# OSLL/slam-constructor

Hardware: AMD Instinct MI355X
Metric: pose-candidates*beams/sec (1080-beam scan, 2000^2 grid) (higher is better)
Workload: dtype f64; 1 GPU; cfg2: tinySLAM HC(dt 0.1, dr 0.1, failed-rounds 128), 1080 beams, 2000x2000 @0.05 m, occupancy cell; parallelism=1 gpu, ranks=1, includes_filter_and_upload=True, mode=default (canonical tree sum, device sincos; com~

## Files before the change

### include/slamhip.h

```cpp
#ifndef SLAMHIP_H
#define SLAMHIP_H

#include <stddef.h>
#include <stdint.h>

#ifdef __cplusplus
extern "C" {
#endif

#define SLAMHIP_VERSION 100

typedef enum {
  SLAMHIP_OK = 0,
  SLAMHIP_ERR_INVALID = -1,
  SLAMHIP_ERR_HIP = -2,
  SLAMHIP_ERR_NO_DEVICE = -3,
  SLAMHIP_ERR_STATE = -4,
  SLAMHIP_ERR_UNSUPPORTED = -5,
  SLAMHIP_ERR_TIMEOUT = -6
} slamhip_status;

enum { SLAMHIP_CELL_OCC = 0, SLAMHIP_CELL_TBM = 1, SLAMHIP_CELL_GMAPPING = 2, SLAMHIP_CELL_CREDIBILIST = 3 };
enum { SLAMHIP_OOPE_OBSTACLE = 0, SLAMHIP_OOPE_MAX = 1, SLAMHIP_OOPE_MEAN = 2,
       SLAMHIP_OOPE_OVERLAP = 3, SLAMHIP_OOPE_GMAPPING = 4 };
enum { SLAMHIP_OIE_DISCREPANCY = 0, SLAMHIP_OIE_OCCUPANCY = 1 };
enum { SLAMHIP_SUM_TREE256 = 0, SLAMHIP_SUM_SEQUENTIAL = 1 };
enum { SLAMHIP_POSE_TRIG_DEVICE = 0, SLAMHIP_POSE_TRIG_HOST = 1,
       SLAMHIP_POSE_TRIG_RAW_EXACT = 2 };
enum { SLAMHIP_TRIG_RAW = 0, SLAMHIP_TRIG_CACHED = 1 };

typedef struct slamhip_ctx slamhip_ctx;
typedef struct slamhip_matcher slamhip_matcher;

typedef struct {
  int oope;
  int oie;
  double area[4];
  double gm_fullness_th;
  int gm_window;
  int sum_order;
  int pose_trig;
} slamhip_spe_cfg;

const char *slamhip_last_error(void);
int slamhip_device_count(int *count);
int slamhip_ctx_create(int device, slamhip_ctx **out);
int slamhip_ctx_destroy(slamhip_ctx *ctx);
int slamhip_ctx_synchronize(slamhip_ctx *ctx);
void *slamhip_ctx_stream(slamhip_ctx *ctx);
enum {
  SLAMHIP_OPT_LOW_LATENCY = 0,
  SLAMHIP_OPT_STAGE_POSES = 1,
  SLAMHIP_OPT_FILTER_CHAINS = 2,
  SLAMHIP_OPT_K6_PATH = 3,
  SLAMHIP_OPT_K6_BATCH_FAST = 4,
  SLAMHIP_OPT_RESIDENT_CHAINS = 6,
  SLAMHIP_OPT_K6_BATCH_KEY64 = 5,
  SLAMHIP_OPT_TBM_PLANE = 7,
  SLAMHIP_OPT_INERT_TAIL = 8
};
int slamhip_ctx_set_option(slamhip_ctx *ctx, int option, int value);
int slamhip_ctx_get_option(slamhip_ctx *ctx, int option, int *value);

int slamhip_map_bind(slamhip_ctx *ctx, int map_id, int cell_model, int width, int height,
                     int origin_x, int origin_y, double scale, const double *unknown_payload);
int slamhip_map_upload_window(slamhip_ctx *ctx, int map_id, int x0, int y0, int w, int h,
                              const double *payload);
int slamhip_map_apply_dirty(slamhip_ctx *ctx, int map_id, int n, const int *coords_xy,
                            const double *payloads);
int slamhip_map_release(slamhip_ctx *ctx, int map_id);
int slamhip_map_set_auto_grow(slamhip_ctx *ctx, int map_id, int on);
int slamhip_map_info(slamhip_ctx *ctx, int map_id, int *cell_model, int *width, int *height, int *origin_x,
                     int *origin_y, double *scale, long long *times_grown);
int slamhip_map_download_window(slamhip_ctx *ctx, int map_id, int x0, int y0, int w, int h,
                                double *payload_out);

enum { SLAMHIP_RENDER_OCCGRID = 0, SLAMHIP_RENDER_PGM = 1 };
enum { SLAMHIP_OCC_TBM_CONSISTENT = 0, SLAMHIP_OCC_TBM_UNKNOWN_EVEN = 1 };
int slamhip_map_render(slamhip_ctx *ctx, int map_id, int format, int occ_kind, int x0, int y0, int w, int h,
                       void *out);
int slamhip_render_cells(int cell_model, int occ_kind, int format, int n, const double *payload, void *out);

enum { SLAMHIP_SCAN_GEN_SEQUENTIAL = 1 };
int slamhip_scan_gen_libm_variant(int *variant);
int slamhip_scan_gen_angles(double half_sector, double angle_inc, int cap, double *angles, int *n);
int slamhip_map_generate_scans(slamhip_ctx *ctx, int map_id, int occ_kind, int variant, int flags, int n_poses,
                               const double *poses_xyt, int n_angles, const double *angles, double max_dist,
                               double occ_threshold, double *range_out, unsigned char *status_out);
int slamhip_scan_generate_host(int cell_model, int occ_kind, int variant, int width, int height, int origin_x, int origin_y,
                               double scale, const double *unknown_payload, const double *payload, int n_poses,
                               const double *poses_xyt, int n_angles, const double *angles, double max_dist,
                               double occ_threshold, double *range_out, unsigned char *status_out);

typedef struct slamhip_pyramid slamhip_pyramid;
int slamhip_pyramid_create(slamhip_ctx *ctx, int fine_map_id, int oie, int first_level_map_id, slamhip_pyramid **out);
int slamhip_pyramid_destroy(slamhip_pyramid *pyr);
int slamhip_pyramid_info(slamhip_pyramid *pyr, int *n_levels, int cap, int *map_id, int *width, int *height,
                         int *origin_x, int *origin_y, double *scale);
int slamhip_pyramid_rebuild(slamhip_pyramid *pyr);
int slamhip_pyramid_refresh(slamhip_pyramid *pyr, int x0, int y0, int w, int h);
int slamhip_pyramid_build_host(int cell_model, int oie, int width, int height, int origin_x, int origin_y, double scale,
                               const double *unknown_payload, const double *payload, int level_cap, int *n_levels,
                               int *level_width, int *level_height, int *level_origin_x, int *level_origin_y,
                               double *level_scale, size_t payload_cap, double *payload_out, size_t *payload_need);
int slamhip_pyramid_score_matches(slamhip_ctx *ctx, slamhip_pyramid *pyr, const slamhip_spe_cfg *cfg,
                                  const double base_pose[3], int n, const double *rotation, const double *rect,
                                  double *score_out, int *level_out);
int slamhip_pyramid_score_matches_device(slamhip_ctx *ctx, slamhip_pyramid *pyr, const slamhip_spe_cfg *cfg,
                                         const double base_pose[3], int n, const double *d_rotation, const double *d_rect,
                                         double *d_score_out, int *d_level_out);

enum { SLAMHIP_RULE_LAST = 0,
       SLAMHIP_RULE_AFFINE = 1,
       SLAMHIP_RULE_MEAN = 2,
       SLAMHIP_RULE_TBM = 3,
       SLAMHIP_RULE_GMAPPING = 4   };
typedef struct {
  int rule;
  double scan_quality;
  double base_occupied_prob, base_occupied_qual;
  double base_empty_prob, base_empty_qual;
  double blur;
  double max_range;
  int occupancy_estimator;
  double area_shift_amount;
} slamhip_scan_adder_cfg;
int slamhip_map_append_scan(slamhip_ctx *ctx, int map_id, const slamhip_scan_adder_cfg *cfg,
                            const double pose[3], int n, const double *range, const double *cos_a,
                            const double *sin_a, const int *is_occ, long long *n_updates);
int slamhip_map_append_scan_q(slamhip_ctx *ctx, int map_id, const slamhip_scan_adder_cfg *cfg,
                              const double pose[3], int n, const double *range, const double *cos_a,
                              const double *sin_a, const int *is_occ, const double *quality, long long *n_updates);
int slamhip_map_append_scan_raw(slamhip_ctx *ctx, int map_id, const slamhip_scan_adder_cfg *cfg, const double pose[3],
                                int n, const double *range, const double *angle, const int *is_occ,
                                const double *quality, long long *n_updates);
int slamhip_omqe_quality(int kind, int n, const double *range, const double *angle, double *out);
int slamhip_map_set_deferred(slamhip_ctx *ctx, int on);
int slamhip_map_drain(slamhip_ctx *ctx, long long *n_updates);
int slamhip_map_download_aux(slamhip_ctx *ctx, int map_id, int x0, int y0, int w, int h, double *out);

int slamhip_scan_upload(slamhip_ctx *ctx, int n, const double *range, const double *cos_a,
                        const double *sin_a, const double *weight, const double *factor);
int slamhip_scan_store(slamhip_ctx *ctx, int slot, int n, const double *range, const double *cos_a,
                       const double *sin_a, const double *weight, const double *factor);
int slamhip_scan_select(slamhip_ctx *ctx, int slot);
int slamhip_scan_set_angles(slamhip_ctx *ctx, int n, const double *angle);
int slamhip_libm_variant(int *variant);
int slamhip_libm_eval(slamhip_ctx *ctx, int variant, int fn, int n, const double *x, double *out);
int slamhip_beam_trig_raw(int n, const double *angle, double *cos_out, double *sin_out);
int slamhip_beam_trig_cached(int n, const double *angle, double a_min, double a_max, double a_inc,
                             double *cos_out, double *sin_out);
int slamhip_filter_scan(int n, const double *range, const double *angle, const int *is_occ,
                        int trig_mode, double a_min, double a_delta, int table_n,
                        const double *tab_sin, const double *tab_cos, const double pose[3],
                        unsigned skip_rate, double max_range, int bounded, int width, int height,
                        int origin_x, int origin_y, double scale, int *kept_idx, int *kept_n);
int slamhip_scan_filter_upload(slamhip_ctx *ctx, int map_id, int n, const double *range, const double *angle,
                               const int *is_occ, const double *factor, int trig_mode, double a_min, double a_max,
                               double a_inc, const double pose[3], unsigned skip_rate, double max_range, int bounded,
                               int weighting, int *kept_n, int *kept_idx);
int slamhip_scan_table_uploads(slamhip_ctx *ctx, long long *uploads);
int slamhip_scan_download(slamhip_ctx *ctx, int cap, double *out5, int *n);
int slamhip_scan_weights(int kind, int n, const double *range, const double *angle, double *out);

int slamhip_score_poses(slamhip_ctx *ctx, int map_id, const slamhip_spe_cfg *cfg, int n_poses,
                        const double *poses_xyt, double *scores_out);
int slamhip_score_poses_device(slamhip_ctx *ctx, int map_id, const slamhip_spe_cfg *cfg,
                               int n_poses, const double *d_poses_xyt, double *d_scores_out);
int slamhip_gm_cache_reset(slamhip_ctx *ctx);
int slamhip_gm_cache_get(slamhip_ctx *ctx, int *cell_xy, double *prob);
int slamhip_gm_cache_set(slamhip_ctx *ctx, const int *cell_xy, double prob);

int slamhip_profile_enable(slamhip_ctx *ctx, int on);
int slamhip_profile_read(slamhip_ctx *ctx, double *kernel_ms_total, long long *launches,
                         long long *units , int reset);

int slamhip_profile_read_map_update(slamhip_ctx *ctx, double *ms_total, long long *calls, long long *records,
                                    int reset);

typedef struct {
  void *user;
  void (*on_scan_test)(void *user, const double pose[3], double score);
  void (*on_pose_update)(void *user, const double pose[3], double score);
  void (*on_matching_end)(void *user, const double delta[3], double best_score);
} slamhip_observer;

int slamhip_matcher_create_mc(slamhip_ctx *ctx, const slamhip_spe_cfg *cfg, unsigned seed,
                              double translation_dispersion, double rotation_dispersion,
                              unsigned failed_attempts_limit, unsigned attempts_limit,
                              slamhip_matcher **out);
int slamhip_matcher_create_hc(slamhip_ctx *ctx, const slamhip_spe_cfg *cfg,
                              unsigned failed_rounds_limit, double translation_delta,
                              double rotation_delta, slamhip_matcher **out);
int slamhip_matcher_create_bf(slamhip_ctx *ctx, const slamhip_spe_cfg *cfg, const double range9[9],
                              slamhip_matcher **out);
int slamhip_matcher_destroy(slamhip_matcher *m);
int slamhip_matcher_reset_state(slamhip_matcher *m);
int slamhip_matcher_set_observer(slamhip_matcher *m, const slamhip_observer *obs);
int slamhip_matcher_set_batch(slamhip_matcher *m, int max_batch);
int slamhip_matcher_set_device_chain(slamhip_matcher *m, int mode, int threads);
int slamhip_matcher_resident_stats(slamhip_matcher *m, long long *matches, long long *gave_up);
int slamhip_matcher_set_tie_check(slamhip_matcher *m, int on);
int slamhip_matcher_process_scan(slamhip_matcher *m, int map_id, const double init_pose[3],
                                 double out_delta[3], double *out_prob);
typedef struct slamhip_raw_scan {
  int n;
  const double *range, *angle;
  const int *is_occ;
  const double *factor;
  int trig_mode;
  double a_min, a_max, a_inc;
// ... 133 lines not shown
```

### slam-constructor_amd/__init__.py

```python
import atexit
import ctypes as C
import os
import subprocess
import weakref

import numpy as np

PKG_DIR = os.path.dirname(os.path.abspath(__file__))
LIB_PATH = os.path.join(PKG_DIR, "libslamhip.so")
TESTING_LIB_PATH = os.path.join(PKG_DIR, "libslamhip_testing.so")
CSRC = os.path.join(PKG_DIR, "csrc")

CELL_OCC, CELL_TBM, CELL_GMAPPING, CELL_CREDIBILIST = 0, 1, 2, 3
OOPE_OBSTACLE, OOPE_MAX, OOPE_MEAN, OOPE_OVERLAP, OOPE_GMAPPING = range(5)
OIE_DISCREPANCY, OIE_OCCUPANCY = 0, 1
SUM_TREE256, SUM_SEQUENTIAL = 0, 1
POSE_TRIG_DEVICE, POSE_TRIG_HOST, POSE_TRIG_RAW_EXACT = 0, 1, 2
(OPT_LOW_LATENCY, OPT_STAGE_POSES, OPT_FILTER_CHAINS, OPT_K6_PATH, OPT_K6_BATCH_FAST, OPT_K6_BATCH_KEY64,
 OPT_RESIDENT_CHAINS, OPT_TBM_PLANE, OPT_INERT_TAIL) = range(9)
TRIG_RAW, TRIG_CACHED = 0, 1
RENDER_OCCGRID, RENDER_PGM = 0, 1
OCC_TBM_CONSISTENT, OCC_TBM_UNKNOWN_EVEN = 0, 1
SCAN_GEN_SEQUENTIAL = 1
SCAN_NO_HIT, SCAN_HIT, SCAN_ASSERT = 0, 1, 2
STRIDE = {CELL_OCC: 1, CELL_TBM: 4, CELL_GMAPPING: 3, CELL_CREDIBILIST: 4}

EXPORTS = """slamhip_last_error slamhip_device_count slamhip_ctx_create slamhip_ctx_destroy
slamhip_ctx_synchronize slamhip_ctx_stream slamhip_ctx_set_option slamhip_ctx_get_option slamhip_map_bind slamhip_map_upload_window
slamhip_map_apply_dirty slamhip_map_release slamhip_map_download_window slamhip_scan_upload
slamhip_beam_trig_raw slamhip_beam_trig_cached slamhip_filter_scan slamhip_scan_weights
slamhip_score_poses slamhip_score_poses_device slamhip_gm_cache_reset slamhip_gm_cache_get slamhip_gm_cache_set
slamhip_profile_enable slamhip_profile_read slamhip_profile_read_map_update slamhip_matcher_create_mc slamhip_matcher_create_hc
slamhip_matcher_create_bf slamhip_matcher_destroy slamhip_matcher_reset_state
slamhip_map_set_auto_grow slamhip_map_info slamhip_map_set_deferred slamhip_map_drain slamhip_matcher_set_observer slamhip_matcher_set_batch slamhip_matcher_set_device_chain slamhip_matcher_set_tie_check slamhip_matcher_process_scan
slamhip_matcher_process_raw_scan slamhip_matcher_stats slamhip_matcher_chain_stats slamhip_matcher_tail_stats slamhip_matcher_resident_stats slamhip_matcher_timing slamhip_pf_normalize slamhip_pf_resampling_is_required slamhip_pf_resample
slamhip_pf_heaviest slamhip_gmapping_create slamhip_gmapping_destroy slamhip_gmapping_predict_match
slamhip_gmapping_plan_resample slamhip_gmapping_blob_size slamhip_gmapping_export
slamhip_gmapping_import slamhip_gmapping_step slamhip_gmapping_set slamhip_gmapping_get
slamhip_gmapping_stats slamhip_gmapping_set_map_update slamhip_map_append_scan slamhip_map_download_aux
slamhip_gmapping_enable_particle_maps slamhip_gmapping_particle_map_download
slamhip_gmapping_particle_map_stats slamhip_gmapping_particle_map_export_size
slamhip_gmapping_particle_map_export slamhip_gmapping_import_maps slamhip_gmapping_particle_maps_append
slamhip_shard_unique_id slamhip_shard_init slamhip_shard_destroy slamhip_shard_info slamhip_shard_allgather
slamhip_shard_stats slamhip_gmapping_set_shard_chain slamhip_gmapping_match_begin slamhip_gmapping_carry_record
slamhip_gmapping_carry_fix slamhip_gmapping_carry_commit slamhip_gmapping_match_finish
slamhip_gmapping_step_sharded slamhip_matcher_process_scan_batch slamhip_matcher_batch_stats slamhip_scan_store slamhip_scan_select
slamhip_shard_attach slamhip_shard_exchange slamhip_shard_p2p_stats slamhip_shard_set_timeout slamhip_gmapping_match_abort
slamhip_gmapping_migration_stats slamhip_map_append_scan_q slamhip_omqe_quality slamhip_scan_filter_upload
slamhip_scan_set_angles slamhip_libm_variant slamhip_libm_eval slamhip_map_append_scan_raw
slamhip_map_render slamhip_gmapping_particle_map_render slamhip_render_cells
slamhip_scan_gen_angles slamhip_scan_gen_libm_variant slamhip_map_generate_scans slamhip_scan_generate_host
slamhip_pyramid_create slamhip_pyramid_destroy slamhip_pyramid_info slamhip_pyramid_rebuild slamhip_pyramid_refresh
slamhip_pyramid_build_host slamhip_pyramid_score_matches slamhip_pyramid_score_matches_device
slamhip_scan_table_uploads slamhip_scan_download""".split()

SHARD_ID_BYTES = 128

_dp = C.POINTER(C.c_double)
_ip = C.POINTER(C.c_int)


class SlamHipError(RuntimeError):
    pass


class ShardMsg(C.Structure):
    _fields_ = [("peer", C.c_int), ("buf", C.c_void_p), ("bytes", C.c_size_t)]


class MatchJob(C.Structure):
    _fields_ = [("map_id", C.c_int), ("scan_slot", C.c_int), ("n", C.c_int), ("range", _dp), ("cos_a", _dp), ("sin_a", _dp),
                ("weight", _dp), ("factor", _dp), ("init_pose", C.c_double * 3)]


class CarryRecord(C.Structure):
    _fields_ = [("has_active", C.c_int), ("first_cx", C.c_int), ("first_cy", C.c_int), ("first_v0", C.c_double),
                ("carry_cx", C.c_int), ("carry_cy", C.c_int), ("carry_prob", C.c_double)]


class SpeCfg(C.Structure):
    _fields_ = [("oope", C.c_int), ("oie", C.c_int), ("area", C.c_double * 4),
                ("gm_fullness_th", C.c_double), ("gm_window", C.c_int), ("sum_order", C.c_int),
                ("pose_trig", C.c_int)]


RULE_LAST, RULE_AFFINE, RULE_MEAN, RULE_TBM, RULE_GMAPPING = range(5)


class ScanAdderCfg(C.Structure):
    _fields_ = [("rule", C.c_int), ("scan_quality", C.c_double), ("base_occupied_prob", C.c_double),
                ("base_occupied_qual", C.c_double), ("base_empty_prob", C.c_double),
                ("base_empty_qual", C.c_double), ("blur", C.c_double), ("max_range", C.c_double),
                ("occupancy_estimator", C.c_int), ("area_shift_amount", C.c_double)]


class GmappingParams(C.Structure):
    _fields_ = [("mean_sample_xy", C.c_double), ("sigma_sample_xy", C.c_double),
                ("mean_sample_th", C.c_double), ("sigma_sample_th", C.c_double),
                ("min_sm_lim_xy", C.c_double), ("max_sm_lim_xy", C.c_double),
                ("min_sm_lim_th", C.c_double), ("max_sm_lim_th", C.c_double),
                ("hc_failed_rounds_limit", C.c_uint), ("hc_translation", C.c_double),
                ("hc_rotation", C.c_double), ("sp_skip_rate", C.c_uint),
                ("sp_max_usable_range", C.c_double), ("oope_fullness_th", C.c_double),
                ("oope_window", C.c_int), ("pose_trig", C.c_int)]


def gmapping_params(gp8=(0.0, 0.1, 0.0, 0.03, 0.6, 0.8, 0.3, 0.4), hc=(6, 0.1, 0.1), skip_rate=0,
                    max_range=-1.0, fullness_th=0.1, window=1, pose_trig=POSE_TRIG_DEVICE):
    p = GmappingParams()
    (p.mean_sample_xy, p.sigma_sample_xy, p.mean_sample_th, p.sigma_sample_th, p.min_sm_lim_xy,
     p.max_sm_lim_xy, p.min_sm_lim_th, p.max_sm_lim_th) = [float(v) for v in gp8]
    p.hc_failed_rounds_limit, p.hc_translation, p.hc_rotation = int(hc[0]), hc[1], hc[2]
    p.sp_skip_rate, p.sp_max_usable_range = skip_rate, max_range
    p.oope_fullness_th, p.oope_window, p.pose_trig = fullness_th, window, pose_trig
    return p


OBS_FN = C.CFUNCTYPE(None, C.c_void_p, _dp, C.c_double)


class Observer(C.Structure):
    _fields_ = [("user", C.c_void_p), ("on_scan_test", OBS_FN), ("on_pose_update", OBS_FN),
                ("on_matching_end", OBS_FN)]


def spe_cfg(oope=OOPE_OBSTACLE, oie=OIE_DISCREPANCY, area=(0, 0, 0, 0), gm_th=0.1, gm_window=1,
            sum_order=SUM_TREE256, pose_trig=POSE_TRIG_DEVICE):
    c = SpeCfg()
    c.oope, c.oie = oope, oie
    for k in range(4):
        c.area[k] = float(area[k])
    c.gm_fullness_th, c.gm_window = gm_th, gm_window
    c.sum_order, c.pose_trig = sum_order, pose_trig
    return c


def build(verbose=False):
    out = None if verbose else subprocess.DEVNULL
    subprocess.check_call(["make", "-j8", "-C", CSRC], stdout=out)
    return LIB_PATH


_libs = {}


def load(testing=False):
    if testing in _libs:
        return _libs[testing]
    path = TESTING_LIB_PATH if testing else LIB_PATH
    if not os.path.exists(path):
        raise SlamHipError("%s is not built (run __graft_entry__.build()); "
                           "there is no CPU fallback" % os.path.basename(path))
    L = C.CDLL(path)
    vp, d, i, u = C.c_void_p, C.c_double, C.c_int, C.c_uint
    L.slamhip_last_error.restype = C.c_char_p
    L.slamhip_ctx_create.argtypes = [i, C.POINTER(vp)]
    L.slamhip_ctx_destroy.argtypes = [vp]
    L.slamhip_ctx_synchronize.argtypes = [vp]
    L.slamhip_ctx_stream.restype = vp
    L.slamhip_ctx_stream.argtypes = [vp]
    L.slamhip_map_bind.argtypes = [vp, i, i, i, i, i, i, d, _dp]
    L.slamhip_map_upload_window.argtypes = [vp, i, i, i, i, i, _dp]
    L.slamhip_map_download_window.argtypes = [vp, i, i, i, i, i, _dp]
    L.slamhip_map_apply_dirty.argtypes = [vp, i, i, _ip, _dp]
    L.slamhip_map_release.argtypes = [vp, i]
    L.slamhip_map_set_auto_grow.argtypes = [vp, i, i]
    L.slamhip_map_info.argtypes = [vp, i, _ip, _ip, _ip, _ip, _ip, _dp, C.POINTER(C.c_longlong)]
    L.slamhip_map_set_deferred.argtypes = [vp, i]
    L.slamhip_map_drain.argtypes = [vp, C.POINTER(C.c_longlong)]
    L.slamhip_scan_upload.argtypes = [vp, i, _dp, _dp, _dp, _dp, _dp]
    L.slamhip_scan_store.argtypes = [vp, i, i, _dp, _dp, _dp, _dp, _dp]
    L.slamhip_scan_select.argtypes = [vp, i]
# ... 1144 lines not shown
```

### slam-constructor_amd/csrc/hc_chain_device.h

```cpp
#pragma once

#include "hc_chain.h"
#include "kernel_pick.h"
#include "slamhip_internal.h"

namespace slamhip {

struct HcTraceEntry {
  double x, y, theta, score;
  int accepted, pad;
};

struct HcHostOut {
  double pose[3];
  double best_prob;
  long long calls, evaluated;
  int steps;
  long long rescored;
  int gm_cx, gm_cy;
  double gm_prob;
  int error;
  unsigned progress;
  unsigned done_seq;
  GmPoseInfo first_info;
  double first_raw;
  long long tail_calls;
};

struct HcChainCtl {
  HcState state[2];
  HcInst walk[2][kHcMaxInst];
  double scores[2][kHcSlots + 7];
  double scores_seq[2][kHcSlots + 7];
  unsigned long long hashes[2][kHcSlots + 7];
  GmPoseInfo infos[2][kHcSlots + 7];
  unsigned done_epoch;
  GmPoseInfo first_info;
  double first_raw;
};

struct alignas(16) HcGranule {
  double score;
  unsigned hash, tag;
};
struct HcResidentCtl {
  HcGranule gran[2][kHcSlots + 7];
  HcGranule seq[2][kHcSlots + 7];
  unsigned fail_epoch;
  unsigned pad[3];
};

struct HcResidentGmCtl {
  HcGranule gran[2][kHcSlots + 7][4];
  unsigned fail_epoch;
  unsigned pad[3];
};

struct HcJobView {
  MapView map;
  ScanView scan;
};

struct HcChainArgs {
  MapView map;
  ScanView scan;
  const HcJobView *jobs;
  int oie;
  GmParams gm;
  int gm_cx, gm_cy;
  double gm_prob;
  int seq;
  int verify;
  HcChainCtl *ctl;
  const double *inits;
  unsigned *n_done;
  const int *tables;
  const int *slots;
  int table_stride;
  const HcShape *shapes;
  int max_inst;
  unsigned long long n_inst;
  double init[3];
  double dt0, dr0;
  unsigned max_failed;
  int shape0;
  unsigned epoch;
  HcHostOut *host;
  HcTraceEntry *trace;
  int trace_cap;
  int trace_stride;
  long long *stamps;
  HcResidentCtl *rctl;
  HcResidentGmCtl *rctl_gm;
  unsigned spin_limit;
  unsigned tag_epoch;
  unsigned *h_all_done;
  int debug_mute;
  int lds_consts;
  int pair;
  int tab_offset;
  int oope;
  double area[4];
  int inert_tail;
};

hipError_t launch_hc_chain_step(const HcChainArgs &a, int cell_model, int k, int nt, hipStream_t stream,
                                hipEvent_t ev_start = nullptr, hipEvent_t ev_stop = nullptr, int n_chains = 1);
hipError_t launch_hc_chain_resident(const HcChainArgs &a, int cell_model, int nt, hipStream_t stream,
                                    hipEvent_t ev_start = nullptr, hipEvent_t ev_stop = nullptr, int n_chains = 1);
hipError_t hc_resident_capacity(int cell_model, HcResidentKey key, int n_beams, bool lds_consts, int *out_wgs,
                                int *out_per_cu = nullptr);
size_t hc_resident_lds_bytes(int nt, int n_beams, bool lds_consts, int max_inst, bool pair = false);
hipError_t launch_hc_chain_resident_gm(const HcChainArgs &a, int nt, hipStream_t stream, hipEvent_t ev_start = nullptr,
                                       hipEvent_t ev_stop = nullptr, int n_chains = 1);
hipError_t hc_resident_gm_capacity(int nt, int n_beams, int *out_wgs, int *out_per_cu = nullptr);
hipError_t launch_chain_marker(const unsigned *n_done, unsigned *h_done_count, unsigned *flag, unsigned seq,
                               hipStream_t stream);

}
```

### slam-constructor_amd/csrc/hc_resident.hip

```cpp
#include <hip/hip_runtime.h>

#include "hc_chain_device.h"
#include "hc_resident_device.h"
#include "score_device.h"

namespace slamhip {

namespace {
constexpr int kSumLanes = 256;
}

template <int H>
struct HcNextEntryT {
  double x, y, theta;
  double p[H][4];
  unsigned counts;
  unsigned flags;
};
static_assert(sizeof(HcNextEntryT<1>) == 64 && sizeof(HcNextEntryT<2>) == 96, "HcNextEntry layout");
static_assert(kHcMaxSeg + 1 <= 15, "HcNextEntry::counts: accepted rounds of a path in 4 bits");
static_assert(6 * kHcMaxInst + 6 < 4096, "HcNextEntry::counts: scorer calls of a path in 12 bits");
__device__ __forceinline__ unsigned hc_entry_counts(const HcNextCore &c, int rounds_acc) {
  return (c.failed & 0xffffu) | (((unsigned)c.batch_calls & 0xfffu) << 16) | (((unsigned)rounds_acc & 0xfu) << 28);
}

__device__ __forceinline__ void wave_min2(double &a, double &b) {
#define HCR_MIN_STEP(OFF)                              \
  {                                                    \
    const double oa = lane_xor_f64<OFF>(a), ob = lane_xor_f64<OFF>(b); \
    a = a < oa ? a : oa;                               \
    b = b < ob ? b : ob;                               \
  }
  HCR_MIN_STEP(32) HCR_MIN_STEP(16) HCR_MIN_STEP(8) HCR_MIN_STEP(4) HCR_MIN_STEP(2) HCR_MIN_STEP(1)
#undef HCR_MIN_STEP
}

constexpr int kSelRescore = -1;
constexpr int kSelFirst = -2;
constexpr int kSelStop = -3;

template <int MODEL, int NT, bool SEQ, bool BATCH, int G, bool WIN = false, bool PAIR = false>
__global__ __launch_bounds__(NT, 4) void k_hc_chain_resident(HcChainArgs a) {
  constexpr int H = PAIR ? 2 : 1;
  constexpr int NTH = NT / H;
  constexpr bool CERT = !WIN;
  typedef HcNextEntryT<H> HcNextEntry;
  extern __shared__ double s_term[];
  __shared__ unsigned long long s_hash[kHcSlots + 7];
  __shared__ double s_sc[kHcSlots + 7];
  __shared__ HcInst s_mine[H][kHcShapes];
  __shared__ double s_cur[H][4];
  __shared__ int s_cur_go[H];
  __shared__ int s_sel;
  __shared__ int s_stop;
  __shared__ HcState s_st;
  __shared__ double s_part[H][4];
  __shared__ unsigned long long s_hpart[H][4];
  __shared__ double s_cert[2][16];
  __shared__ int s_cert_end;
  const int t = threadIdx.x, wave = t >> 6;
  const int half = PAIR ? (t >= NTH ? 1 : 0) : 0;
  const int tl = t - half * NTH, lwave = tl >> 6;
  const bool init_slot = blockIdx.x + 1 == gridDim.x;
  const int slot = init_slot ? kHcSlots - 1 : (PAIR ? 2 * (int)blockIdx.x + half : (int)blockIdx.x);
  const int inst_of_slot = slot / 6, cand = slot - 6 * inst_of_slot;
  const bool exists = init_slot ? half == 0 : slot < 6 * a.max_inst;
  HcResidentCtl *const rc = a.rctl + blockIdx.y;
  HcHostOut *const host = a.host + blockIdx.y;
  const unsigned fail_epoch_at_entry = __hip_atomic_load(&rc->fail_epoch, __ATOMIC_RELAXED, __HIP_MEMORY_SCOPE_AGENT);
#ifdef SLAMHIP_TESTING
  if (a.debug_mute && (int)blockIdx.x + 1 == a.debug_mute) return;
#endif
  MapViewCP map_p;
  ScanViewCP scan_p;
  {
    const __attribute__((address_space(4))) HcChainArgs *ap0 =
        (const __attribute__((address_space(4))) HcChainArgs *)__builtin_amdgcn_kernarg_segment_ptr();
    if (BATCH) {
      const __attribute__((address_space(4))) HcJobView *jv =
          (const __attribute__((address_space(4))) HcJobView *)(unsigned long long)(a.jobs + blockIdx.y);
      map_p = &jv->map;
      scan_p = &jv->scan;
    } else {
      map_p = &ap0->map;
      scan_p = &ap0->scan;
    }
  }
  const ScanView scan = load_view(scan_p);
  const int n = scan.n;
  double br = 0.0, bc = 0.0, bs = 0.0, bw = 0.0, bf = 0.0;
  if (tl < n) {
    br = scan.range[tl];
    bc = scan.cos_a[tl];
    bs = scan.sin_a[tl];
    bw = scan.weight[tl];
    bf = scan.factor[tl];
  }
  if (lwave == 1 && (t & 63) < kHcShapes && !init_slot && exists) {
    const uint4 *src = reinterpret_cast<const uint4 *>(&a.shapes[t & 63].inst[inst_of_slot]);
    uint4 *dst = reinterpret_cast<uint4 *>(&s_mine[half][t & 63]);
#pragma unroll
    for (int q = 0; q < (int)(sizeof(HcInst) / 16); ++q) dst[q] = src[q];
  }
  const bool ldsc = !WIN && a.lds_consts != 0;
  const int n_more = n > NTH ? n - NTH : 0;
  double *const my_term = s_term + (PAIR ? half * a.scan.n : 0);
  double *const s_r = s_term + (PAIR ? 2 * a.scan.n : n) - NTH, *const s_ca = s_r + n_more, *const s_sa = s_ca + n_more;
  if (ldsc) {
    for (int b = NTH + t; b < n; b += NT) {
      s_r[b] = scan.range[b];
      s_ca[b] = scan.cos_a[b];
      s_sa[b] = scan.sin_a[b];
    }
  }
  HcNextEntry *const s_tab = reinterpret_cast<HcNextEntry *>(s_term + a.tab_offset);
  if (t == 0) s_stop = fail_epoch_at_entry == a.epoch ? 1 : 0;
  if (tl < 4 && exists) {
    HcGranule *g0 = (tl & 2) ? &rc->seq[tl & 1][slot] : &rc->gran[tl & 1][slot];
    gran_store(g0, 0.0, 0ull, 0u);
  }
  const bool verify = a.verify != 0;
  const bool stamp = SLAMHIP_STAMPS_ON(a.stamps && slot == 1 && tl == 0 && blockIdx.y == 0);
  HcGranule *const gran = &rc->gran[0][0];
  HcGranule *const gseq = &rc->seq[0][0];
  constexpr int kGranRow = kHcSlots + 7;

  if (t == 0) {
    HcState st{};
    st.x = a.inits ? a.inits[3 * blockIdx.y] : a.init[0];
    st.y = a.inits ? a.inits[3 * blockIdx.y + 1] : a.init[1];
    st.theta = a.inits ? a.inits[3 * blockIdx.y + 2] : a.init[2];
    st.dt = a.dt0;
    st.dr = a.dr0;
    st.shape = a.shape0;
    st.first = 1;
    st.carry_cx = st.carry_cy = -1;
    st.carry_prob = -1.0;
    s_st = st;
    s_sel = kSelFirst;
    s_cert_end = 0;
  }
  __syncthreads();
  if (s_stop) return;
  if (lwave == 0) {
    const HcState &st = s_st;
    bool go = exists;
    double px = st.x, py = st.y, pth = st.theta;
    if (!init_slot && exists) {
      HcInst in;
#pragma unroll
      for (int q = 0; q < 14; ++q) in.w[q] = s_mine[half][st.shape].w[q];
      go = inst_of_slot < (int)((a.n_inst >> (8 * st.shape)) & 0xffull) &&
           (hc_is_root(in) || st.failed + hc_nfail_parent(in) < a.max_failed);
      if (go) {
        const HcRound r = hc_round_of(st, in);
        go = !(hc_trailing(r.failed, a.max_failed) && cand > 0);
        hc_candidate(r.x, r.y, r.theta, r.dt, r.dr, cand, &px, &py, &pth);
      }
    }
    double sn, cs;
    sincos(pth, &sn, &cs);
    if (tl == 0) {
      s_cur[half][0] = px;
      s_cur[half][1] = py;
      s_cur[half][2] = sn;
      s_cur[half][3] = cs;
      s_cur_go[half] = go ? 1 : 0;
    }
  }
  __syncthreads();

  const int t_entry = t;
  for (int k = 0;; ++k) {
    const int pk = k & 1;
    int t = t_entry;
    asm volatile("" : "+v"(t));
    const int lane = t & 63;
    const int tl = PAIR ? t - half * NTH : t;
    const __attribute__((address_space(4))) HcChainArgs *ap =
        (const __attribute__((address_space(4))) HcChainArgs *)__builtin_amdgcn_kernarg_segment_ptr();
    asm volatile("" : "+s"(ap));
    MapViewCP mp = map_p;
    asm volatile("" : "+s"(mp));
    const MapView map = load_view(mp);
    if (stamp && k < 64) ap->stamps[8 * k + 0] = wall_clock64();
    const int sel = s_sel;
    if (sel == kSelStop) break;
    int go, mode = 0;
    double px, py, sn, cs;
    if (sel >= 0) {
      const HcNextEntry &e = s_tab[sel];
      const unsigned flags = e.flags;
      const bool cert_end = CERT && s_cert_end != 0;
      const int done = (int)((flags >> 3) & 1u) | (cert_end ? 1 : 0);
      go = (int)((flags >> (4 + half)) & 1u);
      px = e.p[half][0];
      py = e.p[half][1];
      sn = e.p[half][2];
      cs = e.p[half][3];
      if (wave == NT / 64 - 1 && lane < 1 + H) {
        if (lane == 0) {
          HcState &w = s_st;
          const unsigned counts = e.counts;
          const unsigned failed = counts & 0xffffu;
          const double half = hc_pow_half(failed - w.failed);
          w.x = e.x;
          w.y = e.y;
          w.theta = e.theta;
          w.dt = w.dt * half;
          w.dr = w.dr * half;
          w.recent_acc = 0.5 * w.recent_acc + (double)(counts >> 28);
          w.recent_n = 0.5 * w.recent_n + (double)((counts >> 16) & 0xfffu);
          w.failed = failed;
          w.shape = (int)(flags & 7u);
          w.done = done;
        } else {
          const int hh = lane - 1;
          s_cur[hh][0] = e.p[hh][0];
          s_cur[hh][1] = e.p[hh][1];
          s_cur[hh][2] = e.p[hh][2];
          s_cur[hh][3] = e.p[hh][3];
          s_cur_go[hh] = (int)((flags >> (4 + hh)) & 1u);
        }
      }
      long long tail_calls = 0;
      if (done && ((flags & 64u) || cert_end)) tail_calls = 6ll * (long long)(ap->max_failed - (e.counts & 0xffffu)) + 1ll;
      if (done && init_slot && tail_calls > 0 && ap->trace) {
        __syncthreads();
        HcTraceEntry *const trace = ap->trace + (size_t)blockIdx.y * (size_t)ap->trace_stride;
        const long long at0 = s_st.calls;
        const double best = s_st.best_prob, dt_e = s_st.dt, dr_e = s_st.dr;
        for (long long q = t; q < tail_calls; q += NT) {
          const double hlf = hc_pow_half((unsigned)(q / 6));
          HcTraceEntry te;
          hc_candidate(e.x, e.y, e.theta, dt_e * hlf, dr_e * hlf, (int)(q % 6), &te.x, &te.y, &te.theta);
          te.score = best;
          te.accepted = 0;
          te.pad = 0;
          if (at0 + q < ap->trace_cap) trace[at0 + q] = te;
          else host->error = 2;
        }
        __threadfence_system();
        __syncthreads();
      }
      if (done && init_slot && t == 0) {
        const HcState &w = s_st;
        __threadfence_system();
        HcHostOut *h = host;
        h->pose[0] = e.x;
        h->pose[1] = e.y;
        h->pose[2] = e.theta;
        h->best_prob = w.best_prob;
        h->calls = w.calls + tail_calls;
        h->tail_calls = tail_calls;
        h->evaluated = w.evaluated;
        h->steps = w.steps;
        h->rescored = w.rescored;
        h->gm_cx = -1;
        h->gm_cy = -1;
        h->gm_prob = -1.0;
        __hip_atomic_store(&h->done_seq, ap->epoch, __ATOMIC_RELEASE, __HIP_MEMORY_SCOPE_SYSTEM);
        if (ap->n_done) {
          __threadfence_system();
          const unsigned before = atomicAdd(ap->n_done, 1u);
          if (before + 1u == gridDim.y && ap->h_all_done)
            __hip_atomic_store(ap->h_all_done, ap->epoch, __ATOMIC_RELEASE, __HIP_MEMORY_SCOPE_SYSTEM);
        }
      }
      if (done) break;
    } else {
      if (sel == kSelRescore && init_slot) {
        if (wave == 0) {
          double sn_, cs_;
          sincos(s_st.theta, &sn_, &cs_);
          if (t == 0) {
            s_cur[0][0] = s_st.x;
            s_cur[0][1] = s_st.y;
            s_cur[0][2] = sn_;
            s_cur[0][3] = cs_;
            s_cur_go[0] = 1;
          }
        }
        __syncthreads();
      }
      go = s_cur_go[half];
      px = s_cur[half][0];
      py = s_cur[half][1];
      sn = s_cur[half][2];
      cs = s_cur[half][3];
      mode = sel == kSelRescore ? 1 : 0;
    }
    if (stamp && k < 64) ap->stamps[8 * k + 3] = wall_clock64();
    const unsigned tag = hc_tag(ap->tag_epoch, k);
    if (go) {
      if (WIN) {
        const double half_v = (ap->area[1] - ap->area[0]) / 2, half_h = (ap->area[3] - ap->area[2]) / 2;
        for (int b = tl; b < n; b += NTH) {
          double r_ = br, ca = bc, sa = bs, w = bw, f = bf;
          if (b != tl) {
            r_ = scan.range[b];
            ca = scan.cos_a[b];
            sa = scan.sin_a[b];
            w = scan.weight[b];
            f = scan.factor[b];
          }
          const double c = cs * ca - sn * sa;
          const double s = sn * ca + cs * sa;
          const double ox = px + r_ * c, oy = py + r_ * s;
          my_term[b] = window_probability<MODEL>(map, ap->oie, ap->oope, half_v, half_h, ox, oy) * w * f;
        }
      } else {
        constexpr int UNR = NTH == 256 ? 5 : 4;
        for (int base = tl; base < n; base += UNR * NTH) {
          double4 cell[UNR];
          double w_[UNR], f_[UNR];
  #pragma unroll
          for (int j = 0; j < UNR; ++j) {
            const int b = base + j * NTH;
            w_[j] = 0.0;
            f_[j] = 0.0;
            cell[j] = make_double4(0.0, 0.0, 0.0, 0.0);
            if ((base - lane) + j * NTH >= n) continue;
            const int bc_ = b < n ? b : n - 1;
            double r_ = br, ca = bc, sa = bs;
            w_[j] = bw;
            f_[j] = bf;
            if (j > 0 || base != tl) {
              r_ = ldsc ? s_r[bc_] : scan.range[bc_];
              ca = ldsc ? s_ca[bc_] : scan.cos_a[bc_];
              sa = ldsc ? s_sa[bc_] : scan.sin_a[bc_];
              w_[j] = scan.weight[bc_];
              f_[j] = scan.factor[bc_];
            }
            cell[j] = beam_cell<MODEL>(map, px, py, sn, cs, r_, ca, sa);
          }
  #pragma unroll
          for (int j = 0; j < UNR; ++j) {
            const int b = base + j * NTH;
            if (b < n) my_term[b] = cell_probability<MODEL>(ap->oie, cell[j]) * w_[j] * f_[j];
          }
        }
      }
    }
    double cert_t = 0.0, cert_r = 0.0;
    const bool cert_here = CERT && init_slot && half == 0 && sel >= 0 && !go && ap->inert_tail > 1;
    if (cert_here) {
      const double theta_abs = __builtin_fabs(s_tab[sel].theta);
      double tt = __builtin_inf(), tr = __builtin_inf();
      for (int b = tl; b < n; b += NTH) {
        double r_ = br, ca = bc, sa = bs;
        if (b != tl) {
          r_ = ldsc ? s_r[b] : scan.range[b];
          ca = ldsc ? s_ca[b] : scan.cos_a[b];
          sa = ldsc ? s_sa[b] : scan.sin_a[b];
        }
        double t1, t2;
        hc_cert_beam(px, py, sn, cs, theta_abs, r_, ca, sa, map.scale, map.inv_scale, &t1, &t2);
        tt = tt < t1 ? tt : t1;
        tr = tr < t2 ? tr : t2;
      }
      wave_min2(tt, tr);
      if (lane == 0) {
        s_cert[0][lwave] = tt;
        s_cert[1][lwave] = tr;
      }
    }
    __syncthreads();
    if (cert_here && tl < 64) {
      double tt = tl < NTH / 64 ? s_cert[0][tl] : __builtin_inf(), tr = tl < NTH / 64 ? s_cert[1][tl] : __builtin_inf();
      wave_min2(tt, tr);
      cert_t = tt;
      cert_r = tr;
    }
    if (stamp && k < 64) ap->stamps[8 * k + 4] = wall_clock64();
    if (go) {
      if (SEQ) {
        if (tl == 0) {
          double acc = 0.0;
          int b = 0;
          for (; b + 8 <= n; b += 8) {
            const double t0 = my_term[b], t1 = my_term[b + 1], t2 = my_term[b + 2], t3 = my_term[b + 3];
            const double t4 = my_term[b + 4], t5 = my_term[b + 5], t6 = my_term[b + 6], t7 = my_term[b + 7];
            acc = acc + t0;
            acc = acc + t1;
            acc = acc + t2;
            acc = acc + t3;
            acc = acc + t4;
            acc = acc + t5;
            acc = acc + t6;
            acc = acc + t7;
          }
          for (; b < n; ++b) acc = acc + my_term[b];
          gran_store(&gran[pk * kGranRow + slot], (scan.tot_w == 0.0) ? __builtin_nan("") : acc / scan.tot_w, 0ull, tag);
        }
      } else if (tl < kSumLanes) {
        double acc = 0.0;
        unsigned long long h = 0ull;
        unsigned k_lo = (2u * (unsigned)tl + 1u) * 0x9E3779B1u, k_hi = (2u * (unsigned)tl + 1u) * 0x85EBCA6Bu;
        for (int b = tl; b < n; b += kSumLanes) {
          const double term = my_term[b];
          acc = acc + term;
          if (verify) {
            h += term_fingerprint(term, k_lo, k_hi);
            k_lo += 2u * kSumLanes * 0x9E3779B1u;
            k_hi += 2u * kSumLanes * 0x85EBCA6Bu;
          }
        }
        wave_xor_sum_with(acc, h);
        if (lane == 0) {
          s_part[half][lwave] = acc;
          s_hpart[half][lwave] = h;
        }
      }
    }
    __syncthreads();
    if (go) {
      if (!SEQ) {
        if (tl == 0) {
          const double total = (s_part[half][0] + s_part[half][1]) + (s_part[half][2] + s_part[half][3]);
          const unsigned long long fp =
              verify ? fold_fingerprint48(s_hpart[half][0] + s_hpart[half][1] + s_hpart[half][2] + s_hpart[half][3]) : 0ull;
          gran_store(&gran[pk * kGranRow + slot], (scan.tot_w == 0.0) ? __builtin_nan("") : total / scan.tot_w, fp, tag);
        }
        if (verify && mode && tl == 64) {
          double acc = 0.0;
          for (int b = 0; b < n; ++b) acc = acc + my_term[b];
          gran_store(&gseq[pk * kGranRow + slot], (scan.tot_w == 0.0) ? __builtin_nan("") : acc / scan.tot_w, 0ull, tag);
        }
      }
      if (stamp && k < 64) ap->stamps[8 * k + 5] = wall_clock64();
    } else if (tl == 0 && exists) {
      gran_store(&gran[pk * kGranRow + slot], cert_here ? cert_t : 0.0,
                 cert_here ? (unsigned long long)__double_as_longlong(cert_r) >> 16 : 0ull, tag);
      if (verify && mode) gran_store(&gseq[pk * kGranRow + slot], 0.0, 0ull, tag);
    }

    if (wave != 0) {
      {
        const HcState &sp = s_st;
        const int shape = sp.shape;
        const int n_inst = (int)((ap->n_inst >> (8 * shape)) & 0xffull);
        const unsigned max_failed = ap->max_failed;
        for (int e = t - 64; e < 7 * n_inst; e += NT - 64) {
          const int ti = e / 7, out = e - 7 * ti;
          HcInst in;
          {
            const unsigned long long *src = &ap->shapes[shape].inst[ti].w[0];
#pragma unroll
            for (int q = 0; q < 14; ++q) in.w[q] = src[q];
          }
          if (!(hc_is_root(in) || sp.failed + hc_nfail_parent(in) < max_failed)) continue;
          const bool trailing = hc_trailing(sp.failed + hc_nfail(in), max_failed);
          if (trailing ? out > 1 : hc_child(in, out) >= 0) continue;
          const HcRound r = hc_round_of(sp, in);
          const HcNextCore c = hc_next_core(sp, in, r, out, max_failed);
          HcNextEntry &w = s_tab[e];
          w.x = c.x;
          w.y = c.y;
          w.theta = c.theta;
          w.counts = hc_entry_counts(c, hc_nseg(in) + (out > 0 ? 1 : 0));
          const bool inert = !c.done && ap->inert_tail && hc_inert(c.x, c.y, c.theta, c.dt, c.dr);
          unsigned flags = (unsigned)c.shape | (c.done || inert ? 8u : 0u) | (inert ? 64u : 0u);
#pragma unroll
          for (int hh = 0; hh < H; ++hh) {
            const int slot_h = PAIR ? 2 * (int)blockIdx.x + hh : slot;
            const int inst_h = slot_h / 6, cand_h = slot_h - 6 * inst_h;
            bool go = !c.done && !inert && !init_slot && slot_h < 6 * ap->max_inst;
            double px_ = c.x, py_ = c.y, pth_ = c.theta;
            if (go) {
              HcInst mine;
#pragma unroll
              for (int q = 0; q < 14; ++q) mine.w[q] = s_mine[hh][c.shape].w[q];
              go = inst_h < (int)((ap->n_inst >> (8 * c.shape)) & 0xffull) &&
                   (hc_is_root(mine) || c.failed + hc_nfail_parent(mine) < max_failed);
              if (go) {
                const HcRound r2 = hc_round_from(c.x, c.y, c.theta, c.dt, c.dr, c.failed, mine);
                go = !(hc_trailing(r2.failed, max_failed) && cand_h > 0);
                hc_candidate(r2.x, r2.y, r2.theta, r2.dt, r2.dr, cand_h, &px_, &py_, &pth_);
              }
            }
            double sn_ = 0.0, cs_ = 1.0;
            if (go || (CERT && init_slot && hh == 0 && ap->inert_tail > 1)) sincos(pth_, &sn_, &cs_);
            w.p[hh][0] = px_;
            w.p[hh][1] = py_;
            w.p[hh][2] = sn_;
            w.p[hh][3] = cs_;
            flags |= go ? (16u << hh) : 0u;
          }
          w.flags = flags;
        }
      }
    } else {
      const HcState &sp = s_st;
      const int n_inst = (int)((ap->n_inst >> (8 * sp.shape)) & 0xffull);
      HcInst me;
      {
        const unsigned long long *src = &ap->shapes[sp.shape].inst[lane].w[0];
#pragma unroll
        for (int q = 0; q < 14; ++q) me.w[q] = src[q];
      }
      const bool active = lane < n_inst;
      const bool reach = active && (hc_is_root(me) || sp.failed + hc_nfail_parent(me) < ap->max_failed);
      const bool trailing = reach && hc_trailing(sp.failed + hc_nfail(me), ap->max_failed);
      const int bpi = hc_bp_inst(me);
      const int bp_slot = (!active || bpi < 0) ? -1 : 6 * bpi + hc_bp_cand(me);
      const bool base_here = sp.first || sp.mode == 1;
      const int n_grid = 6 * ap->max_inst;
      const bool rescored = !SEQ && verify && sp.mode == 1;
      bool failed = false;
      {
        const HcGranule *g0 = gran + pk * kGranRow;
        unsigned spins = 0;
        for (;;) {
          u32x4 g[G];
          const HcGranule *gp[G];
          bool ok = true;
#pragma unroll
          for (int q = 0; q < G; ++q) {
            const int i = lane + 64 * q;
            gp[q] = g0 + (i < n_grid ? i : kHcSlots - 1);
          }
          gran_fetch(g, gp);
#pragma unroll
          for (int q = 0; q < G; ++q) {
            const int i = lane + 64 * q;
            const int j = i < n_grid ? i : kHcSlots - 1;
            const bool here = gran_tag(g[q]) == tag;
            ok = ok && here;
            if (here) {
              s_sc[j] = gran_score(g[q]);
              s_hash[j] = gran_hash(g[q]);
            }
          }
          if (__all(ok)) break;
          ++spins;
          if (BATCH) __builtin_amdgcn_s_sleep(8);
          if ((spins & 31u) == 0u) {
            const bool gone = __hip_atomic_load(&rc->fail_epoch, __ATOMIC_RELAXED, __HIP_MEMORY_SCOPE_AGENT) == ap->epoch;
            if (gone || spins > ap->spin_limit) {
              failed = true;
              break;
            }
          }
        }
      }
      if (stamp && k < 64) ap->stamps[8 * k + 1] = wall_clock64();
      if (failed || k + 1 >= kHcResidentMaxSteps) {
        if (lane == 0) {
          __hip_atomic_store(&rc->fail_epoch, ap->epoch, __ATOMIC_RELAXED, __HIP_MEMORY_SCOPE_AGENT);
          __hip_atomic_store(&host->error, failed ? 4 : 5, __ATOMIC_RELAXED, __HIP_MEMORY_SCOPE_SYSTEM);
          __threadfence_system();
          __hip_atomic_store(&host->done_seq, ap->epoch, __ATOMIC_RELEASE, __HIP_MEMORY_SCOPE_SYSTEM);
          s_sel = kSelStop;
        }
      } else {
        double root_prob = sp.first ? s_sc[kHcSlots - 1] : sp.best_prob;
        double s6[6];
#pragma unroll
        for (int c = 0; c < 6; ++c) s6[c] = s_sc[6 * lane + c];
        const double enter = bp_slot < 0 ? root_prob : s_sc[bp_slot];
        double run = enter;
        int out = 0;
        unsigned accmask = 0u;
        bool ambiguous = false;
        unsigned long long run_hash = 0ull;
        if (!SEQ && verify) {
          const unsigned long long root_hash = base_here ? s_hash[kHcSlots - 1] : sp.best_hash;
          unsigned long long hb = bp_slot < 0 ? root_hash : s_hash[bp_slot];
          unsigned long long h6[6];
#pragma unroll
          for (int c = 0; c < 6; ++c) h6[c] = s_hash[6 * lane + c];
          if (!rescored) {
            int amb = 0;
#pragma unroll
            for (int c = 0; c < 6; ++c) {
              const double s = s6[c];
              const double diff = __builtin_fabs(s - run);
              const double as = __builtin_fabs(s), ab = __builtin_fabs(run);
              const int live = (c == 0) | (int)!trailing;
              const int close = (int)(diff <= (as > ab ? as : ab) * 9.094947017729282e-13);
              amb |= live & close & ((int)(h6[c] != hb) | (int)(__double_as_longlong(s) != __double_as_longlong(run)));
              const bool acc = (live & (int)(run < s)) != 0;
              run = acc ? s : run;
              hb = acc ? h6[c] : hb;
              out = acc ? c + 1 : out;
              accmask |= acc ? 1u << c : 0u;
            }
            ambiguous = amb != 0;
          } else {
            const HcGranule *q0 = gseq + pk * kGranRow;
            double bdec = 0.0;
#pragma unroll 1
            for (int c = -1; c < 6; ++c) {
              const int j = c < 0 ? (bp_slot < 0 ? kHcSlots - 1 : bp_slot) : (active ? 6 * lane + c : kHcSlots - 1);
              double sd = 0.0;
              for (unsigned spins = 0;; ++spins) {
                u32x4 g[1];
                const HcGranule *gp[1] = {q0 + j};
                gran_fetch(g, gp);
                sd = gran_score(g[0]);
                if (__all(gran_tag(g[0]) == tag) || spins > ap->spin_limit) break;
              }
              if (c < 0) {
                bdec = sd;
                continue;
              }
              const bool acc = active && (c == 0 || !trailing) && bdec < sd;
              bdec = acc ? sd : bdec;
              run = acc ? s_sc[6 * lane + c] : run;
              hb = acc ? s_hash[6 * lane + c] : hb;
              out = acc ? c + 1 : out;
              accmask |= acc ? 1u << c : 0u;
            }
          }
          run_hash = hb;
        } else {
#pragma unroll
          for (int c = 0; c < 6; ++c)
            if ((c == 0 || !trailing) && run < s6[c]) {
              run = s6[c];
              out = c + 1;
              accmask |= 1u << c;
            }
        }
        bool valid = reach;
#pragma unroll
        for (int o = 0; o < 7; ++o) {
          const unsigned long long has = __ballot(reach && out == o);
          valid = valid && (me.w[o] & ~has) == 0ull;
        }
        const bool terminal = valid && (trailing || hc_child(me, out) < 0);
        const unsigned long long tmask = __ballot(terminal);
        const int tl = tmask ? __ffsll((long long)tmask) - 1 : 0;
        if (stamp && k < 64) ap->stamps[8 * k + 7] = wall_clock64();
        const bool dirty = !SEQ && verify && sp.mode == 0 && __ballot(valid && ambiguous) != 0ull;
        const int out_t = bcast_i(out, tl);
        const double run_t = bcast(run, tl);
        const int depth_t = bcast_i(hc_depth(me), tl);
        const bool trailing_t = bcast_i(trailing ? 1 : 0, tl) != 0;
        const unsigned long long run_hash_t = (unsigned long long)bcast_ll((long long)run_hash, tl);
        if (init_slot && ap->trace && !dirty) {
          HcTraceEntry *const trace = ap->trace + (size_t)blockIdx.y * (size_t)ap->trace_stride;
          const long long base = sp.calls + (sp.first ? 1 : 0);
          if (sp.first && lane == 0 && ap->trace_cap > 0) {
            HcTraceEntry e{sp.x, sp.y, sp.theta, root_prob, 1, 0};
            trace[0] = e;
          }
          if (valid) {
            const HcRound rr = hc_round_of(sp, me);
            const int nc = trailing ? 1 : 6;
            for (int c = 0; c < nc; ++c) {
              HcTraceEntry e;
              hc_candidate(rr.x, rr.y, rr.theta, rr.dt, rr.dr, c, &e.x, &e.y, &e.theta);
              e.score = s_sc[6 * lane + c];
              e.accepted = (accmask >> c) & 1u;
              e.pad = 0;
              const long long at = base + 6ll * hc_depth(me) + c;
              if (at < ap->trace_cap) trace[at] = e;
              else host->error = 2;
            }
          }
        }
        bool cert_end = false;
        if (CERT && ap->inert_tail > 1 && !sp.first && sp.mode == 0 && !dirty && tmask != 0ull) {
          const int nseg_t = bcast_i(hc_nseg(me), tl), nfail_t = bcast_i((int)hc_nfail(me), tl);
          const unsigned failed_next = sp.failed + (unsigned)nfail_t + 1u;
          if (nseg_t == 0 && out_t == 0 && !trailing_t && failed_next < ap->max_failed) {
            const double hlf = hc_pow_half((unsigned)nfail_t + 1u);
            const double t_t = s_sc[kHcSlots - 1];
            const double t_r = __longlong_as_double((long long)(s_hash[kHcSlots - 1] << 16));
            cert_end = sp.dt * hlf < t_t && sp.dr * hlf < t_r;
          }
        }
        if (stamp && k < 64) ap->stamps[8 * k + 2] = wall_clock64();
        if (lane == 0) {
          s_cert_end = cert_end ? 1 : 0;
          HcState &w = s_st;
          if (tmask == 0ull) {
            if (init_slot) {
              __hip_atomic_store(&host->error, 1, __ATOMIC_RELAXED, __HIP_MEMORY_SCOPE_SYSTEM);
              __threadfence_system();
              __hip_atomic_store(&host->done_seq, ap->epoch, __ATOMIC_RELEASE, __HIP_MEMORY_SCOPE_SYSTEM);
            }
            s_sel = kSelStop;
          } else if (!dirty) {
            w.best_prob = run_t;
            w.calls = sp.calls + (sp.first ? 1 : 0) + 6ll * depth_t + (trailing_t ? 1 : 6);
            w.evaluated = sp.evaluated + 6ll * n_inst + (sp.first ? 1 : 0);
            w.first = 0;
            w.mode = 0;
            w.steps = sp.steps + 1;
            if (!SEQ && verify) w.best_hash = run_hash_t;
            s_sel = 7 * tl + out_t;
          } else {
            w.mode = 1;
            w.steps = sp.steps + 1;
            w.evaluated = sp.evaluated + 6ll * n_inst + 1;
            w.rescored = sp.rescored + 1;
            s_sel = kSelRescore;
          }
        }
      }
    }
    __syncthreads();
  }
}

size_t hc_resident_tab_offset(int nt, int n_beams, bool lds_consts, bool pair) {
  const size_t n = (size_t)(n_beams > 0 ? n_beams : 1);
  const size_t nth = (size_t)(pair ? nt / 2 : nt);
  const size_t more = lds_consts && n > nth ? n - nth : 0;
  return (pair ? 2 : 1) * n + 3 * more;
}
size_t hc_resident_lds_bytes(int nt, int n_beams, bool lds_consts, int max_inst, bool pair) {
  return sizeof(double) * hc_resident_tab_offset(nt, n_beams, lds_consts, pair) +
         (pair ? sizeof(HcNextEntryT<2>) : sizeof(HcNextEntryT<1>)) * 7 * (size_t)max_inst;
}

typedef void (*HcResidentKernel)(HcChainArgs);
static HcResidentKernel hc_resident_kernel(int cell_model, const HcResidentKey &key) {
  int nt_v = 0, g_v = 0;
  if (!hc_resident_variant(key, &nt_v, &g_v)) return nullptr;
  return pick_cell_model(cell_model, [&](auto model) -> HcResidentKernel {
    constexpr int M = decltype(model)::value;
    return pick_hc_nt(nt_v, [&](auto nt) -> HcResidentKernel {
      constexpr int NT = decltype(nt)::value;
      if (key.window) return k_hc_chain_resident<M, NT, false, false, 4, true>;
      const auto sweep = [&](auto g) -> HcResidentKernel {
        constexpr int G = decltype(g)::value;
        if constexpr (NT == 512)
          if (key.batch && key.pair) return k_hc_chain_resident<M, 512, false, true, G, false, true>;
        if (key.batch) return k_hc_chain_resident<M, NT, false, true, G>;
        return key.seq ? k_hc_chain_resident<M, NT, true, false, G> : k_hc_chain_resident<M, NT, false, false, G>;
      };
      if (g_v == 2) return sweep(int_c<2>{});
      if (g_v == 4) return sweep(int_c<4>{});
      if constexpr (NT != 1024) return sweep(int_c<7>{});
      return nullptr;
    });
  });
}

static HcResidentKey key_of(const HcChainArgs &a, int nt) {
  return {nt, a.max_inst, a.seq != 0, a.jobs != nullptr, a.pair != 0, a.oope != SLAMHIP_OOPE_OBSTACLE};
}

hipError_t launch_hc_chain_resident(const HcChainArgs &a_in, int cell_model, int nt, hipStream_t stream, hipEvent_t e0,
                                    hipEvent_t e1, int n_chains) {
  if (!a_in.rctl) return hipErrorInvalidValue;
  HcChainArgs a = a_in;
  const HcResidentKey key = key_of(a, nt);
  const bool pair = key.batch && key.pair;
  const bool ldsc = !key.window && a.lds_consts != 0;
  const int grid = pair ? 3 * a.max_inst + 1 : 6 * a.max_inst + 1;
  a.tab_offset = (int)hc_resident_tab_offset(nt, a.scan.n, ldsc, pair);
  return launch_kernel(hc_resident_kernel(cell_model, key), dim3(grid, n_chains), dim3(hc_nt_of(nt)),
                       hc_resident_lds_bytes(nt, a.scan.n, ldsc, a.max_inst, pair), stream, e0, e1, a);
}

hipError_t hc_resident_capacity(int cell_model, HcResidentKey key, int n_beams, bool lds_consts, int *out_wgs,
                                int *out_per_cu) {
  key.seq = false;
  return resident_capacity_of((const void *)hc_resident_kernel(cell_model, key), key.nt,
                              hc_resident_lds_bytes(key.nt, n_beams, lds_consts, key.max_inst, key.batch && key.pair),
                              2048 / key.nt , 6, out_wgs, out_per_cu);
}

}
```

### slam-constructor_amd/csrc/kernel_pick.h

```cpp
#pragma once

#include <hip/hip_runtime_api.h>

#include <type_traits>

#include "slamhip.h"

extern "C" hipError_t hipExtLaunchKernel(const void *function_address, dim3 numBlocks, dim3 dimBlocks, void **args,
                                         size_t sharedMemBytes, hipStream_t stream, hipEvent_t startEvent,
                                         hipEvent_t stopEvent, int flags);

namespace slamhip {

template <int V>
using int_c = std::integral_constant<int, V>;

template <class F>
auto pick_cell_model(int model, F &&f) -> decltype(f(int_c<SLAMHIP_CELL_OCC>{})) {
  switch (model) {
    case SLAMHIP_CELL_OCC: return f(int_c<SLAMHIP_CELL_OCC>{});
    case SLAMHIP_CELL_TBM: return f(int_c<SLAMHIP_CELL_TBM>{});
    case SLAMHIP_CELL_CREDIBILIST: return f(int_c<SLAMHIP_CELL_CREDIBILIST>{});
    default: return nullptr;
  }
}
template <class F>
auto pick_belief_model(int model, F &&f) -> decltype(f(int_c<SLAMHIP_CELL_TBM>{})) {
  switch (model) {
    case SLAMHIP_CELL_TBM: return f(int_c<SLAMHIP_CELL_TBM>{});
    case SLAMHIP_CELL_CREDIBILIST: return f(int_c<SLAMHIP_CELL_CREDIBILIST>{});
    default: return nullptr;
  }
}
template <class F>
auto pick_bool(bool b, F &&f) -> decltype(f(std::false_type{})) {
  return b ? f(std::true_type{}) : f(std::false_type{});
}
constexpr int hc_nt_of(int nt) { return nt == 256 || nt == 1024 ? nt : 512; }
constexpr int mc_nt_of(int nt) { return nt == 512 ? 512 : 1024; }
template <class F>
auto pick_hc_nt(int nt, F &&f) -> decltype(f(int_c<512>{})) {
  switch (hc_nt_of(nt)) {
    case 256: return f(int_c<256>{});
    case 1024: return f(int_c<1024>{});
    default: return f(int_c<512>{});
  }
}
template <class F>
auto pick_mc_nt(int nt, F &&f) -> decltype(f(int_c<512>{})) {
  return mc_nt_of(nt) == 512 ? f(int_c<512>{}) : f(int_c<1024>{});
}

template <class... P>
hipError_t launch_kernel(void (*kernel)(P...), dim3 grid, dim3 block, size_t lds_bytes, hipStream_t stream, hipEvent_t e0,
                         hipEvent_t e1, typename std::common_type<P>::type... args) {
  if (!kernel) return hipErrorInvalidValue;
  void *argv[] = {(void *)&args..., nullptr};
  if (e0 || e1) hipExtLaunchKernel((const void *)kernel, grid, block, argv, lds_bytes, stream, e0, e1, 0);
  else hipLaunchKernel((const void *)kernel, grid, block, argv, lds_bytes, stream);
  return hipGetLastError();
}

constexpr int hc_gran_per_lane(int grid) { return grid <= 128 ? 2 : (grid <= 256 ? 4 : 7); }

struct HcResidentKey {
  int nt, max_inst;
  bool seq, batch, pair, window;
};
inline bool hc_resident_variant(const HcResidentKey &k, int *nt, int *g) {
  const int slots = 6 * k.max_inst + 1;
  *nt = hc_nt_of(k.nt);
  *g = k.window ? 4 : hc_gran_per_lane(slots);
  if (k.seq && k.batch) return false;
  if (k.window) return !k.seq && !k.batch && slots <= 256;
  if (k.batch && k.pair) return k.nt == 512;
  return !(*nt == 1024 && *g == 7);
}

inline hipError_t resident_capacity_of(const void *kernel, int nt, size_t lds_bytes, int by_waves, int per_cu_cap,
                                       int *out_wgs, int *out_per_cu) {
  if (!kernel) return hipErrorInvalidValue;
  int dev = 0, cus = 0, per_cu = 0;
  hipError_t e = hipGetDevice(&dev);
  if (e != hipSuccess) return e;
  e = hipDeviceGetAttribute(&cus, hipDeviceAttributeMultiprocessorCount, dev);
  if (e != hipSuccess) return e;
  e = hipOccupancyMaxActiveBlocksPerMultiprocessor(&per_cu, kernel, nt, lds_bytes);
  if (e != hipSuccess) return e;
  per_cu = per_cu < by_waves ? per_cu : by_waves;
  if (per_cu_cap > 0 && per_cu > per_cu_cap) per_cu = per_cu_cap;
  *out_wgs = per_cu * (cus - 1);
  if (out_per_cu) *out_per_cu = per_cu;
  return hipSuccess;
}

}
```

### slam-constructor_amd/csrc/matchers.cpp

```cpp

#include <cstdlib>
#include <limits>
#include <mutex>

#include "bf_device.h"
#include "hc_chain_device.h"
#include "hc_shape.h"
#include "mc_chain_device.h"
#include "matchers.h"
#include "resident_policy.h"

namespace slamhip {

template <class T, bool kPinned>
class HipBlock {
  T *p_ = nullptr;

 public:
  HipBlock() = default;
  HipBlock(const HipBlock &) = delete;
  HipBlock &operator=(const HipBlock &) = delete;
  HipBlock(HipBlock &&o) noexcept : p_(o.p_) { o.p_ = nullptr; }
  HipBlock &operator=(HipBlock &&o) noexcept {
    if (this != &o) {
      reset();
      p_ = o.p_;
      o.p_ = nullptr;
    }
    return *this;
  }
  ~HipBlock() { reset(); }
  T *get() const { return p_; }
  explicit operator bool() const { return p_ != nullptr; }
  void reset() {
    if (p_) {
      if constexpr (kPinned) hipHostFree(p_);
      else hipFree(p_);
    }
    p_ = nullptr;
  }
  hipError_t alloc(size_t count, unsigned pinned_flags = 0) {
    reset();
    if constexpr (kPinned) return hipHostMalloc(&p_, sizeof(T) * count, pinned_flags);
    else return hipMalloc(&p_, sizeof(T) * count);
  }
};
template <class T>
using DeviceBuf = HipBlock<T, false>;
template <class T>
using PinnedBuf = HipBlock<T, true>;
constexpr unsigned kPinnedCoherent = hipHostMallocMapped | hipHostMallocCoherent;

template <class Entry>
struct StageBlock {
  PinnedBuf<char> h;
  DeviceBuf<char> d;
  size_t table_at = 0;
  int alloc(int cap, hipStream_t stream) {
    table_at = 16 + ((sizeof(double) * 3 * (size_t)cap + 15) & ~(size_t)15);
    const size_t bytes = table_at + ((sizeof(Entry) * (size_t)cap + 15) & ~(size_t)15);
    SLAMHIP_CHECK(h.alloc(bytes, hipHostMallocMapped));
    std::memset(h.get(), 0, bytes);
    SLAMHIP_CHECK(d.alloc(bytes));
    SLAMHIP_CHECK(hipMemsetAsync(d.get(), 0, bytes, stream));
    return SLAMHIP_OK;
  }
  unsigned *d_n_done() const { return reinterpret_cast<unsigned *>(d.get()); }
  double *h_inits() const { return reinterpret_cast<double *>(h.get() + 16); }
  double *d_inits() const { return reinterpret_cast<double *>(d.get() + 16); }
  Entry *h_table() const { return reinterpret_cast<Entry *>(h.get() + table_at); }
  Entry *d_table() const { return reinterpret_cast<Entry *>(d.get() + table_at); }
  size_t bytes_upto_inits(int n) const { return 16 + sizeof(double) * 3 * (size_t)n; }
  size_t bytes_upto_table(int n) const { return table_at + sizeof(Entry) * (size_t)n; }
};

struct ShapeSizes {
  int n_inst[kHcShapes] = {0};
  int max_inst = 1;
  unsigned long long packed() const {
    unsigned long long v = 0;
    for (int b = 0; b < kHcShapes; ++b) v |= (unsigned long long)(n_inst[b] & 0xff) << (8 * b);
    return v;
  }
};

template <class Rctl, class Entry>
struct ChainSet {
  int cap = 0;
  DeviceBuf<HcChainCtl> d_ctl;
  PinnedBuf<HcHostOut> h_out;
  StageBlock<Entry> stage;
  DeviceBuf<HcShape> d_shapes;
  ShapeSizes shapes;
  int built_inst = 0, nt = 256;
  PinnedBuf<unsigned> h_done_count;
  DeviceBuf<Rctl> d_rctl;
  PinnedBuf<unsigned> h_all_done;
  int rctl_grid = 0, rctl_chains = 0;
  unsigned rctl_launches = 0;
  unsigned epoch = 0;
  double steps_avg;
  explicit ChainSet(double steps_avg0) : steps_avg(steps_avg0) {}
};

}

struct BatchJobResult {
  double pose[3] = {0, 0, 0}, prob = 0;
  long long calls = 0, evaluated = 0, rescored = 0;
  int steps = 0, error = 0;
  bool on_chain = false;
};
struct HcBatch : slamhip::ChainSet<slamhip::HcResidentCtl, slamhip::HcJobView> {
  HcBatch() : ChainSet(16.0) {}
  bool resident_call = false;
  slamhip::PinnedBuf<double> h_scan;
  slamhip::DeviceBuf<double> d_scan;
  size_t scan_cap = 0;
  bool pair = false;
  int cus = 0;
  slamhip::PinnedBuf<slamhip::HcTraceEntry> h_trace;
  int trace_per = 0, trace_chains = 0;
  long long kernels = 0;
  std::vector<BatchJobResult> res;
};

struct slamhip_matcher {
  slamhip_ctx *ctx = nullptr;
  slamhip_spe_cfg cfg{};
  std::unique_ptr<slamhip::PoseEnumerator> pe;
  slamhip_observer obs{};
  bool has_obs = false;
  bool is_hc = false, is_mc = false, is_bf = false;
  int max_batch = 0;
  double p_accept0 = 0.25;
  slamhip::MatchJob job;
  double t_stage_us = 0, t_score_us = 0;
  int device = 0;
  int tie_check = -1;
  long long chain_rescored = 0;
  long long tail_calls = 0;
  long long rescored_poses = 0;
  std::vector<double> keep_scores;
  std::vector<unsigned long long> keep_fprints;
  int chain_mode = -1;
  bool chain_mode_explicit = false;
  int chain_nt = 1024, chain_ahead = 3;
  unsigned chain_epoch = 0;
  double chain_steps_avg = 12.0;
  long long chain_launched = 0;
  unsigned rctl_launches = 0;
  slamhip::ResidentPolicy resident;
  enum class ResidentForm { Lone, Batch, Window, MonteCarlo, Pair };
  struct ResidentCap {
    int cell_model, nt;
    ResidentForm form;
    int n_beams, lds_consts, max_inst, cap, per_cu;
  };
  std::vector<ResidentCap> resident_caps;
  slamhip::PinnedBuf<slamhip::HcTraceEntry> h_trace;
  int trace_cap = 0;
  slamhip::DeviceBuf<long long> d_stamps;
  int debug_resident_mute = 0;
  int debug_trace_cap = 0;
  int debug_fail_next = 0;
  struct HcChain {
    unsigned max_failed = 0;
    double dt = 0, dr = 0;
    slamhip::DeviceBuf<slamhip::HcChainCtl> d_chain;
    slamhip::DeviceBuf<slamhip::HcShape> d_shapes;
    slamhip::PinnedBuf<slamhip::HcHostOut> h_chain;
    slamhip::ShapeSizes shapes;
    slamhip::DeviceBuf<slamhip::HcResidentCtl> d_rctl;
    slamhip::DeviceBuf<slamhip::HcResidentGmCtl> d_rctl_gm;
  } hc;
  std::unique_ptr<HcBatch> batch;
  struct McChain {
    slamhip::DeviceBuf<slamhip::McChainCtl> d_mc;
    slamhip::PinnedBuf<slamhip::McHostOut> h_mc;
    slamhip::DeviceBuf<slamhip::McResidentCtl> d_rctl;
    int rctl_grid = 0;
    slamhip::DeviceBuf<slamhip::McPair> d_tape;
    slamhip::PinnedBuf<double> h_tape;
    size_t tape_cap = 0;
    size_t tape_base = 0;
    size_t tape_filled = 0;
    hipStream_t tape_stream = nullptr;
    hipEvent_t tape_ready = nullptr;
    int slots = 0;
    ~McChain() {
      if (tape_stream) hipStreamDestroy(tape_stream);
      if (tape_ready) hipEventDestroy(tape_ready);
    }
  } mc;
  struct BfSweep {
    double r[9] = {0};
    std::vector<double> off;
    int nx = 0, ny = 0, nt = 0;
    slamhip::DeviceBuf<double> d_off, d_poses, d_scores, d_agg_s;
    slamhip::DeviceBuf<unsigned long long> d_fp;
    slamhip::DeviceBuf<long long> d_pidx, d_agg_i;
    slamhip::DeviceBuf<unsigned> d_counters;
    slamhip::PinnedBuf<slamhip::BfHostOut> h_out;
    long long cap = 0;
    unsigned seq = 0;
    std::vector<double> scores_host;
  } bf;
};

using namespace slamhip;

namespace {

int invalid_arg(const char *msg) {
  set_error(msg);
  return SLAMHIP_ERR_INVALID;
}

int make_matcher(slamhip_ctx *ctx, const slamhip_spe_cfg *cfg, std::unique_ptr<PoseEnumerator> pe,
                 int default_batch, slamhip_matcher **out) {
  if (!ctx || !cfg || !out) return invalid_arg("null argument");
  auto *m = new slamhip_matcher;
  m->ctx = ctx;
  m->device = ctx->device;
  m->cfg = *cfg;
  m->pe = std::move(pe);
  m->max_batch = default_batch;
  *out = m;
  return SLAMHIP_OK;
}

constexpr int kChainNeedsHost = 1;
constexpr int kChainUnsettled = 3;
constexpr int kChainDefaultMode = 2;


unsigned next_epoch(unsigned &counter) {
  if (++counter == 0) ++counter;
  return counter;
}

void replay_trace(const slamhip_observer &obs, const HcTraceEntry *entries, long long calls) {
  for (long long i = 0; i < calls; ++i) {
    const HcTraceEntry &e = entries[i];
    const double p3[3] = {e.x, e.y, e.theta};
    if (obs.on_scan_test) obs.on_scan_test(obs.user, p3, e.score);
    if (e.accepted && obs.on_pose_update) obs.on_pose_update(obs.user, p3, e.score);
  }
}

int build_shapes(int want, double reach, HcShape *d_shapes, ShapeSizes *sizes) {
  std::vector<HcShape> shapes(kHcShapes);
  sizes->max_inst = 1;
  for (int b = 0; b < kHcShapes; ++b) {
    hc_build_shape(hc_bucket_rate(b), 1.0, reach, want, &shapes[b]);
    sizes->n_inst[b] = shapes[b].n_inst;
    sizes->max_inst = std::max(sizes->max_inst, shapes[b].n_inst);
  }
  SLAMHIP_CHECK(hipMemcpy(d_shapes, shapes.data(), sizeof(HcShape) * kHcShapes, hipMemcpyHostToDevice));
  return SLAMHIP_OK;
}

bool hc_limit_on_device(const slamhip_matcher *m) {
  if (m->hc.max_failed == 0 || m->hc.max_failed > 1000) return false;
  for (double step : {m->hc.dt, m->hc.dr}) {
    if (step == 0.0) continue;
    int e = 0;
    (void)std::frexp(std::fabs(step), &e);
    if (!std::isfinite(step) || e - 1 - (int)m->hc.max_failed - 1 < -1021) return false;
  }
  return true;
}

bool is_window_oope(int oope) {
  return oope == SLAMHIP_OOPE_MAX || oope == SLAMHIP_OOPE_MEAN || oope == SLAMHIP_OOPE_OVERLAP;
}

bool tie_check_default(slamhip_matcher *m) {
  if (m->tie_check < 0) m->tie_check = 1;
  return m->tie_check == 1;
}

bool chain_eligible(slamhip_matcher *m) {
  if (!m->is_hc || !hc_limit_on_device(m)) return false;
  const bool gm = m->cfg.oope == SLAMHIP_OOPE_GMAPPING;
  const bool win = is_window_oope(m->cfg.oope);
  if (win && (m->cfg.sum_order != SLAMHIP_SUM_TREE256 || m->chain_mode == 1)) return false;
  if ((m->cfg.oope != SLAMHIP_OOPE_OBSTACLE && !gm && !win) || m->cfg.pose_trig != SLAMHIP_POSE_TRIG_DEVICE) return false;
  if (gm && (m->cfg.gm_window != 1 || m->cfg.sum_order != SLAMHIP_SUM_TREE256 || m->ctx->scan_n > 1280)) return false;
  if (!m->ctx->low_latency || m->ctx->stage_poses) return false;
  if (m->ctx->scan_n > 4096) return false;
  if (m->max_batch < 6 * kHcMaxInst) return false;
  if (m->chain_mode < 0) m->chain_mode = kChainDefaultMode;
  return m->chain_mode >= 1;
}

bool hc_resident_asked(slamhip_matcher *m) {
  const bool gm = m->cfg.oope == SLAMHIP_OOPE_GMAPPING && m->chain_mode_explicit;
  const bool armed = m->resident.armed();
  return m->chain_mode == 2 && (m->cfg.oope == SLAMHIP_OOPE_OBSTACLE || is_window_oope(m->cfg.oope) || gm) && armed;
}
std::mutex g_resident_mu;
int g_resident_cus[64] = {0};
int g_device_cus[64] = {0};
struct ResidentLease {
  int device = -1, cus = 0;
  bool take(int dev, int wgs, int per_cu) {
    if (dev < 0 || dev >= 64 || per_cu <= 0) return false;
    std::lock_guard<std::mutex> lk(g_resident_mu);
    if (g_device_cus[dev] == 0) {
      int n = 0;
      if (hipDeviceGetAttribute(&n, hipDeviceAttributeMultiprocessorCount, dev) != hipSuccess || n <= 1) return false;
      g_device_cus[dev] = n;
    }
    const int need = (wgs + per_cu - 1) / per_cu;
    if (g_resident_cus[dev] + need > g_device_cus[dev] - 1) return false;
    g_resident_cus[dev] += need;
    device = dev;
    cus = need;
    return true;
  }
  void release() {
    if (device < 0) return;
    std::lock_guard<std::mutex> lk(g_resident_mu);
    g_resident_cus[device] -= cus;
    device = -1;
  }
  ~ResidentLease() { release(); }
};

using ResidentForm = slamhip_matcher::ResidentForm;
int resident_capacity(slamhip_matcher *m, int cell_model, int nt, ResidentForm form, int n_beams, bool lds_consts, int max_inst,
                      int *wgs, int *per_cu = nullptr) {
  for (const auto &c : m->resident_caps)
    if (c.cell_model == cell_model && c.nt == nt && c.form == form && c.n_beams == n_beams &&
        c.lds_consts == (lds_consts ? 1 : 0) && c.max_inst == max_inst) {
      *wgs = c.cap;
      if (per_cu) *per_cu = c.per_cu;
      return SLAMHIP_OK;
    }
  int cap = 0, pc = 0;
  if (form == ResidentForm::MonteCarlo) {
    SLAMHIP_CHECK(mc_resident_capacity(cell_model, nt, n_beams, lds_consts, &cap, &pc));
  } else {
    const bool pair = form == ResidentForm::Pair;
    const HcResidentKey key{nt, max_inst, false, pair || form == ResidentForm::Batch, pair, form == ResidentForm::Window};
    SLAMHIP_CHECK(hc_resident_capacity(cell_model, key, n_beams, lds_consts, &cap, &pc));
  }
  if (cap < 0) cap = 0;
  if (m->resident_caps.size() >= 64) m->resident_caps.clear();
  m->resident_caps.push_back({cell_model, nt, form, n_beams, lds_consts ? 1 : 0, max_inst, cap, pc});
  *wgs = cap;
  if (per_cu) *per_cu = pc;
  return SLAMHIP_OK;
}
int resident_capacity_pick(slamhip_matcher *m, int cell_model, int nt, ResidentForm form, int n_beams, int max_inst, int wgs_needed,
                           bool may_lds_consts, int *lds_consts, int *wgs, int *per_cu = nullptr) {
  *lds_consts = 0;
  if (may_lds_consts) {
    int rc = resident_capacity(m, cell_model, nt, form, n_beams, true, max_inst, wgs, per_cu);
    if (rc) return rc;
    if (wgs_needed <= *wgs) {
      *lds_consts = 1;
      return SLAMHIP_OK;
    }
  }
  return resident_capacity(m, cell_model, nt, form, n_beams, false, max_inst, wgs, per_cu);
}

struct LoneChainText {
  const char *resident_ended, *resident, *no_end, *step;
};

template <bool kResident, class HostOut, class LaunchOne, class Idle>
int lone_chain_wait(slamhip_ctx *ctx, volatile HostOut *h, unsigned epoch, int ahead, const int &launched,
                    LaunchOne &&launch_one, Idle &&idle, const LoneChainText &text) {
  unsigned long long spins = 0;
  while (h->done_seq != epoch) {
    if constexpr (!kResident) {
      const int started = (int)h->progress;
      if (launched - started < ahead) {
        if (launched >= (1 << 20)) {
          set_error(text.no_end);
          return SLAMHIP_ERR_STATE;
        }
        const int rc = launch_one();
        if (rc) return rc;
        continue;
      }
    }
    const int rc = idle();
    if (rc) return rc;
    if ((++spins & 0xfffffull) == 0) {
      hipError_t qe = hipStreamQuery(ctx->stream);
      if (kResident && qe == hipSuccess && h->done_seq != epoch) {
        set_error(text.resident_ended);
        return SLAMHIP_ERR_STATE;
      }
      if (qe != hipSuccess && qe != hipErrorNotReady) return hip_fail(qe, kResident ? text.resident : text.step);
    }
  }
  __atomic_thread_fence(__ATOMIC_ACQUIRE);
  return SLAMHIP_OK;
}

template <class Args, class HostOut, class Fit, class LaunchResident, class FailOver, class LaunchStep, class Idle>
int run_lone_chain(slamhip_matcher *m, Args &a, volatile HostOut *h, bool resident, const double &t0, int *launched_out,
                   Fit &&fit, LaunchResident &&launch_resident, FailOver &&fail_over, LaunchStep &&launch_step,
                   Idle &&idle, const LoneChainText &text) {
  slamhip_ctx *ctx = m->ctx;
  int launched = 0, rc = SLAMHIP_OK;
  auto launch_one = [&]() -> int {
    hipEvent_t e0, e1;
    int r = profile_event_pair(ctx, &e0, &e1);
    if (r) return r;
    SLAMHIP_CHECK(launch_step(launched, e0, e1));
    ++launched;
    return SLAMHIP_OK;
  };
  bool ran_resident = false;
  if (resident) {
    ResidentLease lease;
    bool fits = false, gave_up = false;
    rc = fit(lease, &fits);
    if (rc) return rc;
    if (fits) {
      a.spin_limit = m->resident.spin_limit();
      a.tag_epoch = ++m->rctl_launches;
      a.debug_mute = m->debug_resident_mute;
      hipEvent_t e0, e1;
      rc = profile_event_pair(ctx, &e0, &e1);
      if (rc) return rc;
      SLAMHIP_CHECK(launch_resident(e0, e1));
      launched = 1;
      m->resident.note_launch();
      rc = lone_chain_wait<true>(ctx, h, a.epoch, 0, launched, launch_one, idle, text);
      if (rc) return rc;
      if (h->error == 4 || h->error == 5) {
        SLAMHIP_CHECK(hipStreamSynchronize(ctx->stream));
        if (h->error == 4) m->resident.note_give_up();
        h->error = 0;
        launched = 0;
        gave_up = true;
      } else {
        m->resident.note_success(MatchJob::now_us() - t0);
        ran_resident = true;
      }
    }
    if (!ran_resident) {
      rc = fail_over(gave_up);
      if (rc) return rc;
    }
  }
  if (!ran_resident) {
    const int first = std::max(2, std::min(256, (int)(m->chain_steps_avg * 0.75)));
    for (int i = 0; i < first; ++i) {
      rc = launch_one();
      if (rc) return rc;
    }
    rc = lone_chain_wait<false>(ctx, h, a.epoch, m->chain_ahead, launched, launch_one, idle, text);
    if (rc) return rc;
  }
  *launched_out = launched;
  return SLAMHIP_OK;
}

template <class HostOut>
int lone_chain_report(slamhip_matcher *m, volatile HostOut *h, int launched, int scan_n, double t0,
                      const double init_pose[3], double out_delta[3], double *out_prob) {
  slamhip_ctx *ctx = m->ctx;
  MatchJob &job = m->job;
  job.scorer_calls = h->calls;
  job.poses_evaluated = h->evaluated;
  job.launches = h->steps;
  job.t_build_us = job.t_replay_us = 0;
  m->chain_launched = launched;
  m->chain_rescored = h->rescored;
  m->chain_steps_avg = 0.75 * m->chain_steps_avg + 0.25 * (double)h->steps;
  if (ctx->profile) {
    ctx->prof_launches += launched;
    ctx->prof_units += h->evaluated * (long long)scan_n;
  }
  out_delta[0] = h->pose[0] - init_pose[0];
  out_delta[1] = h->pose[1] - init_pose[1];
  out_delta[2] = h->pose[2] - init_pose[2];
  *out_prob = h->best_prob;
  m->t_score_us = MatchJob::now_us() - t0;
  if (m->has_obs) {
    const double t1 = MatchJob::now_us();
    replay_trace(m->obs, m->h_trace.get(), h->calls);
    job.t_replay_us = MatchJob::now_us() - t1;
    if (m->obs.on_matching_end) m->obs.on_matching_end(m->obs.user, out_delta, *out_prob);
  }
  return SLAMHIP_OK;
}

int chain_prepare(slamhip_matcher *m) {
  slamhip_matcher::HcChain &hc = m->hc;
  if (hc.d_chain) return SLAMHIP_OK;
  SLAMHIP_CHECK(hc.d_chain.alloc(1));
  SLAMHIP_CHECK(hipMemsetAsync(hc.d_chain.get(), 0, sizeof(HcChainCtl), m->ctx->stream));
  SLAMHIP_CHECK(hc.d_shapes.alloc(kHcShapes));
  const int rc = build_shapes(kHcDefaultInst, 0.002, hc.d_shapes.get(), &hc.shapes);
  if (rc) return rc;
  SLAMHIP_CHECK(hc.h_chain.alloc(1, kPinnedCoherent));
  std::memset(hc.h_chain.get(), 0, sizeof(HcHostOut));
  return SLAMHIP_OK;
}

int chain_process_scan(slamhip_matcher *m, int map_id, const double init_pose[3], double out_delta[3],
                       double *out_prob, bool resident) {
  slamhip_ctx *ctx = m->ctx;
  slamhip_matcher::HcChain &hc = m->hc;
  int rc = chain_prepare(m);
  if (rc) return rc;
  HcChainArgs a;
  std::memset(&a, 0, sizeof(a));
  int cell_model = 0, oie_eff = m->cfg.oie;
  rc = score_views(ctx, map_id, &m->cfg, &a.map, &a.scan, &cell_model, nullptr, &oie_eff);
  if (rc) return rc;
  if (m->has_obs && !m->h_trace) {
    m->trace_cap = 1 << 16;
    SLAMHIP_CHECK(m->h_trace.alloc(m->trace_cap, kPinnedCoherent));
  }
  const bool win = is_window_oope(m->cfg.oope), gm = m->cfg.oope == SLAMHIP_OOPE_GMAPPING;
  a.oie = oie_eff;
  a.oope = win ? m->cfg.oope : SLAMHIP_OOPE_OBSTACLE;
  for (int k = 0; k < 4; ++k) a.area[k] = m->cfg.area[k];
  if (win && !resident) return kChainNeedsHost;
  a.max_inst = hc.shapes.max_inst;
  a.gm.fullness_th = m->cfg.gm_fullness_th;
  a.gm.window = m->cfg.gm_window;
  a.gm_cx = ctx->gm_cx;
  a.gm_cy = ctx->gm_cy;
  a.gm_prob = ctx->gm_prob;
  a.seq = m->cfg.sum_order == SLAMHIP_SUM_SEQUENTIAL ? 1 : 0;
  a.verify = (tie_check_default(m) && !a.seq) ? 1 : 0;
  a.inert_tail = ctx->inert_tail;
  a.ctl = hc.d_chain.get();
  a.shapes = hc.d_shapes.get();
  a.n_inst = hc.shapes.packed();
  for (int k = 0; k < 3; ++k) a.init[k] = init_pose[k];
  a.dt0 = hc.dt;
  a.dr0 = hc.dr;
  a.max_failed = hc.max_failed;
  a.shape0 = hc_bucket_of(m->p_accept0);
  a.epoch = next_epoch(m->chain_epoch);
  a.host = hc.h_chain.get();
  a.trace = m->has_obs ? m->h_trace.get() : nullptr;
  a.trace_cap = m->has_obs ? m->trace_cap : 0;
  if (m->has_obs && m->debug_trace_cap > 0) a.trace_cap = std::min(a.trace_cap, m->debug_trace_cap);
  a.stamps = m->d_stamps.get();
  volatile HcHostOut *h = hc.h_chain.get();
  h->error = 0;
  h->progress = 0;
  h->tail_calls = 0;
  double t0 = MatchJob::now_us();
  const HcChainArgs a_chain = a;
  const int grid = 6 * a.max_inst + 1;
  int launched = 0;
  rc = run_lone_chain(
      m, a, h, resident, t0, &launched,
      [&](ResidentLease &lease, bool *fits) -> int {
        int cap = 0, per_cu = 0, r = SLAMHIP_OK;
        if (gm) SLAMHIP_CHECK(hc_resident_gm_capacity(m->chain_nt, a.scan.n, &cap, &per_cu));
        else r = resident_capacity_pick(m, cell_model, m->chain_nt, win ? ResidentForm::Window : ResidentForm::Lone, a.scan.n,
                                        a.max_inst, grid, !win, &a.lds_consts, &cap, &per_cu);
        if (r) return r;
        if (grid > cap || !lease.take(m->device, grid, per_cu)) return SLAMHIP_OK;
        if (gm && !hc.d_rctl_gm) {
          SLAMHIP_CHECK(hc.d_rctl_gm.alloc(1));
          SLAMHIP_CHECK(hipMemsetAsync(hc.d_rctl_gm.get(), 0, sizeof(HcResidentGmCtl), ctx->stream));
        }
        if (!gm && !hc.d_rctl) {
          SLAMHIP_CHECK(hc.d_rctl.alloc(1));
          SLAMHIP_CHECK(hipMemsetAsync(hc.d_rctl.get(), 0, sizeof(HcResidentCtl), ctx->stream));
        }
        a.rctl = hc.d_rctl.get();
        a.rctl_gm = hc.d_rctl_gm.get();
        *fits = true;
        return SLAMHIP_OK;
      },
      [&](hipEvent_t e0, hipEvent_t e1) {
        return gm ? launch_hc_chain_resident_gm(a, m->chain_nt, ctx->stream, e0, e1)
                  : launch_hc_chain_resident(a, cell_model, m->chain_nt, ctx->stream, e0, e1);
      },
      [&](bool) -> int {
        if (win) return kChainNeedsHost;
        a = a_chain;
        a.epoch = next_epoch(m->chain_epoch);
        h->progress = 0;
        h->tail_calls = 0;
        t0 = MatchJob::now_us();
        return SLAMHIP_OK;
      },
      [&](int step, hipEvent_t e0, hipEvent_t e1) {
        return launch_hc_chain_step(a, cell_model, step, m->chain_nt, ctx->stream, e0, e1);
      },
      []() -> int {
        __builtin_ia32_pause();
        return SLAMHIP_OK;
      },
      LoneChainText{"internal: the co-resident chain ended without publishing a result", "co-resident hill-climbing chain",
                    "hill-climbing chain did not end", "hill-climbing chain kernel"});
  if (rc) return rc;
  m->chain_launched = launched;
  if (h->error == 1) {
    set_error("internal: the device replay found no terminal round (hill-climbing chain bug)");
    return SLAMHIP_ERR_STATE;
  }
  if (h->error == 7) return kChainUnsettled;
  if (h->error == 2 || h->error == 3) return kChainNeedsHost;
  if (gm) {
    ctx->gm_cx = h->gm_cx;
    ctx->gm_cy = h->gm_cy;
    ctx->gm_prob = h->gm_prob;
  }
  m->tail_calls = h->tail_calls;
  return lone_chain_report(m, h, launched, a.scan.n, t0, init_pose, out_delta, out_prob);
}

struct ManyChainsText {
  const char *resident, *no_end;
};
inline void set_rctl(HcChainArgs &a, HcResidentCtl *p) { a.rctl = p; }
inline void set_rctl(HcChainArgs &a, HcResidentGmCtl *p) { a.rctl_gm = p; }

template <class Set>
int many_chains_prepare(slamhip_ctx *ctx, Set &s, int n, int want, double reach, int cap0) {
  if (want != s.built_inst) {
    SLAMHIP_CHECK(hipStreamSynchronize(ctx->stream));
    const int rc = build_shapes(want, reach, s.d_shapes.get(), &s.shapes);
    if (rc) return rc;
    s.built_inst = want;
  }
  const int total = n * (6 * s.shapes.max_inst + 1);
  s.nt = total <= 256 ? 1024 : (total <= 512 ? 512 : 256);
  if (n > s.cap) {
    SLAMHIP_CHECK(hipStreamSynchronize(ctx->stream));
    s.d_rctl.reset();
    s.rctl_grid = s.rctl_chains = 0;
    int cap = cap0;
    while (cap < n) cap *= 2;
    SLAMHIP_CHECK(s.d_ctl.alloc(cap));
    SLAMHIP_CHECK(hipMemsetAsync(s.d_ctl.get(), 0, sizeof(HcChainCtl) * cap, ctx->stream));
    SLAMHIP_CHECK(s.h_out.alloc(cap, kPinnedCoherent));
    std::memset(s.h_out.get(), 0, sizeof(HcHostOut) * cap);
    const int rc = s.stage.alloc(cap, ctx->stream);
    if (rc) return rc;
    s.cap = cap;
  }
  return SLAMHIP_OK;
}

template <class Set>
void many_chains_args(Set &s, int n, HcChainArgs &a) {
  a.max_inst = s.shapes.max_inst;
  a.ctl = s.d_ctl.get();
  a.inits = s.stage.d_inits();
  a.n_done = s.stage.d_n_done();
  a.shapes = s.d_shapes.get();
  a.n_inst = s.shapes.packed();
  a.epoch = next_epoch(s.epoch);
  a.host = s.h_out.get();
  volatile HcHostOut *h = s.h_out.get();
  for (int c = 0; c < n; ++c) {
    h[c].error = 0;
    h[c].progress = 0;
    h[c].tail_calls = 0;
  }
}

template <class Set, class Fit, class LaunchResident, class LaunchStep, class Collect>
int run_many_chains(slamhip_ctx *ctx, ResidentPolicy &policy, Set &s, HcChainArgs &a, int n, bool resident,
                    double first_burst, bool *ran_resident_out, int *launched_out, Fit &&fit,
                    LaunchResident &&launch_resident, LaunchStep &&launch_step, Collect &&collect,
                    const ManyChainsText &text) {
  hipStream_t st = ctx->stream;
  volatile HcHostOut *h_out = s.h_out.get();
  int launched = 0, rc = SLAMHIP_OK;
  bool ran_resident = false;
  if (resident) {
    ResidentLease lease;
    bool fits = false;
    rc = fit(lease, &fits);
    if (rc) return rc;
    if (fits) {
      const double t_res0 = MatchJob::now_us();
      a.spin_limit = policy.spin_limit();
      if (!s.d_rctl) {
        SLAMHIP_CHECK(s.d_rctl.alloc(s.cap));
        SLAMHIP_CHECK(hipMemsetAsync(s.d_rctl.get(), 0, sizeof(*s.d_rctl.get()) * s.cap, st));
      }
      if (!s.h_all_done) {
        SLAMHIP_CHECK(s.h_all_done.alloc(1, kPinnedCoherent));
        *s.h_all_done.get() = 0;
      }
      if (6 * s.shapes.max_inst + 1 > s.rctl_grid || n > s.rctl_chains)
        SLAMHIP_CHECK(hipMemsetAsync(s.d_rctl.get(), 0, sizeof(*s.d_rctl.get()) * s.cap, st));
      s.rctl_grid = 6 * s.shapes.max_inst + 1;
      s.rctl_chains = n;
      set_rctl(a, s.d_rctl.get());
      a.tag_epoch = ++s.rctl_launches;
      a.h_all_done = s.h_all_done.get();
      hipEvent_t e0, e1;
      rc = profile_event_pair(ctx, &e0, &e1);
      if (rc) return rc;
      SLAMHIP_CHECK(launch_resident(e0, e1));
      launched = 1;
      policy.note_launch();
      volatile unsigned *all_done = s.h_all_done.get();
      unsigned long long spins = 0;
      bool gave_up = false;
      for (;;) {
        if (*all_done == a.epoch) break;
        __builtin_ia32_pause();
        if ((++spins & 0xffffull) == 0) {
          for (int c = 0; c < n && !gave_up; ++c)
            gave_up = h_out[c].done_seq == a.epoch && (h_out[c].error == 4 || h_out[c].error == 5);
          if (gave_up) break;
          hipError_t qe = hipStreamQuery(st);
          if (qe == hipSuccess && *all_done != a.epoch) {
            gave_up = true;
            break;
          }
          if (qe != hipSuccess && qe != hipErrorNotReady) return hip_fail(qe, text.resident);
        }
      }
      if (gave_up) {
        SLAMHIP_CHECK(hipStreamSynchronize(st));
        policy.note_give_up();
        SLAMHIP_CHECK(hipMemsetAsync(s.stage.d_n_done(), 0, sizeof(unsigned), st));
        for (int c = 0; c < n; ++c) h_out[c].error = 0;
        a.rctl = nullptr;
        a.rctl_gm = nullptr;
        a.h_all_done = nullptr;
        a.debug_mute = 0;
        launched = 0;
        a.epoch = next_epoch(s.epoch);
      } else {
        ran_resident = true;
        policy.note_success(MatchJob::now_us() - t_res0);
      }
    }
  }
  auto burst = [&](int count, unsigned *seq_out) -> int {
    for (int i = 0; i < count; ++i) {
      hipEvent_t e0, e1;
      int r = profile_event_pair(ctx, &e0, &e1);
      if (r) return r;
      SLAMHIP_CHECK(launch_step(launched, e0, e1));
      ++launched;
    }
    const unsigned seq = next_epoch(ctx->seq);
    SLAMHIP_CHECK(launch_chain_marker(s.stage.d_n_done(), s.h_done_count.get(), ctx->h_done_flag, seq, st));
    *seq_out = seq;
    return SLAMHIP_OK;
// ... 730 lines not shown
int slamhip_matcher_set_device_chain(slamhip_matcher *m, int mode, int threads) {
  if (!m || mode < 0 || mode > 2 || (threads != 0 && threads != 256 && threads != 512 && threads != 1024))
    return invalid_arg("bad device-chain setting");
  (void)chain_eligible(m);
  m->chain_mode = mode;
  m->chain_mode_explicit = true;
  m->resident.reset();
  if (threads) m->chain_nt = threads;
  return SLAMHIP_OK;
}

int slamhip_matcher_set_tie_check(slamhip_matcher *m, int on) {
  if (!m || (on != 0 && on != 1)) return invalid_arg("bad tie-check setting");
  m->tie_check = on;
  return SLAMHIP_OK;
}

#ifdef SLAMHIP_TESTING
int slamhip_matcher_debug_stamps(slamhip_matcher *m, long long *out512) {
  if (!m) return invalid_arg("null matcher");
  if (!m->d_stamps) {
    SLAMHIP_CHECK(m->d_stamps.alloc(512));
    SLAMHIP_CHECK(hipMemset(m->d_stamps.get(), 0, sizeof(long long) * 512));
    SLAMHIP_CHECK(hipDeviceSynchronize());
    return SLAMHIP_OK;
  }
  SLAMHIP_CHECK(hipDeviceSynchronize());
  if (out512) SLAMHIP_CHECK(hipMemcpy(out512, m->d_stamps.get(), sizeof(long long) * 512, hipMemcpyDeviceToHost));
  return SLAMHIP_OK;
}
#endif

int slamhip_matcher_process_scan_batch(slamhip_matcher *m, int n_jobs, const slamhip_match_job *jobs,
                                       double *out_deltas, double *out_probs) {
  if (!m || n_jobs < 0 || (n_jobs > 0 && (!jobs || !out_deltas || !out_probs))) return invalid_arg("null argument");
  if (n_jobs == 0) return SLAMHIP_OK;
  slamhip_ctx *ctx = m->ctx;
  for (int c = 0; c < n_jobs; ++c) {
    const slamhip_match_job &j = jobs[c];
    if (j.scan_slot >= 0) {
      if (j.scan_slot >= (int)ctx->scan_slots.size() || !ctx->scan_slots[j.scan_slot].d)
        return invalid_arg("a match job names a scan slot nothing is stored in");
    } else if (j.n <= 0 || !j.range || !j.cos_a || !j.sin_a || !j.weight) {
      return invalid_arg("bad scan in a match job");
    }
  }
  SLAMHIP_CHECK(hipSetDevice(ctx->device));
  if (!m->batch) m->batch = std::make_unique<HcBatch>();
  HcBatch *b = m->batch.get();
  b->res.assign(n_jobs, BatchJobResult{});
  b->kernels = 0;
  bool chains = n_jobs > 1 && batch_chain_eligible(m);
  for (int c = 0; c < n_jobs && chains; ++c)
    chains = (jobs[c].scan_slot >= 0 ? ctx->scan_slots[jobs[c].scan_slot].n : jobs[c].n) <= 4096;
  if (chains) {
    const int rc = hc_batch_run(m, n_jobs, jobs);
    if (rc) return rc;
  }
  long long calls = 0, evaluated = 0, steps = 0;
  const double *saved_ptr = ctx->scan_ptr;
  const size_t saved_stride = ctx->scan_stride;
  const int saved_n = ctx->scan_n;
  const double saved_tot_w = ctx->scan_tot_w;
  std::vector<double> saved_w, saved_f;
  bool fell_back = false, uploaded = false;
  for (int c = 0; c < n_jobs; ++c) {
    BatchJobResult &r = b->res[c];
    const slamhip_match_job &j = jobs[c];
    double *dl = out_deltas + 3 * c;
    if (r.on_chain) {
      for (int q = 0; q < 3; ++q) dl[q] = r.pose[q] - j.init_pose[q];
      out_probs[c] = r.prob;
      if (m->has_obs) {
        replay_trace(m->obs, b->h_trace.get() + (size_t)c * b->trace_per, r.calls);
        if (m->obs.on_matching_end) m->obs.on_matching_end(m->obs.user, dl, r.prob);
      }
    } else {
      if (!fell_back) {
        saved_w = ctx->h_weight;
        saved_f = ctx->h_factor;
        fell_back = true;
      }
      uploaded = uploaded || j.scan_slot < 0;
      int rc = j.scan_slot >= 0 ? slamhip_scan_select(ctx, j.scan_slot)
                                : slamhip_scan_upload(ctx, j.n, j.range, j.cos_a, j.sin_a, j.weight, j.factor);
      if (rc) return rc;
      rc = slamhip_matcher_process_scan(m, j.map_id, j.init_pose, dl, &out_probs[c]);
      if (rc) return rc;
      r.calls = m->job.scorer_calls;
      r.evaluated = m->job.poses_evaluated;
      r.steps = (int)m->job.launches;
      r.rescored = m->chain_rescored;
      for (int q = 0; q < 3; ++q) r.pose[q] = j.init_pose[q] + dl[q];
      r.prob = out_probs[c];
    }
    calls += r.calls;
    evaluated += r.evaluated;
    steps = std::max<long long>(steps, r.steps);
  }
  if (fell_back) {
    if (uploaded && saved_ptr == ctx->d_scan) {
      ctx->scan_n = 0;
    } else {
      ctx->scan_ptr = saved_ptr;
      ctx->scan_stride = saved_stride;
      ctx->scan_n = saved_n;
      ctx->scan_tot_w = saved_tot_w;
      ctx->h_weight.swap(saved_w);
      ctx->h_factor.swap(saved_f);
    }
  }
  m->job.scorer_calls = calls;
  m->job.poses_evaluated = evaluated;
  m->job.launches = steps;
  m->chain_launched = b->kernels;
  long long resc = 0;
  for (const BatchJobResult &r : b->res) resc += r.rescored;
  m->chain_rescored = resc;
  return SLAMHIP_OK;
}

int slamhip_matcher_batch_stats(slamhip_matcher *m, int job, long long *scorer_calls, long long *poses_evaluated,
                                long long *super_steps, int *on_device_chain) {
  if (!m || !m->batch || job < 0 || job >= (int)m->batch->res.size()) return invalid_arg("no such job in the last batch");
  const BatchJobResult &r = m->batch->res[job];
  if (scorer_calls) *scorer_calls = r.calls;
  if (poses_evaluated) *poses_evaluated = r.evaluated;
  if (super_steps) *super_steps = r.steps;
  if (on_device_chain) *on_device_chain = r.on_chain ? 1 : 0;
  return SLAMHIP_OK;
}

#ifdef SLAMHIP_TESTING
int slamhip_matcher_debug_trace_cap(slamhip_matcher *m, int cap) {
  if (!m || cap < 0) return invalid_arg("bad trace cap");
  m->debug_trace_cap = cap;
  return SLAMHIP_OK;
}
#endif

int slamhip_matcher_stats(slamhip_matcher *m, long long *scorer_calls, long long *poses_evaluated,
                          long long *launches) {
  if (!m) return invalid_arg("null matcher");
  if (scorer_calls) *scorer_calls = m->job.scorer_calls;
  if (poses_evaluated) *poses_evaluated = m->job.poses_evaluated;
  if (launches) *launches = m->job.launches;
  return SLAMHIP_OK;
}

int slamhip_matcher_process_raw_scan(slamhip_matcher *m, int map_id, const slamhip_raw_scan *scan, const double init_pose[3],
                                     double out_delta[3], double *out_prob, int *kept_n) {
  if (!m || !scan || !init_pose || !out_delta || !out_prob) return invalid_arg("null argument");
  int kept = 0;
  const int rc = slamhip_scan_filter_upload(m->ctx, map_id, scan->n, scan->range, scan->angle, scan->is_occ, scan->factor,
                                            scan->trig_mode, scan->a_min, scan->a_max, scan->a_inc, init_pose, scan->skip_rate,
                                            scan->max_range, scan->bounded, scan->weighting, &kept, nullptr);
  if (kept_n) *kept_n = kept;
  if (rc) return rc;
  if (kept == 0) {
    out_delta[0] = out_delta[1] = out_delta[2] = 0.0;
    *out_prob = std::numeric_limits<double>::quiet_NaN();
    return SLAMHIP_OK;
  }
  return slamhip_matcher_process_scan(m, map_id, init_pose, out_delta, out_prob);
}

int slamhip_matcher_tail_stats(slamhip_matcher *m, long long *calls_closed_form) {
  if (!m || !calls_closed_form) return invalid_arg("null argument");
  *calls_closed_form = m->tail_calls;
  return SLAMHIP_OK;
}

int slamhip_matcher_chain_stats(slamhip_matcher *m, long long *kernels_launched, long long *steps_rescored) {
  if (!m) return invalid_arg("null matcher");
  if (kernels_launched) *kernels_launched = m->chain_launched;
  if (steps_rescored) *steps_rescored = m->chain_rescored;
  return SLAMHIP_OK;
}

#ifdef SLAMHIP_TESTING
int slamhip_matcher_debug_fail_next(slamhip_matcher *m, int n) {
  if (!m || n < 0) return invalid_arg("bad count");
  m->debug_fail_next = n;
  return SLAMHIP_OK;
}
int slamhip_matcher_debug_resident_mute(slamhip_matcher *m, int slot_plus_1) {
  if (!m) return invalid_arg("null matcher");
  m->debug_resident_mute = slot_plus_1;
  return SLAMHIP_OK;
}
int slamhip_map_debug_nbr_masks(slamhip_ctx *ctx, int map_id, int *valid, long long *mismatches) {
  if (!ctx || map_id < 0 || map_id >= (int)ctx->maps.size() || !ctx->maps[map_id].bound) return invalid_arg("unknown map id");
  DeviceMap &dm = ctx->maps[map_id];
  if (valid) *valid = dm.nbr_ok ? 1 : 0;
  if (mismatches) *mismatches = 0;
  if (!dm.nbr_ok || !mismatches) return SLAMHIP_OK;
  SLAMHIP_CHECK(hipSetDevice(ctx->device));
  DeviceBuf<unsigned long long> d_count;
  unsigned long long h_count = 0;
  SLAMHIP_CHECK(d_count.alloc(1));
  SLAMHIP_CHECK(hipMemsetAsync(d_count.get(), 0, sizeof(unsigned long long), ctx->stream));
  SLAMHIP_CHECK(launch_nbr_check(dm.d_payload, dm.width, dm.height, dm.pitch, dm.nbr_th, d_count.get(), ctx->stream));
  SLAMHIP_CHECK(hipMemcpyAsync(&h_count, d_count.get(), sizeof(h_count), hipMemcpyDeviceToHost, ctx->stream));
  SLAMHIP_CHECK(hipStreamSynchronize(ctx->stream));
  *mismatches = (long long)h_count;
  return SLAMHIP_OK;
}
int slamhip_map_debug_prob_plane(slamhip_ctx *ctx, int map_id, int *valid, long long *mismatches) {
  if (!ctx || map_id < 0 || map_id >= (int)ctx->maps.size() || !ctx->maps[map_id].bound) return invalid_arg("unknown map id");
  DeviceMap &dm = ctx->maps[map_id];
  if (valid) *valid = dm.prob_ok ? 1 : 0;
  if (mismatches) *mismatches = 0;
  if (!dm.prob_ok || !mismatches) return SLAMHIP_OK;
  DeviceBuf<unsigned long long> d_count;
  unsigned long long h_count = 0;
  SLAMHIP_CHECK(d_count.alloc(1));
  SLAMHIP_CHECK(hipMemsetAsync(d_count.get(), 0, sizeof(unsigned long long), ctx->stream));
  SLAMHIP_CHECK(launch_prob_check(dm.cell_model, dm.d_payload, dm.d_prob, dm.width, dm.height, dm.pitch, d_count.get(), ctx->stream));
  SLAMHIP_CHECK(hipMemcpyAsync(&h_count, d_count.get(), sizeof(h_count), hipMemcpyDeviceToHost, ctx->stream));
  SLAMHIP_CHECK(hipStreamSynchronize(ctx->stream));
  *mismatches = (long long)h_count;
  return SLAMHIP_OK;
}
#endif

int slamhip_matcher_resident_stats(slamhip_matcher *m, long long *matches, long long *gave_up) {
  if (!m) return invalid_arg("null matcher");
  if (matches) *matches = m->resident.matches;
  if (gave_up) *gave_up = m->resident.gave_up;
  return SLAMHIP_OK;
}

int slamhip_matcher_timing(slamhip_matcher *m, double *build_us, double *stage_us, double *score_us,
                           double *replay_us) {
  if (!m) return invalid_arg("null matcher");
  if (build_us) *build_us = m->job.t_build_us;
  if (stage_us) *stage_us = m->t_stage_us;
  if (score_us) *score_us = m->t_score_us;
  if (replay_us) *replay_us = m->job.t_replay_us;
  return SLAMHIP_OK;
}

int slamhip_matcher_process_scan(slamhip_matcher *m, int map_id, const double init_pose[3],
                                 double out_delta[3], double *out_prob) {
  if (!m || !init_pose || !out_delta || !out_prob) return invalid_arg("null argument");
  slamhip_ctx *ctx = m->ctx;
  SLAMHIP_CHECK(hipSetDevice(ctx->device));
#ifdef SLAMHIP_TESTING
  if (m->debug_fail_next > 0) {
    --m->debug_fail_next;
    set_error("injected failure (slamhip_matcher_debug_fail_next)");
    return SLAMHIP_ERR_HIP;
  }
#endif
  bool force_exact = false;
  if (chain_eligible(m)) {
    const int crc = chain_process_scan(m, map_id, init_pose, out_delta, out_prob, hc_resident_asked(m));
    if (crc == kChainUnsettled) force_exact = true;
    else if (crc != kChainNeedsHost) return crc;
  }
  if (!force_exact && mc_chain_eligible(m)) {
    const int crc = mc_chain_process_scan(m, map_id, init_pose, out_delta, out_prob);
    if (crc != kChainNeedsHost) return crc;
  }
  if (!force_exact && bf_device_eligible(m)) {
    const int crc = bf_device_process_scan(m, map_id, init_pose, out_delta, out_prob);
    if (crc != kChainNeedsHost) return crc;
  }
  const bool gm_cfg = m->cfg.oope == SLAMHIP_OOPE_GMAPPING;
  const bool gm_exact_cfg = gm_cfg && (m->cfg.sum_order == SLAMHIP_SUM_SEQUENTIAL || m->cfg.pose_trig == SLAMHIP_POSE_TRIG_RAW_EXACT);
  const bool gm_checked = gm_cfg && !gm_exact_cfg && tie_check_default(m);
  std::unique_ptr<PoseEnumerator> pe_at_start;
  if (gm_checked && !force_exact) pe_at_start = m->pe->clone();
  const GmCarry carry_at_start{ctx->gm_cx, ctx->gm_cy, ctx->gm_prob};
  struct BufferingObserver {
    const slamhip_observer *to;
    bool hold;
    struct Ev {
      int kind;
      double p[3], s;
    };
    std::vector<Ev> held;
    static void test(void *u, const double p[3], double s) {
      auto *o = static_cast<BufferingObserver *>(u);
      if (o->hold) o->held.push_back(Ev{0, {p[0], p[1], p[2]}, s});
      else if (o->to->on_scan_test) o->to->on_scan_test(o->to->user, p, s);
    }
    static void update(void *u, const double p[3], double s) {
      auto *o = static_cast<BufferingObserver *>(u);
      if (o->hold) o->held.push_back(Ev{1, {p[0], p[1], p[2]}, s});
      else if (o->to->on_pose_update) o->to->on_pose_update(o->to->user, p, s);
    }
    void flush() {
      for (const Ev &e : held) {
        if (e.kind == 0 && to->on_scan_test) to->on_scan_test(to->user, e.p, e.s);
        if (e.kind == 1 && to->on_pose_update) to->on_pose_update(to->user, e.p, e.s);
      }
      held.clear();
    }
  } buffering{&m->obs, false, {}};
  const slamhip_observer obs_wrap{&buffering, &BufferingObserver::test, &BufferingObserver::update, nullptr};
  m->chain_rescored = 0;
  m->tail_calls = 0;
  m->t_stage_us = m->t_score_us = 0;
  for (;;) {
    const bool gm_exact = gm_exact_cfg || force_exact;
    const bool gm = gm_cfg && !gm_exact;
    slamhip_spe_cfg run_cfg = m->cfg;
    if (force_exact) {
      run_cfg.sum_order = SLAMHIP_SUM_SEQUENTIAL;
      run_cfg.pose_trig = scan_angles_known(ctx) ? SLAMHIP_POSE_TRIG_RAW_EXACT : SLAMHIP_POSE_TRIG_HOST;
    }
    const int budget = gm_exact ? 1 : (m->max_batch > 0 ? m->max_batch : 256);
    int rc = ensure_pose_capacity(ctx, budget + 2);
    if (rc) return rc;
    (void)tie_check_default(m);
    const bool checked = m->tie_check == 1 && !gm_cfg && m->cfg.sum_order == SLAMHIP_SUM_TREE256 && ctx->low_latency &&
                         !ctx->stage_poses;
    GmCarry carry;
    carry.cx = ctx->gm_cx;
    carry.cy = ctx->gm_cy;
    carry.prob = ctx->gm_prob;
    MatchJob &job = m->job;
    buffering.hold = gm && gm_checked && pe_at_start != nullptr;
    job.start(m->pe.get(), Pose{init_pose[0], init_pose[1], init_pose[2]}, gm, m->has_obs ? &obs_wrap : nullptr,
              carry, m->p_accept0);
    bool redo = false;
    while (!job.done) {
      const int n = job.plan(budget, ctx->h_poses);
      if (n == 0) break;
      const double t0 = MatchJob::now_us();
      unsigned seq = 0;
      ctx->want_fprints = checked;
      rc = score_staged(ctx, map_id, &run_cfg, n, nullptr, 0, &seq);
      ctx->want_fprints = false;
      if (rc) return rc;
      m->pe->idle_work();
      rc = score_wait(ctx, seq);
      if (rc) return rc;
      m->t_score_us += MatchJob::now_us() - t0;
      if (gm && gm_checked && pe_at_start && job.gm_unsettled(ctx->h_scores, ctx->h_gm_info, ctx)) {
        redo = true;
        break;
      }
      if (checked && job.ambiguous(ctx->h_scores, ctx->h_fprints)) {
        m->keep_scores.assign(ctx->h_scores, ctx->h_scores + n);
        m->keep_fprints.assign(ctx->h_fprints, ctx->h_fprints + n);
        ctx->h_poses[3 * n] = job.best.x;
        ctx->h_poses[3 * n + 1] = job.best.y;
        ctx->h_poses[3 * n + 2] = job.best.theta;
        slamhip_spe_cfg seq_cfg = m->cfg;
        seq_cfg.sum_order = SLAMHIP_SUM_SEQUENTIAL;
        rc = score_staged(ctx, map_id, &seq_cfg, n + 1, nullptr, 0, &seq);
        if (rc) return rc;
        rc = score_wait(ctx, seq);
        if (rc) return rc;
        ++m->chain_rescored;
        m->rescored_poses += n + 1;
        rc = job.consume(m->keep_scores.data(), ctx->h_gm_info, ctx, m->keep_fprints.data(), ctx->h_scores, ctx->h_scores[n]);
      } else {
        rc = job.consume(ctx->h_scores, ctx->h_gm_info, ctx, checked ? ctx->h_fprints : nullptr);
      }
      if (rc) return rc;
    }
    if (redo) {
      m->pe->assign(*pe_at_start);
      pe_at_start.reset();
      ctx->gm_cx = carry_at_start.cx;
      ctx->gm_cy = carry_at_start.cy;
      ctx->gm_prob = carry_at_start.prob;
      buffering.held.clear();
      force_exact = true;
      continue;
    }
    buffering.flush();
    if (force_exact) ++m->chain_rescored;
    if (gm) {
      ctx->gm_cx = job.carry.cx;
      ctx->gm_cy = job.carry.cy;
      ctx->gm_prob = job.carry.prob;
    }
    job.delta(out_delta);
    *out_prob = job.best_prob;
    if (m->has_obs && m->obs.on_matching_end) m->obs.on_matching_end(m->obs.user, out_delta, job.best_prob);
    return SLAMHIP_OK;
  }
}

}
```

### slam-constructor_amd/csrc/score_kernels.hip

```cpp


#include <algorithm>

#include "gm_score_device.h"
#include "kernel_pick.h"
#include "score_device.h"

namespace slamhip {

static constexpr int kBlock = 256;
static constexpr int kMaxPosesPerBlock = 16;

__global__ void k_publish(unsigned *flag, unsigned seq) {
  __hip_atomic_store(flag, seq, __ATOMIC_RELEASE, __HIP_MEMORY_SCOPE_SYSTEM);
}

__global__ void k_stall(long long ticks) {
  const long long t0 = wall_clock64();
  while (wall_clock64() - t0 < ticks) __builtin_amdgcn_s_sleep(64);
}
hipError_t launch_stall(int ms, hipStream_t stream) {
  hipLaunchKernelGGL(k_stall, dim3(1), dim3(1), 0, stream, (long long)ms * 100000ll);
  return hipGetLastError();
}

hipError_t launch_publish(unsigned *flag, unsigned seq, hipStream_t stream) {
  hipLaunchKernelGGL(k_publish, dim3(1), dim3(1), 0, stream, flag, seq);
  return hipGetLastError();
}

__global__ __launch_bounds__(256) void k_scan_pull(const double2 *__restrict__ src, double2 *__restrict__ dst, int n2,
                                                   unsigned *counter, unsigned *h_flag, unsigned seq) {
  const int i = blockIdx.x * 256 + threadIdx.x;
  if (i < n2) dst[i] = src[i];
  __syncthreads();
  if (threadIdx.x == 0) {
    const unsigned before = __hip_atomic_fetch_add(counter, 1u, __ATOMIC_RELAXED, __HIP_MEMORY_SCOPE_AGENT);
    if (before + 1u == gridDim.x) {
      __hip_atomic_store(counter, 0u, __ATOMIC_RELAXED, __HIP_MEMORY_SCOPE_AGENT);
      __hip_atomic_store(h_flag, seq, __ATOMIC_RELAXED, __HIP_MEMORY_SCOPE_SYSTEM);
    }
  }
}

hipError_t launch_scan_pull(const double *h_src, double *d_dst, size_t n_doubles, unsigned *counter, unsigned *h_flag,
                            unsigned seq, hipStream_t stream) {
  const int n2 = (int)((n_doubles + 1) / 2);
  hipLaunchKernelGGL(k_scan_pull, dim3((n2 + 255) / 256), dim3(256), 0, stream,
                     reinterpret_cast<const double2 *>(h_src), reinterpret_cast<double2 *>(d_dst), n2, counter, h_flag,
                     seq);
  return hipGetLastError();
}

__global__ __launch_bounds__(256) void k_scan_assemble(ScanAssembleArgs a, unsigned *counter, unsigned *h_flag, unsigned seq) {
  const int q = blockIdx.x * 256 + threadIdx.x;
  if (q < (int)a.stride) {
    double r = 0.0, c = 0.0, s = 0.0, w = 0.0, f = 0.0;
    if (q < a.n) {
      r = a.h_range[q];
      const int i = a.h_kept ? a.h_kept[q] : q;
      c = a.tab_cos[i];
      s = a.tab_sin[i];
      w = a.h_weight ? a.h_weight[q] : (a.tab_viny ? a.tab_viny[i] * sqrt(r) : a.w_even);
      f = a.h_factor ? a.h_factor[q] : 1.0;
    }
    a.dst[q] = r;
    a.dst[a.stride + q] = c;
    a.dst[2 * a.stride + q] = s;
    a.dst[3 * a.stride + q] = w;
    a.dst[4 * a.stride + q] = f;
  }
  __syncthreads();
  if (threadIdx.x == 0) {
    const unsigned before = __hip_atomic_fetch_add(counter, 1u, __ATOMIC_RELAXED, __HIP_MEMORY_SCOPE_AGENT);
    if (before + 1u == gridDim.x) {
      __hip_atomic_store(counter, 0u, __ATOMIC_RELAXED, __HIP_MEMORY_SCOPE_AGENT);
      __hip_atomic_store(h_flag, seq, __ATOMIC_RELAXED, __HIP_MEMORY_SCOPE_SYSTEM);
    }
  }
}

hipError_t launch_scan_assemble(const ScanAssembleArgs &a, unsigned *counter, unsigned *h_flag, unsigned seq,
                                hipStream_t stream) {
  hipLaunchKernelGGL(k_scan_assemble, dim3(((int)a.stride + 255) / 256), dim3(256), 0, stream, a, counter, h_flag, seq);
  return hipGetLastError();
}

__global__ __launch_bounds__(256) void k_block_pull(const uint4 *__restrict__ src, uint4 *__restrict__ dst, int n16) {
  const int i = blockIdx.x * 256 + threadIdx.x;
  if (i < n16) dst[i] = src[i];
}

hipError_t launch_block_pull(const void *h_src, void *d_dst, size_t bytes, hipStream_t stream) {
  const int n16 = (int)((bytes + 15) / 16);
  if (n16 <= 0) return hipSuccess;
  hipLaunchKernelGGL(k_block_pull, dim3((n16 + 255) / 256), dim3(256), 0, stream, reinterpret_cast<const uint4 *>(h_src),
                     reinterpret_cast<uint4 *>(d_dst), n16);
  return hipGetLastError();
}

template <int MODEL, int KB, bool WRITE_TERMS, bool FPRINT>
__global__ __launch_bounds__(kBlock) void k_score_point(ScoreArgs a) {
  __shared__ double s_pose[kMaxPosesPerBlock][4];
  __shared__ double s_part[kMaxPosesPerBlock][4];
  __shared__ unsigned long long s_hpart[FPRINT ? kMaxPosesPerBlock : 1][4];
  const int t = threadIdx.x;
  const int lane = t & 63, wave = t >> 6;
  const int n = a.scan.n;
  const int p0 = blockIdx.x * a.poses_per_block;
  const int npb = min(a.poses_per_block, a.n_poses - p0);

  double pose_x = 0.0, pose_y = 0.0, pose_th = 0.0, pose_sn = 0.0, pose_cs = 0.0;
  if (t < npb) {
    const int p = p0 + t;
    pose_th = a.poses[3 * p + 2];
    pose_x = a.poses[3 * p];
    pose_y = a.poses[3 * p + 1];
    if (a.pose_sc) {
      pose_sn = a.pose_sc[2 * p];
      pose_cs = a.pose_sc[2 * p + 1];
    }
  }

  constexpr int KR = KB > 0 ? KB : 1;
  double br[KR], bc[KR], bs[KR], bw[KR], bf[KR];
  if (KB > 0) {
#pragma unroll
    for (int k = 0; k < KR; ++k) {
      const int b = t + kBlock * k;
      const bool ok = b < n;
      br[k] = ok ? a.scan.range[b] : 0.0;
      bc[k] = ok ? a.scan.cos_a[b] : 0.0;
      bs[k] = ok ? a.scan.sin_a[b] : 0.0;
      bw[k] = ok ? a.scan.weight[b] : 0.0;
      bf[k] = ok ? a.scan.factor[b] : 0.0;
    }
  }
  if (t < npb) {
    if (!a.pose_sc) sincos(pose_th, &pose_sn, &pose_cs);
    s_pose[t][0] = pose_x;
    s_pose[t][1] = pose_y;
    s_pose[t][2] = pose_sn;
    s_pose[t][3] = pose_cs;
  }
  __syncthreads();

  const double scale = a.map.scale, inv_scale = a.map.inv_scale;
  const unsigned fk_lo = (2u * (unsigned)t + 1u) * 0x9E3779B1u, fk_hi = (2u * (unsigned)t + 1u) * 0x85EBCA6Bu;
  for (int j = 0; j < npb; ++j) {
    const double x = s_pose[j][0], y = s_pose[j][1], sn = s_pose[j][2], cs = s_pose[j][3];
    double acc = 0.0;
    unsigned long long h = 0ull;
    if (KB > 0) {
#pragma unroll
      for (int k = 0; k < KR; ++k) {
        const int b = t + kBlock * k;
        if (b < n) {
          const double c = cs * bc[k] - sn * bs[k];
          const double s = sn * bc[k] + cs * bs[k];
          const double wx = x + br[k] * c;
          const double wy = y + br[k] * s;
          const double pr = point_probability<MODEL>(a.map, a.oie, to_cell(wx, scale, inv_scale), to_cell(wy, scale, inv_scale));
          const double term = pr * bw[k] * bf[k];
          if (WRITE_TERMS) a.terms[(size_t)(p0 + j) * n + b] = term;
          acc = acc + term;
          if (FPRINT) h += term_fingerprint(term, fk_lo + (unsigned)k * (2u * kBlock * 0x9E3779B1u),
                                            fk_hi + (unsigned)k * (2u * kBlock * 0x85EBCA6Bu));
        }
      }
    } else {
      for (int b = t; b < n; b += kBlock) {
        const double ca = a.scan.cos_a[b], sa = a.scan.sin_a[b], r = a.scan.range[b];
        const double c = cs * ca - sn * sa;
        const double s = sn * ca + cs * sa;
        const double wx = x + r * c;
        const double wy = y + r * s;
        const double pr = point_probability<MODEL>(a.map, a.oie, to_cell(wx, scale, inv_scale), to_cell(wy, scale, inv_scale));
        const double term = pr * a.scan.weight[b] * a.scan.factor[b];
        if (WRITE_TERMS) a.terms[(size_t)(p0 + j) * n + b] = term;
        acc = acc + term;
        if (FPRINT) {
          const unsigned kq = (unsigned)(b / kBlock);
          h += term_fingerprint(term, fk_lo + kq * (2u * kBlock * 0x9E3779B1u), fk_hi + kq * (2u * kBlock * 0x85EBCA6Bu));
        }
      }
    }
    if (FPRINT) {
      wave_xor_sum_with(acc, h);
      if (lane == 0) s_hpart[j][wave] = h;
    } else {
      acc = wave_xor_sum(acc);
    }
    if (lane == 0) s_part[j][wave] = acc;
  }
  __syncthreads();
  if (t < npb) {
    const double total = (s_part[t][0] + s_part[t][1]) + (s_part[t][2] + s_part[t][3]);
    a.scores[p0 + t] = (a.scan.tot_w == 0.0) ? __builtin_nan("") : total / a.scan.tot_w;
    if (FPRINT) a.fprints[p0 + t] = s_hpart[t][0] + s_hpart[t][1] + s_hpart[t][2] + s_hpart[t][3];
  }
}

__global__ __launch_bounds__(64) void k_sum_sequential(const double *terms, int n_poses, int n,
                                                      double tot_w, double *scores) {
  const int p = blockIdx.x * 64 + threadIdx.x;
  if (p < n_poses) {
    const double *row = terms + (size_t)p * n;
    double acc = 0.0;
    for (int b = 0; b < n; ++b) acc = acc + row[b];
    scores[p] = (tot_w == 0.0) ? __builtin_nan("") : acc / tot_w;
  }
}

template <int KB, bool ONE>
__global__ __launch_bounds__(kBlock, (ONE && KB <= 5) ? 5 : 1) void k_score_gmapping(ScoreArgs a) {
  extern __shared__ double s_dyn[];
  __shared__ double s_pose[kMaxPosesPerBlock][4];
  __shared__ double s_part[kMaxPosesPerBlock][4];
  __shared__ double s_unknown[4];
  __shared__ int s_run0_len;
  const int t = threadIdx.x;
  const int lane = t & 63, wave = t >> 6;
  const int n = a.scan.n;
// ... 522 lines not shown
```

### slam-constructor_amd/csrc/slamhip_api.cpp

```cpp

#include <cmath>
#include <cstdio>
#include <cstdlib>
#include <cstring>
#include <limits>
#include <random>

#include "slamhip_internal.h"
#include "libm_exact.h"

namespace slamhip {

static thread_local std::string g_last_error;

void set_error(const std::string &msg) { g_last_error = msg; }

static thread_local std::string g_refusal;

hipError_t refuse_launch(const char *why) {
  g_refusal = why;
  return hipErrorInvalidValue;
}

int hip_fail(hipError_t e, const char *what) {
// ... 520 lines not shown
  if (lane && (!ctx->low_latency || ctx->stage_poses || !ctx->stream_b))
    return invalid("the second launch lane needs the zero-copy path and lane_fork()");
  DeviceMap tiled_view;
  DeviceMap *m = nullptr;
  if (tiled) {
    if (!cfg || cfg->oope != SLAMHIP_OOPE_GMAPPING || !ctx->low_latency)
      return invalid("per-particle maps are scored by the GMapping kernel on the zero-copy path only");
    tiled_device_map(tiled, &tiled_view);
    m = &tiled_view;
  } else {
    m = get_map(ctx, map_id);
  }
  if (!m) return invalid("unknown map id");
  int rc = check_cfg(*m, cfg);
  if (rc) return rc;
  if (n_poses <= 0) return SLAMHIP_OK;
  const bool host_trig = cfg->pose_trig == SLAMHIP_POSE_TRIG_HOST;
  if (cfg->pose_trig != SLAMHIP_POSE_TRIG_DEVICE && cfg->pose_trig != SLAMHIP_POSE_TRIG_HOST &&
      cfg->pose_trig != SLAMHIP_POSE_TRIG_RAW_EXACT)
    return invalid("unknown pose_trig");
  if (off < 0 || off + n_poses > ctx->pose_cap) return invalid("staging window outside the pose capacity");
  ctx->gm_exact_last = false;
  if (off != 0 && (!ctx->low_latency || ctx->stage_poses))
    return invalid("staging windows need the zero-copy path");
  if (host_trig) {
    for (int p = off; p < off + n_poses; ++p) {
      ::sincos(ctx->h_poses[3 * p + 2], &ctx->h_pose_sc[2 * p], &ctx->h_pose_sc[2 * p + 1]);
    }
  }
  const bool gm = cfg->oope == SLAMHIP_OOPE_GMAPPING;
  if (cfg->pose_trig == SLAMHIP_POSE_TRIG_RAW_EXACT || (gm && cfg->sum_order == SLAMHIP_SUM_SEQUENTIAL)) {
    if (lane) return invalid("the exact modes run on the context's first launch lane");
    return score_exact(ctx, *m, cfg, n_poses, tiled, off);
  }
  ScoreArgs a;
  if (ctx->low_latency) {
    const double *poses_src = ctx->h_poses + 3 * (size_t)off;
    const double *sc_src = host_trig ? ctx->h_pose_sc + 2 * (size_t)off : nullptr;
    if (ctx->stage_poses) {
      SLAMHIP_CHECK(hipMemcpyAsync(ctx->d_poses, ctx->h_poses, sizeof(double) * 3 * n_poses,
                                   hipMemcpyHostToDevice, ctx->stream));
      poses_src = ctx->d_poses;
      if (host_trig) {
        SLAMHIP_CHECK(hipMemcpyAsync(ctx->d_pose_sc, ctx->h_pose_sc, sizeof(double) * 2 * n_poses,
                                     hipMemcpyHostToDevice, ctx->stream));
        sc_src = ctx->d_pose_sc;
      }
    }
    rc = fill_args(ctx, *m, cfg, n_poses, poses_src, sc_src, ctx->h_scores + off, &a);
    if (rc) return rc;
    if (gm) a.gm_info = ctx->h_gm_info + off;
    if (ctx->want_fprints && cfg->oope != SLAMHIP_OOPE_GMAPPING && cfg->sum_order == SLAMHIP_SUM_TREE256)
      a.fprints = ctx->h_fprints + off;
    if (tiled) {
      a.tables = tiled->tables;
      a.pose_slot = ctx->h_pose_slot + off;
      a.table_stride = tiled->table_stride;
    }
    unsigned &counter = lane ? ctx->seq_b : ctx->seq;
    unsigned seq = ++counter;
    if (seq == 0) seq = ++counter;
    const hipStream_t stream = lane ? ctx->stream_b : ctx->stream;
    rc = launch_timed(ctx, a, *m, cfg, stream);
    if (rc) return rc;
    SLAMHIP_CHECK(launch_publish(lane ? ctx->h_done_flag_b : ctx->h_done_flag, seq, stream));
    if (async_seq) {
      *async_seq = seq;
      return SLAMHIP_OK;
    }
    return score_wait(ctx, seq, lane);
  }
  if (host_trig)
    SLAMHIP_CHECK(hipMemcpyAsync(ctx->d_pose_sc, ctx->h_pose_sc, sizeof(double) * 2 * n_poses,
                                 hipMemcpyHostToDevice, ctx->stream));
  SLAMHIP_CHECK(hipMemcpyAsync(ctx->d_poses, ctx->h_poses, sizeof(double) * 3 * n_poses,
                               hipMemcpyHostToDevice, ctx->stream));
  rc = fill_args(ctx, *m, cfg, n_poses, ctx->d_poses, host_trig ? ctx->d_pose_sc : nullptr,
                 ctx->d_scores, &a);
  if (rc) return rc;
  if (gm) a.gm_info = ctx->d_gm_info;
  rc = launch_timed(ctx, a, *m, cfg, ctx->stream);
  if (rc) return rc;
  SLAMHIP_CHECK(hipMemcpyAsync(ctx->h_scores, ctx->d_scores, sizeof(double) * n_poses,
                               hipMemcpyDeviceToHost, ctx->stream));
  if (gm)
    SLAMHIP_CHECK(hipMemcpyAsync(ctx->h_gm_info, ctx->d_gm_info, sizeof(GmPoseInfo) * n_poses,
                                 hipMemcpyDeviceToHost, ctx->stream));
  SLAMHIP_CHECK(hipStreamSynchronize(ctx->stream));
  return SLAMHIP_OK;
}

}

using namespace slamhip;

extern "C" {

const char *slamhip_last_error(void) { return g_last_error.c_str(); }

int slamhip_device_count(int *count) {
  if (!count) return invalid("null count");
  *count = 0;
  hipError_t e = hipGetDeviceCount(count);
  if (e != hipSuccess) {
    *count = 0;
    return hip_fail(e, "hipGetDeviceCount");
  }
  return SLAMHIP_OK;
}

int slamhip_ctx_create(int device, slamhip_ctx **out) {
  if (!out) return invalid("null out");
  *out = nullptr;
  int count = 0;
  hipError_t e = hipGetDeviceCount(&count);
  if (e != hipSuccess || count <= 0) {
    g_last_error = "no HIP device available (the scorer has no CPU fallback)";
    return SLAMHIP_ERR_NO_DEVICE;
  }
  if (device < 0 || device >= count) return invalid("device index out of range");
  SLAMHIP_CHECK(hipSetDevice(device));
  auto *ctx = new slamhip_ctx;
  ctx->device = device;
  e = hipStreamCreateWithFlags(&ctx->stream, hipStreamNonBlocking);
  if (e != hipSuccess) {
    delete ctx;
    return hip_fail(e, "hipStreamCreate");
  }
  e = hipHostMalloc(&ctx->h_done_flag, sizeof(unsigned), kPinned);
  if (e != hipSuccess) {
    hipStreamDestroy(ctx->stream);
    delete ctx;
    return hip_fail(e, "completion flag allocation");
  }
  *ctx->h_done_flag = 0;
  *out = ctx;
  return SLAMHIP_OK;
}

int slamhip_ctx_set_option(slamhip_ctx *ctx, int option, int value) {
  if (!ctx) return invalid("null argument");
  switch (option) {
    case SLAMHIP_OPT_LOW_LATENCY: ctx->low_latency = value != 0; break;
    case SLAMHIP_OPT_STAGE_POSES: ctx->stage_poses = value != 0; break;
    case SLAMHIP_OPT_FILTER_CHAINS: ctx->filter_chains = value != 0; break;
    case SLAMHIP_OPT_K6_PATH:
      if (value < 0 || value > 2) return invalid("SLAMHIP_OPT_K6_PATH: 0 (default), 1 (counting sort) or 2 (radix sort)");
      ctx->k6_path = value;
      break;
    case SLAMHIP_OPT_K6_BATCH_FAST: ctx->k6_batch_fast = value != 0; break;
    case SLAMHIP_OPT_K6_BATCH_KEY64: ctx->k6_batch_key64 = value != 0; break;
    case SLAMHIP_OPT_RESIDENT_CHAINS: ctx->resident_chains = value != 0; break;
    case SLAMHIP_OPT_TBM_PLANE: ctx->tbm_plane = value != 0; break;
    case SLAMHIP_OPT_INERT_TAIL:
      if (value < 0 || value > 2) return invalid("SLAMHIP_OPT_INERT_TAIL: 0 (off), 1 (identical poses) or 2 (default: certified poses too)");
      ctx->inert_tail = value;
      break;
    default: return invalid("unknown option");
  }
  return SLAMHIP_OK;
}

int slamhip_ctx_get_option(slamhip_ctx *ctx, int option, int *value) {
  if (!ctx || !value) return invalid("null argument");
  switch (option) {
    case SLAMHIP_OPT_LOW_LATENCY: *value = ctx->low_latency; break;
    case SLAMHIP_OPT_STAGE_POSES: *value = ctx->stage_poses; break;
    case SLAMHIP_OPT_FILTER_CHAINS: *value = ctx->filter_chains; break;
    case SLAMHIP_OPT_K6_PATH: *value = ctx->k6_path; break;
    case SLAMHIP_OPT_K6_BATCH_FAST: *value = ctx->k6_batch_fast; break;
    case SLAMHIP_OPT_K6_BATCH_KEY64: *value = ctx->k6_batch_key64; break;
    case SLAMHIP_OPT_RESIDENT_CHAINS: *value = ctx->resident_chains; break;
    case SLAMHIP_OPT_TBM_PLANE: *value = ctx->tbm_plane; break;
    case SLAMHIP_OPT_INERT_TAIL: *value = ctx->inert_tail; break;
    default: return invalid("unknown option");
  }
  return SLAMHIP_OK;
}

int slamhip_ctx_destroy(slamhip_ctx *ctx) {
  if (!ctx) return SLAMHIP_OK;
  hipSetDevice(ctx->device);
  hipStreamSynchronize(ctx->stream);
  pyramids_release(ctx);
  for (auto &m : ctx->maps) {
    if (m.d_payload) hipFree(m.d_payload);
    if (m.d_aux) hipFree(m.d_aux);
    if (m.d_prob) hipFree(m.d_prob);
  }
  if (ctx->d_scan) hipFree(ctx->d_scan);
  if (ctx->d_scan_tab) hipFree(ctx->d_scan_tab);
  if (ctx->d_scan_angle) hipFree(ctx->d_scan_angle);
  if (ctx->d_exact_trig) hipFree(ctx->d_exact_trig);
  if (ctx->d_gm_exact_cache) hipFree(ctx->d_gm_exact_cache);
  for (auto &sl : ctx->scan_slots)
    if (sl.d) hipFree(sl.d);
  for (int k = 0; k < 2; ++k) {
    if (ctx->h_scan_stage[k]) hipHostFree(ctx->h_scan_stage[k]);
    if (ctx->scan_stage_done[k]) hipEventDestroy(ctx->scan_stage_done[k]);
    if (k == 0 && ctx->h_scan_pulled) hipHostFree(ctx->h_scan_pulled);
    if (k == 0 && ctx->d_scan_pull_count) hipFree(ctx->d_scan_pull_count);
  }
  if (ctx->d_poses) hipFree(ctx->d_poses);
  if (ctx->d_scores) hipFree(ctx->d_scores);
  if (ctx->d_pose_sc) hipFree(ctx->d_pose_sc);
  if (ctx->d_gm_info) hipFree(ctx->d_gm_info);
  if (ctx->h_poses) hipHostFree(ctx->h_poses);
  if (ctx->h_scores) hipHostFree(ctx->h_scores);
  if (ctx->h_pose_sc) hipHostFree(ctx->h_pose_sc);
  if (ctx->h_gm_info) hipHostFree(ctx->h_gm_info);
  if (ctx->h_fprints) hipHostFree(ctx->h_fprints);
  if (ctx->h_pose_slot) hipHostFree(ctx->h_pose_slot);
  if (ctx->d_terms) hipFree(ctx->d_terms);
  if (ctx->d_dirty_xy) hipFree(ctx->d_dirty_xy);
  if (ctx->d_dirty_val) hipFree(ctx->d_dirty_val);
  for (hipEvent_t ev : ctx->ev_pool)
    if (ev) hipEventDestroy(ev);
  if (ctx->h_done_flag) hipHostFree(ctx->h_done_flag);
  if (ctx->stream_b) {
    hipStreamSynchronize(ctx->stream_b);
    hipStreamDestroy(ctx->stream_b);
    hipHostFree(ctx->h_done_flag_b);
    hipEventDestroy(ctx->ev_fork);
  }
  mu_release(ctx);
  render_release(ctx);
  scan_gen_release(ctx);
  shard_release(ctx);
  hipStreamDestroy(ctx->stream);
  delete ctx;
  return SLAMHIP_OK;
}

int slamhip_ctx_synchronize(slamhip_ctx *ctx) {
  if (!ctx) return invalid("null ctx");
  SLAMHIP_CHECK(hipStreamSynchronize(ctx->stream));
  return SLAMHIP_OK;
}

void *slamhip_ctx_stream(slamhip_ctx *ctx) { return ctx ? (void *)ctx->stream : nullptr; }

int slamhip_map_bind(slamhip_ctx *ctx, int map_id, int cell_model, int width, int height,
                     int origin_x, int origin_y, double scale, const double *unknown_payload) {
  if (!ctx) return invalid("null ctx");
  if (map_id < 0 || map_id > 4095) return invalid("map_id out of range [0, 4095]");
  if (cell_model < SLAMHIP_CELL_OCC || cell_model > SLAMHIP_CELL_CREDIBILIST)
    return invalid("unknown cell model");
  if (width <= 0 || height <= 0 || !(scale > 0) || !unknown_payload)
    return invalid("bad map geometry");
  SLAMHIP_CHECK(hipSetDevice(ctx->device));
  if ((int)ctx->maps.size() <= map_id) ctx->maps.resize(map_id + 1);
  DeviceMap old = ctx->maps[map_id];
  DeviceMap nm;
  nm.bound = true;
  nm.cell_model = cell_model;
  nm.width = width;
  nm.height = height;
  nm.pitch = (width + 15) & ~15;
  nm.origin_x = origin_x;
  nm.origin_y = origin_y;
  nm.scale = scale;
  const int sh = cell_stride_host(cell_model), cd = cell_doubles(cell_model);
  for (int k = 0; k < 4; ++k) nm.unknown[k] = k < sh ? unknown_payload[k] : 0.0;
  nm.bytes = (size_t)nm.pitch * height * cd * sizeof(double);
  SLAMHIP_CHECK(hipMalloc(&nm.d_payload, nm.bytes));
  SLAMHIP_CHECK(launch_fill_cells(nm.d_payload, (size_t)nm.pitch * height, cd, nm.unknown, ctx->stream));
  if (old.bound && old.cell_model == cell_model && old.d_payload) {
    const int dx = origin_x - old.origin_x, dy = origin_y - old.origin_y;
    const int sx0 = std::max(0, -dx), sy0 = std::max(0, -dy);
    const int sx1 = std::min(old.width, width - dx), sy1 = std::min(old.height, height - dy);
    if (sx1 > sx0 && sy1 > sy0) {
      const size_t cb = cd * sizeof(double);
      SLAMHIP_CHECK(hipMemcpy2DAsync(
          nm.d_payload + ((size_t)(sy0 + dy) * nm.pitch + (sx0 + dx)) * cd, nm.pitch * cb,
          old.d_payload + ((size_t)sy0 * old.pitch + sx0) * cd, old.pitch * cb,
          (size_t)(sx1 - sx0) * cb, sy1 - sy0, hipMemcpyDeviceToDevice, ctx->stream));
    }
  }
  if (old.bound && old.cell_model == cell_model && old.d_aux && old.aux_stride) {
    const size_t ab = (size_t)nm.pitch * height * old.aux_stride * sizeof(double);
    SLAMHIP_CHECK(hipMalloc(&nm.d_aux, ab));
    SLAMHIP_CHECK(hipMemsetAsync(nm.d_aux, 0, ab, ctx->stream));
    nm.aux_stride = old.aux_stride;
    const int dx = origin_x - old.origin_x, dy = origin_y - old.origin_y;
    const int sx0 = std::max(0, -dx), sy0 = std::max(0, -dy);
    const int sx1 = std::min(old.width, width - dx), sy1 = std::min(old.height, height - dy);
    if (sx1 > sx0 && sy1 > sy0) {
      const size_t cb = old.aux_stride * sizeof(double);
      SLAMHIP_CHECK(hipMemcpy2DAsync(
          nm.d_aux + ((size_t)(sy0 + dy) * nm.pitch + (sx0 + dx)) * old.aux_stride, nm.pitch * cb,
          old.d_aux + ((size_t)sy0 * old.pitch + sx0) * old.aux_stride, old.pitch * cb,
          (size_t)(sx1 - sx0) * cb, sy1 - sy0, hipMemcpyDeviceToDevice, ctx->stream));
    }
  }
  SLAMHIP_CHECK(hipStreamSynchronize(ctx->stream));
  if (old.d_payload) hipFree(old.d_payload);
  if (old.d_aux) hipFree(old.d_aux);
  if (old.d_prob) hipFree(old.d_prob);
  if (old.bound && old.cell_model == cell_model) {
    nm.auto_grow = old.auto_grow;
    nm.grown = old.grown;
  }
  ctx->maps[map_id] = nm;
  return SLAMHIP_OK;
}

int slamhip_map_set_auto_grow(slamhip_ctx *ctx, int map_id, int on) {
  DeviceMap *m = get_map(ctx, map_id);
  if (!m) return invalid("unknown map id");
  m->auto_grow = on != 0;
  return SLAMHIP_OK;
}

int slamhip_map_set_deferred(slamhip_ctx *ctx, int on) {
  if (!ctx) return invalid("null context");
  SLAMHIP_CHECK(hipSetDevice(ctx->device));
  if (!on) {
    long long nu = 0;
    const int rc = slamhip_map_drain(ctx, &nu);
    if (rc) return rc;
  }
  mu_set_deferred(ctx, on != 0);
  return SLAMHIP_OK;
}

int slamhip_map_drain(slamhip_ctx *ctx, long long *n_updates) {
  if (!ctx) return invalid("null context");
// ... 295 lines not shown
}

int slamhip_beam_trig_raw(int n, const double *angle, double *cos_out, double *sin_out) {
  if (n < 0 || !angle || !cos_out || !sin_out) return invalid("bad arguments");
  for (int i = 0; i < n; ++i) ::sincos(angle[i], &sin_out[i], &cos_out[i]);
  return SLAMHIP_OK;
}

int slamhip_beam_trig_cached(int n, const double *angle, double a_min, double a_max, double a_inc,
                             double *cos_out, double *sin_out) {
  if (n < 0 || !angle || !cos_out || !sin_out || !(a_inc > 0)) return invalid("bad arguments");
  struct Table {
    double a_min = 0, a_max = 0, a_inc = 0;
    std::vector<double> ts, tc;
  };
  static thread_local Table tab;
  if (tab.ts.empty() || tab.a_min != a_min || tab.a_max != a_max || tab.a_inc != a_inc) {
    tab.ts.clear();
    tab.tc.clear();
    for (double a = a_min; a < a_max; a += a_inc) {
      double sv, cv;
      ::sincos(a, &sv, &cv);
      tab.ts.push_back(sv);
      tab.tc.push_back(cv);
    }
    tab.a_min = a_min;
    tab.a_max = a_max;
    tab.a_inc = a_inc;
  }
  const std::vector<double> &ts = tab.ts, &tc = tab.tc;
  for (int i = 0; i < n; ++i) {
    const int idx = (int)std::round((angle[i] - a_min) / a_inc);
    if (idx < 0 || idx >= (int)ts.size()) return invalid("scan angle outside the trig table");
    cos_out[i] = tc[idx];
    sin_out[i] = ts[idx];
  }
  return SLAMHIP_OK;
}

int slamhip_filter_scan(int n, const double *range, const double *angle, const int *is_occ,
                        int trig_mode, double a_min, double a_delta, int table_n,
                        const double *tab_sin, const double *tab_cos, const double pose[3],
                        unsigned skip_rate, double max_range, int bounded, int width, int height,
                        int origin_x, int origin_y, double scale, int *kept_idx, int *kept_n) {
  if (n < 0 || !range || !angle || !pose || !kept_idx || !kept_n) return invalid("bad arguments");
  if (trig_mode == SLAMHIP_TRIG_CACHED && (!tab_sin || !tab_cos || table_n <= 0))
    return invalid("cached trig mode needs the table");
  constexpr double eps = std::numeric_limits<double>::epsilon();
  double sb, cb;
  ::sincos(pose[2], &sb, &cb);
  int kept = 0;
  for (int i = 0; i < n; ++i) {
    if (skip_rate && (unsigned(i) % skip_rate)) continue;
    double c, s;
    if (trig_mode == SLAMHIP_TRIG_CACHED) {
      const int idx = (int)std::round((angle[i] - a_min) / a_delta);
      if (idx < 0 || idx >= table_n) return invalid("scan angle outside the trig table");
      c = cb * tab_cos[idx] - sb * tab_sin[idx];
      s = sb * tab_cos[idx] + cb * tab_sin[idx];
    } else {
      ::sincos(pose[2] + angle[i], &s, &c);
    }
    const double wx = pose[0] + range[i] * c, wy = pose[1] + range[i] * s;
    const int cx = (int)std::floor(wx / scale), cy = (int)std::floor(wy / scale);
    bool has_cell = true;
    if (bounded) {
      const int ix = cx + origin_x, iy = cy + origin_y;
      has_cell = 0 <= ix && ix < width && 0 <= iy && iy < height;
    }
    const bool too_far = (0.0 < max_range + eps) && (max_range < range[i] + eps);
    if ((is_occ && !is_occ[i]) || !has_cell || too_far) continue;
    kept_idx[kept++] = i;
  }
  *kept_n = kept;
  return SLAMHIP_OK;
}

int slamhip_scan_weights(int kind, int n, const double *range, const double *angle, double *out) {
  if (n < 0 || !range || !angle || !out) return invalid("bad arguments");
  if (kind == 0) {
    const double w = 1.0 / n;
    for (int i = 0; i < n; ++i) out[i] = w;
    return SLAMHIP_OK;
  }
  if (kind == 1) {
    for (int i = 0; i < n; ++i) {
      double sv, cv;
      ::sincos(angle[i], &sv, &cv);
      const double ac = std::abs(cv);
      double w = std::abs(sv) + ac;
      if (0.9 < ac) w = 3;
      else if (0.8 < ac) w = 2;
      out[i] = w * std::sqrt(range[i]);
    }
    return SLAMHIP_OK;
  }
  if (kind == 2) {
    constexpr int NB = 20;
    unsigned hist[NB] = {0};
    std::vector<double> dirs(n > 0 ? n : 1, 0.0);
    const double step = (180 * M_PI / 180) / NB;
    for (int i = 1; i < n; ++i) {
      double s1, c1, s0, c0;
      ::sincos(angle[i], &s1, &c1);
      ::sincos(angle[i - 1], &s0, &c0);
      const double d_x = range[i] * c1 - range[i - 1] * c0;
      const double d_y = range[i] * s1 - range[i - 1] * s0;
      double a = 0;
      if (d_y != 0) {
        a = std::acos(d_x / std::sqrt(d_x * d_x + d_y * d_y));
        if (d_y < 0 && d_x != 0) a = M_PI - a;
      }
      const size_t bin = (size_t)std::floor(a / step);
      if (bin >= NB) return invalid("angle histogram bin out of range (reference asserts here)");
      hist[bin]++;
      dirs[i] = a;
    }
    for (int i = 0; i < n; ++i) {
      const unsigned v = i == 0 ? (unsigned)n : hist[(size_t)std::floor(dirs[i] / step)];
      out[i] = 1.0 / v;
    }
    return SLAMHIP_OK;
  }
  return invalid("unknown weighting kind");
}

static int scan_tables_upload(slamhip_ctx *ctx) {
  const slamhip_ctx::ScanPrep &sp = ctx->scan_prep;
  const int n = (int)sp.cos_a.size();
  SLAMHIP_CHECK(hipSetDevice(ctx->device));
  if (n > ctx->scan_tab_cap) {
    SLAMHIP_CHECK(hipStreamSynchronize(ctx->stream));
    if (ctx->d_scan_tab) hipFree(ctx->d_scan_tab);
    ctx->d_scan_tab = nullptr;
    ctx->scan_tab_cap = 0;
    int cap = 2048;
    while (cap < n) cap *= 2;
    SLAMHIP_CHECK(hipMalloc(&ctx->d_scan_tab, sizeof(double) * 3 * cap));
    ctx->scan_tab_cap = cap;
  }
  const size_t cap = (size_t)ctx->scan_tab_cap, bytes = sizeof(double) * n;
  SLAMHIP_CHECK(hipMemcpyAsync(ctx->d_scan_tab, sp.cos_a.data(), bytes, hipMemcpyHostToDevice, ctx->stream));
  SLAMHIP_CHECK(hipMemcpyAsync(ctx->d_scan_tab + cap, sp.sin_a.data(), bytes, hipMemcpyHostToDevice, ctx->stream));
  SLAMHIP_CHECK(hipMemcpyAsync(ctx->d_scan_tab + 2 * cap, sp.viny_f.data(), bytes, hipMemcpyHostToDevice, ctx->stream));
  SLAMHIP_CHECK(hipStreamSynchronize(ctx->stream));
  ++ctx->scan_tab_uploads;
  return SLAMHIP_OK;
}

int slamhip_scan_filter_upload(slamhip_ctx *ctx, int map_id, int n, const double *range, const double *angle,
                               const int *is_occ, const double *factor, int trig_mode, double a_min, double a_max,
                               double a_inc, const double pose[3], unsigned skip_rate, double max_range, int bounded,
                               int weighting, int *kept_n, int *kept_idx) {
  if (!ctx || n <= 0 || !range || !angle || !pose) return invalid("bad arguments");
  if (weighting < 0 || weighting > 2) return invalid("unknown weighting kind");
  DeviceMap *m = get_map(ctx, map_id);
  if (bounded && !m) return invalid("unknown map id");
  slamhip_ctx::ScanPrep &sp = ctx->scan_prep;
  const bool same = (int)sp.angle.size() == n && sp.trig_mode == trig_mode && sp.a_min == a_min && sp.a_max == a_max &&
                    sp.a_inc == a_inc && std::memcmp(sp.angle.data(), angle, sizeof(double) * n) == 0;
  if (!same) {
    scan_angles_materialise(ctx);
    sp.angle.assign(angle, angle + n);
    sp.trig_mode = trig_mode;
    sp.a_min = a_min;
    sp.a_max = a_max;
    sp.a_inc = a_inc;
    sp.cos_a.resize(n);
    sp.sin_a.resize(n);
    int rc = trig_mode == SLAMHIP_TRIG_CACHED
                 ? slamhip_beam_trig_cached(n, angle, a_min, a_max, a_inc, sp.cos_a.data(), sp.sin_a.data())
                 : slamhip_beam_trig_raw(n, angle, sp.cos_a.data(), sp.sin_a.data());
    if (rc) {
      sp.angle.clear();
      return rc;
    }
    sp.viny_f.resize(n);
    for (int i = 0; i < n; ++i) {
      double sv, cv;
      ::sincos(angle[i], &sv, &cv);
      const double ac = std::abs(cv);
      double w = std::abs(sv) + ac;
      if (0.9 < ac) w = 3;
      else if (0.8 < ac) w = 2;
      sp.viny_f[i] = w;
    }
    rc = scan_tables_upload(ctx);
    if (rc) {
      sp.angle.clear();
      return rc;
    }
  }
  constexpr double eps = std::numeric_limits<double>::epsilon();
  std::vector<int> &kept = sp.kept_next;
  kept.clear();
  const bool cut = 0.0 < max_range + eps;
  double sb = 0, cb = 1;
  if (bounded) ::sincos(pose[2], &sb, &cb);
  for (int i = 0; i < n; ++i) {
    if (skip_rate && (unsigned(i) % skip_rate)) continue;
    if (is_occ && !is_occ[i]) continue;
    const bool too_far = cut && (max_range < range[i] + eps);
    if (too_far) continue;
    if (bounded) {
      double c, s;
      if (trig_mode == SLAMHIP_TRIG_CACHED) {
        c = cb * sp.cos_a[i] - sb * sp.sin_a[i];
        s = sb * sp.cos_a[i] + cb * sp.sin_a[i];
      } else {
        ::sincos(pose[2] + angle[i], &s, &c);
      }
      const double wx = pose[0] + range[i] * c, wy = pose[1] + range[i] * s;
      const int ix = (int)std::floor(wx / m->scale) + m->origin_x, iy = (int)std::floor(wy / m->scale) + m->origin_y;
      if (!(0 <= ix && ix < m->width && 0 <= iy && iy < m->height)) continue;
    }
    kept.push_back(i);
  }
  const int k = (int)kept.size();
  if (kept_n) *kept_n = k;
  if (kept_idx) std::memcpy(kept_idx, kept.data(), sizeof(int) * k);
  if (k == 0) {
    ctx->scan_n = 0;
    ctx->scan_angle_lazy = false;
    return SLAMHIP_OK;
  }
  double *st = nullptr;
  size_t c = 0;
  int rc = scan_stage_acquire(ctx, k, &st, &c);
  if (rc) return rc;
  ScanAssembleArgs as{};
  double *r_ = st;
  as.h_range = r_;
  if (k == n) {
    std::memcpy(r_, range, sizeof(double) * k);
  } else {
    int *k_ = reinterpret_cast<int *>(st + c);
    for (int q = 0; q < k; ++q) r_[q] = range[kept[q]];
    std::memcpy(k_, kept.data(), sizeof(int) * k);
    as.h_kept = k_;
  }
  if (weighting == 0) {
    as.w_even = 1.0 / k;
    ctx->h_weight.assign(k, as.w_even);
  } else if (weighting == 1) {
    ctx->h_weight.resize(k);
    for (int q = 0; q < k; ++q) ctx->h_weight[q] = sp.viny_f[kept[q]] * std::sqrt(r_[q]);
    as.tab_viny = ctx->d_scan_tab + 2 * (size_t)ctx->scan_tab_cap;
  } else {
    sp.a.resize(k);
    sp.r.assign(r_, r_ + k);
    sp.w.resize(k);
    for (int q = 0; q < k; ++q) sp.a[q] = angle[kept[q]];
    rc = slamhip_scan_weights(2, k, sp.r.data(), sp.a.data(), sp.w.data());
    if (rc) return rc;
    double *w_ = st + 3 * c;
    std::memcpy(w_, sp.w.data(), sizeof(double) * k);
    ctx->h_weight.assign(w_, w_ + k);
    as.h_weight = w_;
  }
  if (factor) {
    double *f_ = st + 2 * c;
    for (int q = 0; q < k; ++q) f_[q] = factor[kept[q]];
    ctx->h_factor.assign(f_, f_ + k);
    as.h_factor = f_;
  } else {
    ctx->h_factor.assign(k, 1.0);
  }
  as.tab_cos = ctx->d_scan_tab;
  as.tab_sin = ctx->d_scan_tab + (size_t)ctx->scan_tab_cap;
  as.dst = ctx->d_scan;
  as.stride = c;
  as.n = k;
  int turn = 0;
  const double tot_w = weighting == 0 ? scan_total_weight_even(k, as.w_even) : scan_total_weight(ctx->h_weight.data(), k);
  const unsigned seq = scan_stage_turnover(ctx, k, c, tot_w, &turn);
  SLAMHIP_CHECK(launch_scan_assemble(as, ctx->d_scan_pull_count, ctx->h_scan_pulled + turn, seq, ctx->stream));
  rc = scan_stage_fork(ctx, turn);
  if (rc) return rc;
  sp.kept.swap(kept);
  ctx->scan_angle_lazy = true;
  return SLAMHIP_OK;
}

int slamhip_scan_set_angles(slamhip_ctx *ctx, int n, const double *angle) {
  if (!ctx || !angle) return invalid("bad arguments");
  if (n != ctx->scan_n || n <= 0) return invalid("slamhip_scan_set_angles: n is not the current scan's point count");
  ctx->h_scan_angle.assign(angle, angle + n);
  ctx->scan_angle_lazy = false;
  ctx->scan_angle_on_device = false;
  return SLAMHIP_OK;
}

int slamhip_scan_table_uploads(slamhip_ctx *ctx, long long *uploads) {
  if (!ctx || !uploads) return invalid("null argument");
  *uploads = ctx->scan_tab_uploads;
  return SLAMHIP_OK;
}

int slamhip_scan_download(slamhip_ctx *ctx, int cap, double *out5, int *n) {
  if (!ctx || !n || cap < 0 || (cap > 0 && !out5)) return invalid("bad arguments");
  *n = ctx->scan_n;
  if (cap == 0 || ctx->scan_n <= 0 || !ctx->scan_ptr) return SLAMHIP_OK;
  if (cap < ctx->scan_n) return invalid("slamhip_scan_download: room for fewer points than the current scan has");
  SLAMHIP_CHECK(hipSetDevice(ctx->device));
  SLAMHIP_CHECK(hipMemcpy2DAsync(out5, sizeof(double) * cap, ctx->scan_ptr, sizeof(double) * ctx->scan_stride,
                                 sizeof(double) * ctx->scan_n, 5, hipMemcpyDeviceToHost, ctx->stream));
  SLAMHIP_CHECK(hipStreamSynchronize(ctx->stream));
  return SLAMHIP_OK;
}

int slamhip_libm_variant(int *variant) {
  if (!variant) return invalid("null variant");
  *variant = libm_variant();
  return SLAMHIP_OK;
}

int slamhip_libm_eval(slamhip_ctx *ctx, int variant, int fn, int n, const double *x, double *out) {
  if (!ctx || n < 0 || (n > 0 && (!x || !out)) || fn < 0 || fn > 2 || (variant != 0 && variant != 1))
    return invalid("bad arguments");
  if (n == 0) return SLAMHIP_OK;
  SLAMHIP_CHECK(hipSetDevice(ctx->device));
  double *d = nullptr;
  SLAMHIP_CHECK(hipMalloc(&d, sizeof(double) * 2 * (size_t)n));
  hipError_t e = hipMemcpyAsync(d, x, sizeof(double) * n, hipMemcpyHostToDevice, ctx->stream);
  if (e == hipSuccess) e = launch_libm_eval(variant == 1, fn, d, d + n, n, ctx->stream);
  if (e == hipSuccess) e = hipMemcpyAsync(out, d + n, sizeof(double) * n, hipMemcpyDeviceToHost, ctx->stream);
  if (e == hipSuccess) e = hipStreamSynchronize(ctx->stream);
  hipFree(d);
  if (e != hipSuccess) return hip_fail(e, "slamhip_libm_eval");
  return SLAMHIP_OK;
}

int slamhip_omqe_quality(int kind, int n, const double *range, const double *angle, double *out) {
  if (n < 0 || !range || !angle || !out) return invalid("bad arguments");
  if (kind == 0) {
    for (int i = 0; i < n; ++i) out[i] = 1.0;
    return SLAMHIP_OK;
  }
  if (kind == 1) return slamhip_scan_weights(2, n, range, angle, out);
  return invalid("unknown observation quality estimator");
}

int slamhip_score_poses(slamhip_ctx *ctx, int map_id, const slamhip_spe_cfg *cfg, int n_poses,
                        const double *poses_xyt, double *scores_out) {
  if (!ctx) return invalid("null ctx");
  if (n_poses < 0 || (n_poses > 0 && (!poses_xyt || !scores_out))) return invalid("bad pose batch");
  if (n_poses == 0) return SLAMHIP_OK;
  SLAMHIP_CHECK(hipSetDevice(ctx->device));
  int rc = ensure_pose_capacity(ctx, n_poses);
  if (rc) return rc;
  std::memcpy(ctx->h_poses, poses_xyt, sizeof(double) * 3 * n_poses);
  rc = score_staged(ctx, map_id, cfg, n_poses);
  if (rc) return rc;
  if (cfg->oope == SLAMHIP_OOPE_GMAPPING) gm_carry_fixup(ctx, n_poses);
  std::memcpy(scores_out, ctx->h_scores, sizeof(double) * n_poses);
  return SLAMHIP_OK;
}

int slamhip_score_poses_device(slamhip_ctx *ctx, int map_id, const slamhip_spe_cfg *cfg,
                               int n_poses, const double *d_poses_xyt, double *d_scores_out) {
  DeviceMap *m = get_map(ctx, map_id);
  if (!m) return invalid("unknown map id");
  int rc = check_cfg(*m, cfg);
  if (rc) return rc;
  if (n_poses <= 0) return SLAMHIP_OK;
  if (!d_poses_xyt || !d_scores_out) return invalid("null device buffers");
  if (cfg->pose_trig != SLAMHIP_POSE_TRIG_DEVICE)
    return invalid("device-resident poses use device sincos (pose_trig = DEVICE): the host-trig and exact modes take host poses");
  if (cfg->oope == SLAMHIP_OOPE_GMAPPING && cfg->sum_order == SLAMHIP_SUM_SEQUENTIAL)
    return invalid("the GMapping OOPE's beam-order mode keeps the reference's cache in call order: slamhip_score_poses");
  SLAMHIP_CHECK(hipSetDevice(ctx->device));
  ScoreArgs a;
  rc = fill_args(ctx, *m, cfg, n_poses, d_poses_xyt, nullptr, d_scores_out, &a);
  if (rc) return rc;
  if (cfg->oope == SLAMHIP_OOPE_GMAPPING) {
    rc = ensure_pose_capacity(ctx, n_poses);
    if (rc) return rc;
    a.gm_info = nullptr;
  }
  return launch_timed(ctx, a, *m, cfg, ctx->stream);
}

int slamhip_gm_cache_reset(slamhip_ctx *ctx) {
  if (!ctx) return invalid("null ctx");
  ctx->gm_cx = ctx->gm_cy = 0;
  ctx->gm_prob = -1.0;
  return SLAMHIP_OK;
}

int slamhip_gm_cache_get(slamhip_ctx *ctx, int *cell_xy, double *prob) {
  if (!ctx || !cell_xy || !prob) return invalid("bad arguments");
  cell_xy[0] = ctx->gm_cx;
  cell_xy[1] = ctx->gm_cy;
  *prob = ctx->gm_prob;
  return SLAMHIP_OK;
}

int slamhip_gm_cache_set(slamhip_ctx *ctx, const int *cell_xy, double prob) {
  if (!ctx || !cell_xy) return invalid("bad arguments");
  ctx->gm_cx = cell_xy[0];
  ctx->gm_cy = cell_xy[1];
  ctx->gm_prob = prob;
  return SLAMHIP_OK;
}

int slamhip_profile_enable(slamhip_ctx *ctx, int on) {
  if (!ctx) return invalid("null ctx");
  ctx->profile = on != 0;
  return SLAMHIP_OK;
}

int slamhip_profile_read(slamhip_ctx *ctx, double *kernel_ms_total, long long *launches,
                         long long *units, int reset) {
  if (!ctx) return invalid("null ctx");
  int rc = profile_resolve(ctx);
  if (rc) return rc;
  if (kernel_ms_total) *kernel_ms_total = ctx->prof_ms;
  if (launches) *launches = ctx->prof_launches;
  if (units) *units = ctx->prof_units;
  if (reset) {
    ctx->prof_ms = 0;
    ctx->prof_launches = 0;
    ctx->prof_units = 0;
  }
  return SLAMHIP_OK;
}

int slamhip_profile_read_map_update(slamhip_ctx *ctx, double *ms_total, long long *calls, long long *records,
                                    int reset) {
  if (!ctx) return invalid("null ctx");
  int rc = profile_resolve(ctx);
  if (rc) return rc;
  if (ms_total) *ms_total = ctx->prof_k6_ms;
  if (calls) *calls = ctx->prof_k6_calls;
  if (records) *records = ctx->prof_k6_records;
// ... 56 lines not shown
```

### slam-constructor_amd/csrc/slamhip_internal.h

```cpp
#pragma once

#ifdef SLAMHIP_TESTING
#define SLAMHIP_STAMPS_ON(expr) (expr)
#else
#define SLAMHIP_STAMPS_ON(expr) false
#endif


#include <hip/hip_runtime.h>

#include <cstdint>
#include <string>
#include <vector>

#include "slamhip.h"

namespace slamhip {

struct MapView {
  const double *payload;
  int width, height, pitch;
  int origin_x, origin_y;
  double scale, inv_scale;
  double unknown[4];
// ... 84 lines not shown
  const double *poses;
  const double *pose_sc;
  double *scores;
  int n_poses;
  int poses_per_block;
  int oie;
  double area[4];
  GmParams gm;
  GmPoseInfo *gm_info;
  double *terms;
  unsigned long long *fprints;
  const int *tables;
  const int *pose_slot;
  int table_stride;
  int xcd_blocks;
  int model_override;
};

constexpr int kTileShift = 7;
constexpr int kTileSide = 1 << kTileShift;
constexpr int kTileMask = kTileSide - 1;
constexpr int kTileCells = kTileSide * kTileSide;
constexpr int kTileStateWords = kTileCells / 16;
__host__ __device__ inline unsigned mu_settle_class(double c0, long long unknown_bits, int fresh_ok) {
  long long bits;
  __builtin_memcpy(&bits, &c0, 8);
  return bits == 0ll ? 1u : ((c0 == 0.0 || (fresh_ok && bits == unknown_bits)) ? 3u : 0u);
}

inline int cell_doubles(int model) { return model == SLAMHIP_CELL_OCC ? 1 : 4; }
inline int cell_stride_host(int model) {
  return cell_is_belief(model) ? 4 : (model == SLAMHIP_CELL_GMAPPING ? 3 : 1);
}

hipError_t launch_score(const ScoreArgs &a, int cell_model, int oope, int sum_order,
                        hipStream_t stream, hipEvent_t ev_start = nullptr,
                        hipEvent_t ev_stop = nullptr);
hipError_t launch_publish(unsigned *flag, unsigned seq, hipStream_t stream);
hipError_t launch_exact_beam_trig(bool fma, const double *poses, int n_poses, const double *d_angle, int n, size_t stride,
                                  double *d_cos, double *d_sin, double *d_identity_sc, hipStream_t stream);
hipError_t launch_score_gmapping_exact(bool fma, const ScoreArgs &a, const double *d_angle, int raw_trig, void *d_cache,
                                       hipStream_t stream);
hipError_t launch_libm_eval(bool fma, int fn, const double *d_x, double *d_out, int n, hipStream_t stream);
int libm_variant();
hipError_t launch_stall(int ms, hipStream_t stream);
hipError_t launch_block_pull(const void *h_src, void *d_dst, size_t bytes, hipStream_t stream);
hipError_t launch_scan_pull(const double *h_src, double *d_dst, size_t n_doubles, unsigned *counter, unsigned *h_flag,
                            unsigned seq, hipStream_t stream);
struct ScanAssembleArgs {
  const double *h_range;
  const int *h_kept;
  const double *h_factor, *h_weight;
  const double *tab_cos, *tab_sin, *tab_viny;
  double *dst;
  size_t stride;
  int n;
  double w_even;
};
hipError_t launch_scan_assemble(const ScanAssembleArgs &a, unsigned *counter, unsigned *h_flag, unsigned seq,
                                hipStream_t stream);
hipError_t launch_scatter_cells(double *payload, int pitch, int cell_dbl, int stride_host, int n,
                                const int *d_coords, const double *d_vals, hipStream_t stream);
hipError_t launch_repack_window(double *dst, int dst_pitch, int cell_dbl, const double *src,
                                int stride_host, int x0, int y0, int w, int h, hipStream_t stream);
hipError_t launch_fill_cells(double *dst, size_t n_cells, int cell_dbl, const double *unknown4,
                             hipStream_t stream);

struct DeviceMap {
  bool bound = false;
  int cell_model = 0;
  int width = 0, height = 0, pitch = 0;
  int origin_x = 0, origin_y = 0;
  double scale = 1.0;
  double unknown[4] = {0, 0, 0, 0};
  double *d_payload = nullptr;
  size_t bytes = 0;
  double *d_aux = nullptr;
  int aux_stride = 0;
  bool auto_grow = false;
  long grown = 0;
  bool nbr_ok = false;
  double nbr_th = 0.0;
  double nbr_other_th = 0.0;
  double *d_prob = nullptr;
  bool prob_ok = false;
};
hipError_t launch_prob_build(int model, const double *payload, double *prob, int width, int height, int pitch, int x0, int y0, int w, int h,
                             hipStream_t stream);
hipError_t launch_prob_cells(int model, const double *payload, double *prob, int width, int height, int pitch, int n, const int *d_coords,
                             hipStream_t stream);
hipError_t launch_prob_check(int model, const double *payload, const double *prob, int width, int height, int pitch,
                             unsigned long long *d_count, hipStream_t stream);
hipError_t launch_nbr_build(double *payload, int width, int height, int pitch, double th, int x0, int y0, int w, int h,
                            hipStream_t stream);
hipError_t launch_nbr_cells(double *payload, int width, int height, int pitch, double th, int n, const int *d_coords,
                            hipStream_t stream);
hipError_t launch_nbr_check(const double *payload, int width, int height, int pitch, double th, unsigned long long *d_count,
                            hipStream_t stream);

void mu_allow_scan_reuse(slamhip_ctx *ctx, bool on);
bool mu_set_deferred(slamhip_ctx *ctx, bool on);
int mu_drain(slamhip_ctx *ctx, long long *n_updates, int *err);
void mu_release(slamhip_ctx *ctx);
void shard_release(slamhip_ctx *ctx);
void render_release(slamhip_ctx *ctx);
void scan_gen_release(slamhip_ctx *ctx);
void pyramids_release(slamhip_ctx *ctx);
void set_error(const std::string &msg);
int hip_fail(hipError_t e, const char *what);
hipError_t refuse_launch(const char *why);

}

#define SLAMHIP_CHECK(expr)                                        \
  do {                                                             \
    hipError_t _e = (expr);                                        \
    if (_e != hipSuccess) return slamhip::hip_fail(_e, #expr);     \
  } while (0)

struct slamhip_ctx {
  int device = 0;
  hipStream_t stream = nullptr;
  std::vector<slamhip::DeviceMap> maps;
  double *d_scan = nullptr;
  double *h_scan_stage[2] = {nullptr, nullptr};
  hipEvent_t scan_stage_done[2] = {nullptr, nullptr};
  int scan_stage_turn = 0;
  unsigned scan_pull_seq[2] = {0, 0}, scan_pull_next = 0;
  unsigned *h_scan_pulled = nullptr;
  unsigned *d_scan_pull_count = nullptr;
  int scan_cap = 0, scan_n = 0;
  double scan_tot_w = 0.0;
  const double *scan_ptr = nullptr;
  size_t scan_stride = 0;
  struct ScanSlot {
    double *d = nullptr;
    int cap = 0, n = 0;
    double tot_w = 0.0;
    std::vector<double> w, f;
  };
  std::vector<ScanSlot> scan_slots;
  struct ScanPrep {
    std::vector<double> angle, cos_a, sin_a, viny_f;
    int trig_mode = -1;
    double a_min = 0, a_max = 0, a_inc = 0;
    std::vector<double> r, a, c, s, w, f;
    std::vector<int> kept;
    std::vector<int> kept_next;
  } scan_prep;
  double *d_scan_tab = nullptr;
  int scan_tab_cap = 0;
  long long scan_tab_uploads = 0;
  std::vector<double> h_weight, h_factor;
  std::vector<double> h_scan_angle;
  bool scan_angle_lazy = false;
  double *d_scan_angle = nullptr;
  int scan_angle_cap = 0;
  bool scan_angle_on_device = false;
  double *d_exact_trig = nullptr;
  size_t exact_trig_cap = 0;
  void *d_gm_exact_cache = nullptr;
  bool gm_exact_last = false;
  double *d_poses = nullptr, *d_scores = nullptr, *d_pose_sc = nullptr;
  double *h_poses = nullptr, *h_scores = nullptr, *h_pose_sc = nullptr;
  slamhip::GmPoseInfo *d_gm_info = nullptr, *h_gm_info = nullptr;
  unsigned long long *h_fprints = nullptr;
  bool want_fprints = false;
  int *h_pose_slot = nullptr;
  int pose_cap = 0;
  double *d_terms = nullptr;
  size_t terms_cap = 0;
  int *d_dirty_xy = nullptr;
  double *d_dirty_val = nullptr;
  int dirty_cap = 0;
  int gm_cx = 0, gm_cy = 0;
  double gm_prob = -1.0;
  unsigned *h_done_flag = nullptr;
  unsigned seq = 0;
  hipStream_t stream_b = nullptr;
  unsigned *h_done_flag_b = nullptr;
  unsigned seq_b = 0;
  hipEvent_t ev_fork = nullptr;
  void *shard = nullptr;
  void *mu_scratch = nullptr, *mu_bscratch = nullptr;
  unsigned char *d_render = nullptr;
  size_t render_cap = 0;
  void *d_scan_gen = nullptr;
  size_t scan_gen_cap = 0;
  std::vector<double> scan_gen_stage;
  std::vector<void *> pyramids;
  bool low_latency = true;
  bool stage_poses = false;
  bool filter_chains = true, k6_batch_fast = true, k6_batch_key64 = false, resident_chains = true, tbm_plane = true;
  int inert_tail = 2;
  int k6_path = 0;
  bool profile = false;
  std::vector<hipEvent_t> ev_pool;
  size_t ev_used = 0;
  std::vector<char> ev_kind;
  double prof_ms = 0.0;
  long long prof_launches = 0, prof_units = 0;
  double prof_k6_ms = 0.0;
  long long prof_k6_calls = 0, prof_k6_records = 0;
};

namespace slamhip {
inline bool scan_angles_known(const slamhip_ctx *ctx) {
  return ctx->scan_angle_lazy || (int)ctx->h_scan_angle.size() == ctx->scan_n;
}
void scan_angles_materialise(slamhip_ctx *ctx);
struct TiledTarget {
  const double *pool;
  const int *tables;
  int table_stride, tiles_x, width, height, origin_x, origin_y;
  double scale;
  double unknown[4];
  int nbr_ok;
  double nbr_th;
};
int ensure_pose_capacity(slamhip_ctx *ctx, int n);
int score_staged(slamhip_ctx *ctx, int map_id, const slamhip_spe_cfg *cfg, int n_poses,
                 const TiledTarget *tiled = nullptr, int off = 0, unsigned *async_seq = nullptr, int lane = 0);
int score_wait(slamhip_ctx *ctx, unsigned seq, int lane = 0);
int lane_fork(slamhip_ctx *ctx);
int score_views(slamhip_ctx *ctx, int map_id, const slamhip_spe_cfg *cfg, MapView *map, ScanView *scan,
                int *cell_model, const TiledTarget *tiled = nullptr, int *oie_eff = nullptr);
int profile_event_pair(slamhip_ctx *ctx, hipEvent_t *e0, hipEvent_t *e1, int kind = 0);
struct ProfilePairGuard {
  hipEvent_t e0 = nullptr, e1 = nullptr;
  hipStream_t stream = nullptr;
  bool closed = true;
  int open(slamhip_ctx *ctx, hipStream_t st, int kind);
  int close();
  bool on() const { return e1 != nullptr; }
  ~ProfilePairGuard() {
    if (!closed && e1) (void)hipEventRecord(e1, stream);
  }
};

struct GmChainResult {
  double pose[3];
  double prob;
  long long calls, evaluated;
  int steps;
  int cx, cy;
  double cprob;
  GmPoseInfo first_info;
  double first_raw;
  int error;
};
struct GmMultiChain;
int gm_multi_chain_run(slamhip_ctx *ctx, GmMultiChain **scratch, int map_id, const slamhip_spe_cfg *cfg,
                       unsigned max_failed, double dt, double dr, int n, const double *inits, GmChainResult *out,
                       long long *kernels_launched, const TiledTarget *tiled = nullptr, const int *slots = nullptr);
void gm_multi_chain_free(GmMultiChain *s);
bool gm_multi_chain_fits_resident(slamhip_ctx *ctx, int n);
}
```

Before: 13.16 billion pose-candidates*beams/s.

## Fuse scan assembly prologue into the resident hill-climbing chain kernel

Scan filtering no longer launches the scan-assemble kernel straight away. It records a pending assembly, and when the lone resident hill-climbing chain can run it, that chain kernel builds the range, trig, weight and factor values itself from the raw filtered scan. Those values go into LDS and are written back to the scan buffer. This saves one kernel launch and a global round trip per scan on the filter-and-match path. In exchange it adds deferred-state bookkeeping, extra LDS for the weight and factor arrays (which may lower occupancy), and fallback paths that run the assembly eagerly when fusion is not possible.

```diff
diff --git a/include/slamhip.h b/include/slamhip.h
--- a/include/slamhip.h
+++ b/include/slamhip.h
@@ -57,6 +57,8 @@
   SLAMHIP_OPT_RESIDENT_CHAINS = 6,
   SLAMHIP_OPT_K6_BATCH_KEY64 = 5,
   SLAMHIP_OPT_TBM_PLANE = 7,
+  SLAMHIP_OPT_RAW_PROLOGUE = 9,
+  SLAMHIP_OPT_RAW_PROLOGUE_MATCHES = 10,
   SLAMHIP_OPT_INERT_TAIL = 8
 };
 int slamhip_ctx_set_option(slamhip_ctx *ctx, int option, int value);
diff --git a/slam-constructor_amd/__init__.py b/slam-constructor_amd/__init__.py
--- a/slam-constructor_amd/__init__.py
+++ b/slam-constructor_amd/__init__.py
@@ -17,7 +17,7 @@
 SUM_TREE256, SUM_SEQUENTIAL = 0, 1
 POSE_TRIG_DEVICE, POSE_TRIG_HOST, POSE_TRIG_RAW_EXACT = 0, 1, 2
 (OPT_LOW_LATENCY, OPT_STAGE_POSES, OPT_FILTER_CHAINS, OPT_K6_PATH, OPT_K6_BATCH_FAST, OPT_K6_BATCH_KEY64,
- OPT_RESIDENT_CHAINS, OPT_TBM_PLANE, OPT_INERT_TAIL) = range(9)
+ OPT_RESIDENT_CHAINS, OPT_TBM_PLANE, OPT_INERT_TAIL, OPT_RAW_PROLOGUE, OPT_RAW_PROLOGUE_MATCHES) = range(11)
 TRIG_RAW, TRIG_CACHED = 0, 1
 RENDER_OCCGRID, RENDER_PGM = 0, 1
 OCC_TBM_CONSISTENT, OCC_TBM_UNKNOWN_EVEN = 0, 1
diff --git a/slam-constructor_amd/csrc/hc_chain_device.h b/slam-constructor_amd/csrc/hc_chain_device.h
--- a/slam-constructor_amd/csrc/hc_chain_device.h
+++ b/slam-constructor_amd/csrc/hc_chain_device.h
@@ -102,6 +102,7 @@
   int oope;
   double area[4];
   int inert_tail;
+  ScanAssembleArgs raw;
 };
 
 hipError_t launch_hc_chain_step(const HcChainArgs &a, int cell_model, int k, int nt, hipStream_t stream,
@@ -110,7 +111,7 @@
                                     hipEvent_t ev_start = nullptr, hipEvent_t ev_stop = nullptr, int n_chains = 1);
 hipError_t hc_resident_capacity(int cell_model, HcResidentKey key, int n_beams, bool lds_consts, int *out_wgs,
                                 int *out_per_cu = nullptr);
-size_t hc_resident_lds_bytes(int nt, int n_beams, bool lds_consts, int max_inst, bool pair = false);
+size_t hc_resident_lds_bytes(int nt, int n_beams, int lds_consts, int max_inst, bool pair = false);
 hipError_t launch_hc_chain_resident_gm(const HcChainArgs &a, int nt, hipStream_t stream, hipEvent_t ev_start = nullptr,
                                        hipEvent_t ev_stop = nullptr, int n_chains = 1);
 hipError_t hc_resident_gm_capacity(int nt, int n_beams, int *out_wgs, int *out_per_cu = nullptr);
diff --git a/slam-constructor_amd/csrc/hc_resident.hip b/slam-constructor_amd/csrc/hc_resident.hip
--- a/slam-constructor_amd/csrc/hc_resident.hip
+++ b/slam-constructor_amd/csrc/hc_resident.hip
@@ -2,6 +2,7 @@
 
 #include "hc_chain_device.h"
 #include "hc_resident_device.h"
+#include "scan_assemble_device.h"
 #include "score_device.h"
 
 namespace slamhip {
@@ -39,8 +40,9 @@
 constexpr int kSelFirst = -2;
 constexpr int kSelStop = -3;
 
-template <int MODEL, int NT, bool SEQ, bool BATCH, int G, bool WIN = false, bool PAIR = false>
+template <int MODEL, int NT, bool SEQ, bool BATCH, int G, bool WIN = false, bool PAIR = false, bool RAW = false>
 __global__ __launch_bounds__(NT, 4) void k_hc_chain_resident(HcChainArgs a) {
+  static_assert(!RAW || (!SEQ && !BATCH && !WIN && !PAIR), "RAW: the lone 1-cell chain in the default sum order only");
   constexpr int H = PAIR ? 2 : 1;
   constexpr int NTH = NT / H;
   constexpr bool CERT = !WIN;
@@ -58,6 +60,7 @@
   __shared__ unsigned long long s_hpart[H][4];
   __shared__ double s_cert[2][16];
   __shared__ int s_cert_end;
+  const long long t_kernel_begin = SLAMHIP_STAMPS_ON(a.stamps != nullptr) ? (long long)wall_clock64() : 0ll;
   const int t = threadIdx.x, wave = t >> 6;
   const int half = PAIR ? (t >= NTH ? 1 : 0) : 0;
   const int tl = t - half * NTH, lwave = tl >> 6;
@@ -89,24 +92,47 @@
   const ScanView scan = load_view(scan_p);
   const int n = scan.n;
   double br = 0.0, bc = 0.0, bs = 0.0, bw = 0.0, bf = 0.0;
-  if (tl < n) {
+  if (!RAW && tl < n) {
     br = scan.range[tl];
     bc = scan.cos_a[tl];
     bs = scan.sin_a[tl];
     bw = scan.weight[tl];
     bf = scan.factor[tl];
   }
-  if (lwave == 1 && (t & 63) < kHcShapes && !init_slot && exists) {
+  const bool mine_here = lwave == 1 && (t & 63) < kHcShapes && !init_slot && exists;
+  constexpr int kMineQ = (int)(sizeof(HcInst) / 16);
+  uint4 mine_regs[kMineQ];
+  ScanPoint raw_more{0.0, 0.0, 0.0, 0.0, 0.0};
+  if constexpr (RAW) {
+    if (mine_here) {
+      const uint4 *src = reinterpret_cast<const uint4 *>(&a.shapes[t & 63].inst[inst_of_slot]);
+#pragma unroll
+      for (int q = 0; q < kMineQ; ++q) mine_regs[q] = src[q];
+    }
+    asm volatile("" ::: "memory");
+    if (tl < n) {
+      const ScanPoint p = scan_assemble_point(a.raw, tl);
+      br = p.range;
+      bc = p.cos_a;
+      bs = p.sin_a;
+      bw = p.weight;
+      bf = p.factor;
+    }
+    if (NTH + t < n) raw_more = scan_assemble_point(a.raw, NTH + t);
+    asm volatile("" ::: "memory");
+  }
+  if (mine_here) {
     const uint4 *src = reinterpret_cast<const uint4 *>(&a.shapes[t & 63].inst[inst_of_slot]);
     uint4 *dst = reinterpret_cast<uint4 *>(&s_mine[half][t & 63]);
 #pragma unroll
-    for (int q = 0; q < (int)(sizeof(HcInst) / 16); ++q) dst[q] = src[q];
-  }
-  const bool ldsc = !WIN && a.lds_consts != 0;
+    for (int q = 0; q < kMineQ; ++q) dst[q] = RAW ? mine_regs[q] : src[q];
+  }
+  const bool ldsc = RAW || (!WIN && a.lds_consts != 0);
   const int n_more = n > NTH ? n - NTH : 0;
   double *const my_term = s_term + (PAIR ? half * a.scan.n : 0);
   double *const s_r = s_term + (PAIR ? 2 * a.scan.n : n) - NTH, *const s_ca = s_r + n_more, *const s_sa = s_ca + n_more;
-  if (ldsc) {
+  double *const s_w = s_sa + n_more, *const s_f = s_w + n_more;
+  if (!RAW && ldsc) {
     for (int b = NTH + t; b < n; b += NT) {
       s_r[b] = scan.range[b];
       s_ca[b] = scan.cos_a[b];
@@ -121,6 +147,7 @@
   }
   const bool verify = a.verify != 0;
   const bool stamp = SLAMHIP_STAMPS_ON(a.stamps && slot == 1 && tl == 0 && blockIdx.y == 0);
+  if (stamp) a.stamps[6] = t_kernel_begin;
   HcGranule *const gran = &rc->gran[0][0];
   HcGranule *const gseq = &rc->seq[0][0];
   constexpr int kGranRow = kHcSlots + 7;
@@ -168,8 +195,41 @@
       s_cur_go[half] = go ? 1 : 0;
     }
   }
+  if constexpr (RAW) {
+    for (int b = NTH + t; b < n; b += NT) {
+      const ScanPoint p = b == NTH + t ? raw_more : scan_assemble_point(a.raw, b);
+      s_r[b] = p.range;
+      s_ca[b] = p.cos_a;
+      s_sa[b] = p.sin_a;
+      s_w[b] = p.weight;
+      s_f[b] = p.factor;
+    }
+  }
   __syncthreads();
 
+  auto write_scan_block = [&](int t, double *dst, int stride) __attribute__((always_inline)) {
+    for (int q = t; q < stride; q += NT) {
+      double r_ = 0.0, ca = 0.0, sa = 0.0, w = 0.0, f = 0.0;
+      if (q < NT && q < n) {
+        r_ = br;
+        ca = bc;
+        sa = bs;
+        w = bw;
+        f = bf;
+      } else if (q < n) {
+        r_ = s_r[q];
+        ca = s_ca[q];
+        sa = s_sa[q];
+        w = s_w[q];
+        f = s_f[q];
+      }
+      dst[q] = r_;
+      dst[stride + q] = ca;
+      dst[2 * stride + q] = sa;
+      dst[3 * stride + q] = w;
+      dst[4 * stride + q] = f;
+    }
+  };
   const int t_entry = t;
   for (int k = 0;; ++k) {
     const int pk = k & 1;
@@ -267,6 +327,9 @@
             __hip_atomic_store(ap->h_all_done, ap->epoch, __ATOMIC_RELEASE, __HIP_MEMORY_SCOPE_SYSTEM);
         }
       }
+      if constexpr (RAW) {
+        if (done && init_slot && k == 1) write_scan_block(t, ap->raw.dst, (int)ap->raw.stride);
+      }
       if (done) break;
     } else {
       if (sel == kSelRescore && init_slot) {
@@ -329,8 +392,8 @@
               r_ = ldsc ? s_r[bc_] : scan.range[bc_];
               ca = ldsc ? s_ca[bc_] : scan.cos_a[bc_];
               sa = ldsc ? s_sa[bc_] : scan.sin_a[bc_];
-              w_[j] = scan.weight[bc_];
-              f_[j] = scan.factor[bc_];
+              w_[j] = RAW ? s_w[bc_] : scan.weight[bc_];
+              f_[j] = RAW ? s_f[bc_] : scan.factor[bc_];
             }
             cell[j] = beam_cell<MODEL>(map, px, py, sn, cs, r_, ca, sa);
           }
@@ -433,6 +496,9 @@
       gran_store(&gran[pk * kGranRow + slot], cert_here ? cert_t : 0.0,
                  cert_here ? (unsigned long long)__double_as_longlong(cert_r) >> 16 : 0ull, tag);
       if (verify && mode) gran_store(&gseq[pk * kGranRow + slot], 0.0, 0ull, tag);
+    }
+    if constexpr (RAW) {
+      if (init_slot && k == 1) write_scan_block(t, ap->raw.dst, (int)ap->raw.stride);
     }
 
     if (wave != 0) {
@@ -706,13 +772,13 @@
   }
 }
 
-size_t hc_resident_tab_offset(int nt, int n_beams, bool lds_consts, bool pair) {
+size_t hc_resident_tab_offset(int nt, int n_beams, int lds_consts, bool pair) {
   const size_t n = (size_t)(n_beams > 0 ? n_beams : 1);
   const size_t nth = (size_t)(pair ? nt / 2 : nt);
   const size_t more = lds_consts && n > nth ? n - nth : 0;
-  return (pair ? 2 : 1) * n + 3 * more;
-}
-size_t hc_resident_lds_bytes(int nt, int n_beams, bool lds_consts, int max_inst, bool pair) {
+  return (pair ? 2 : 1) * n + (lds_consts > 1 ? 5 : 3) * more;
+}
+size_t hc_resident_lds_bytes(int nt, int n_beams, int lds_consts, int max_inst, bool pair) {
   return sizeof(double) * hc_resident_tab_offset(nt, n_beams, lds_consts, pair) +
          (pair ? sizeof(HcNextEntryT<2>) : sizeof(HcNextEntryT<1>)) * 7 * (size_t)max_inst;
 }
@@ -731,6 +797,9 @@
         if constexpr (NT == 512)
           if (key.batch && key.pair) return k_hc_chain_resident<M, 512, false, true, G, false, true>;
         if (key.batch) return k_hc_chain_resident<M, NT, false, true, G>;
+        if constexpr (G == 4)
+          if (key.raw) return k_hc_chain_resident<M, NT, false, false, 4, false, false, true>;
+        if (key.raw) return nullptr;
         return key.seq ? k_hc_chain_resident<M, NT, true, false, G> : k_hc_chain_resident<M, NT, false, false, G>;
       };
       if (g_v == 2) return sweep(int_c<2>{});
@@ -742,7 +811,8 @@
 }
 
 static HcResidentKey key_of(const HcChainArgs &a, int nt) {
-  return {nt, a.max_inst, a.seq != 0, a.jobs != nullptr, a.pair != 0, a.oope != SLAMHIP_OOPE_OBSTACLE};
+  return {nt, a.max_inst, a.seq != 0, a.jobs != nullptr, a.pair != 0, a.oope != SLAMHIP_OOPE_OBSTACLE,
+          a.raw.h_range != nullptr};
 }
 
 hipError_t launch_hc_chain_resident(const HcChainArgs &a_in, int cell_model, int nt, hipStream_t stream, hipEvent_t e0,
@@ -751,7 +821,8 @@
   HcChainArgs a = a_in;
   const HcResidentKey key = key_of(a, nt);
   const bool pair = key.batch && key.pair;
-  const bool ldsc = !key.window && a.lds_consts != 0;
+  const int ldsc = key.window ? 0 : (key.raw ? 2 : (a.lds_consts != 0 ? 1 : 0));
+  if (key.raw && a.raw.n != a.scan.n) return hipErrorInvalidValue;
   const int grid = pair ? 3 * a.max_inst + 1 : 6 * a.max_inst + 1;
   a.tab_offset = (int)hc_resident_tab_offset(nt, a.scan.n, ldsc, pair);
   return launch_kernel(hc_resident_kernel(cell_model, key), dim3(grid, n_chains), dim3(hc_nt_of(nt)),
@@ -762,7 +833,8 @@
                                 int *out_per_cu) {
   key.seq = false;
   return resident_capacity_of((const void *)hc_resident_kernel(cell_model, key), key.nt,
-                              hc_resident_lds_bytes(key.nt, n_beams, lds_consts, key.max_inst, key.batch && key.pair),
+                              hc_resident_lds_bytes(key.nt, n_beams, key.raw ? 2 : (lds_consts ? 1 : 0), key.max_inst,
+                                                    key.batch && key.pair),
                               2048 / key.nt , 6, out_wgs, out_per_cu);
 }
 
diff --git a/slam-constructor_amd/csrc/kernel_pick.h b/slam-constructor_amd/csrc/kernel_pick.h
--- a/slam-constructor_amd/csrc/kernel_pick.h
+++ b/slam-constructor_amd/csrc/kernel_pick.h
@@ -66,12 +66,14 @@
 struct HcResidentKey {
   int nt, max_inst;
   bool seq, batch, pair, window;
+  bool raw = false;
 };
 inline bool hc_resident_variant(const HcResidentKey &k, int *nt, int *g) {
   const int slots = 6 * k.max_inst + 1;
   *nt = hc_nt_of(k.nt);
   *g = k.window ? 4 : hc_gran_per_lane(slots);
   if (k.seq && k.batch) return false;
+  if (k.raw && (k.seq || k.batch || k.window || *g != 4)) return false;
   if (k.window) return !k.seq && !k.batch && slots <= 256;
   if (k.batch && k.pair) return k.nt == 512;
   return !(*nt == 1024 && *g == 7);
diff --git a/slam-constructor_amd/csrc/matchers.cpp b/slam-constructor_amd/csrc/matchers.cpp
--- a/slam-constructor_amd/csrc/matchers.cpp
+++ b/slam-constructor_amd/csrc/matchers.cpp
@@ -151,7 +151,7 @@
   long long chain_launched = 0;
   unsigned rctl_launches = 0;
   slamhip::ResidentPolicy resident;
-  enum class ResidentForm { Lone, Batch, Window, MonteCarlo, Pair };
+  enum class ResidentForm { Lone, Batch, Window, MonteCarlo, Pair, LoneRaw };
   struct ResidentCap {
     int cell_model, nt;
     ResidentForm form;
@@ -344,7 +344,8 @@
     SLAMHIP_CHECK(mc_resident_capacity(cell_model, nt, n_beams, lds_consts, &cap, &pc));
   } else {
     const bool pair = form == ResidentForm::Pair;
-    const HcResidentKey key{nt, max_inst, false, pair || form == ResidentForm::Batch, pair, form == ResidentForm::Window};
+    const HcResidentKey key{nt, max_inst, false, pair || form == ResidentForm::Batch, pair, form == ResidentForm::Window,
+                            form == ResidentForm::LoneRaw};
     SLAMHIP_CHECK(hc_resident_capacity(cell_model, key, n_beams, lds_consts, &cap, &pc));
   }
   if (cap < 0) cap = 0;
@@ -524,6 +525,10 @@
     SLAMHIP_CHECK(m->h_trace.alloc(m->trace_cap, kPinnedCoherent));
   }
   const bool win = is_window_oope(m->cfg.oope), gm = m->cfg.oope == SLAMHIP_OOPE_GMAPPING;
+  if (!resident || win || gm || m->cfg.sum_order == SLAMHIP_SUM_SEQUENTIAL || !ctx->raw_prologue) {
+    rc = scan_assemble_now(ctx);
+    if (rc) return rc;
+  }
   a.oie = oie_eff;
   a.oope = win ? m->cfg.oope : SLAMHIP_OOPE_OBSTACLE;
   for (int k = 0; k < 4; ++k) a.area[k] = m->cfg.area[k];
@@ -578,14 +583,34 @@
         }
         a.rctl = hc.d_rctl.get();
         a.rctl_gm = hc.d_rctl_gm.get();
+        if (ctx->scan_pending.active) {
+          bool fuse = false;
+          int nt_v = 0, g_v = 0;
+          if (a.lds_consts && hc_resident_variant(HcResidentKey{m->chain_nt, a.max_inst, false, false, false, false, true}, &nt_v, &g_v)) {
+            int cap_raw = 0;
+            r = resident_capacity(m, cell_model, m->chain_nt, ResidentForm::LoneRaw, a.scan.n, true, a.max_inst, &cap_raw);
+            if (r) return r;
+            fuse = grid <= cap_raw;
+          }
+          if (fuse) {
+            a.raw = ctx->scan_pending.as;
+          } else {
+            r = scan_assemble_now(ctx);
+            if (r) return r;
+          }
+        }
         *fits = true;
         return SLAMHIP_OK;
       },
       [&](hipEvent_t e0, hipEvent_t e1) {
-        return gm ? launch_hc_chain_resident_gm(a, m->chain_nt, ctx->stream, e0, e1)
-                  : launch_hc_chain_resident(a, cell_model, m->chain_nt, ctx->stream, e0, e1);
+        const hipError_t e = gm ? launch_hc_chain_resident_gm(a, m->chain_nt, ctx->stream, e0, e1)
+                                : launch_hc_chain_resident(a, cell_model, m->chain_nt, ctx->stream, e0, e1);
+        scan_record_finish(ctx);
+        return e;
       },
       [&](bool) -> int {
+        const int arc = scan_assemble_now(ctx);
+        if (arc) return arc;
         if (win) return kChainNeedsHost;
         a = a_chain;
         a.epoch = next_epoch(m->chain_epoch);
@@ -603,6 +628,10 @@
       },
       LoneChainText{"internal: the co-resident chain ended without publishing a result", "co-resident hill-climbing chain",
                     "hill-climbing chain did not end", "hill-climbing chain kernel"});
+  if (ctx->scan_pending.active) {
+    const int src = (rc == SLAMHIP_OK && h->error != 1) ? scan_fused_done(ctx) : scan_assemble_now(ctx);
+    if (!rc) rc = src;
+  }
   if (rc) return rc;
   m->chain_launched = launched;
   if (h->error == 1) {
@@ -1639,9 +1668,9 @@
                                      double out_delta[3], double *out_prob, int *kept_n) {
   if (!m || !scan || !init_pose || !out_delta || !out_prob) return invalid_arg("null argument");
   int kept = 0;
-  const int rc = slamhip_scan_filter_upload(m->ctx, map_id, scan->n, scan->range, scan->angle, scan->is_occ, scan->factor,
-                                            scan->trig_mode, scan->a_min, scan->a_max, scan->a_inc, init_pose, scan->skip_rate,
-                                            scan->max_range, scan->bounded, scan->weighting, &kept, nullptr);
+  int rc = scan_filter_stage(m->ctx, map_id, scan->n, scan->range, scan->angle, scan->is_occ, scan->factor, scan->trig_mode,
+                             scan->a_min, scan->a_max, scan->a_inc, init_pose, scan->skip_rate, scan->max_range,
+                             scan->bounded, scan->weighting, &kept, nullptr);
   if (kept_n) *kept_n = kept;
   if (rc) return rc;
   if (kept == 0) {
@@ -1649,7 +1678,9 @@
     *out_prob = std::numeric_limits<double>::quiet_NaN();
     return SLAMHIP_OK;
   }
-  return slamhip_matcher_process_scan(m, map_id, init_pose, out_delta, out_prob);
+  rc = slamhip_matcher_process_scan(m, map_id, init_pose, out_delta, out_prob);
+  const int arc = scan_assemble_now(m->ctx);
+  return rc ? rc : arc;
 }
 
 int slamhip_matcher_tail_stats(slamhip_matcher *m, long long *calls_closed_form) {
@@ -1745,6 +1776,10 @@
     const int crc = chain_process_scan(m, map_id, init_pose, out_delta, out_prob, hc_resident_asked(m));
     if (crc == kChainUnsettled) force_exact = true;
     else if (crc != kChainNeedsHost) return crc;
+  }
+  {
+    const int arc = scan_assemble_now(ctx);
+    if (arc) return arc;
   }
   if (!force_exact && mc_chain_eligible(m)) {
     const int crc = mc_chain_process_scan(m, map_id, init_pose, out_delta, out_prob);
diff --git a/slam-constructor_amd/csrc/scan_assemble_device.h b/slam-constructor_amd/csrc/scan_assemble_device.h
--- /dev/null
+++ b/slam-constructor_amd/csrc/scan_assemble_device.h
@@ -0,0 +1,24 @@
+#pragma once
+
+#include <hip/hip_runtime.h>
+
+#include "slamhip_internal.h"
+
+namespace slamhip {
+
+struct ScanPoint {
+  double range, cos_a, sin_a, weight, factor;
+};
+
+__device__ __forceinline__ ScanPoint scan_assemble_point(const ScanAssembleArgs &a, int q) {
+  ScanPoint p;
+  p.range = a.h_range[q];
+  const int i = a.h_kept ? a.h_kept[q] : q;
+  p.cos_a = a.tab_cos[i];
+  p.sin_a = a.tab_sin[i];
+  p.weight = a.h_weight ? a.h_weight[q] : (a.tab_viny ? a.tab_viny[i] * sqrt(p.range) : a.w_even);
+  p.factor = a.h_factor ? a.h_factor[q] : 1.0;
+  return p;
+}
+
+}
diff --git a/slam-constructor_amd/csrc/score_kernels.hip b/slam-constructor_amd/csrc/score_kernels.hip
--- a/slam-constructor_amd/csrc/score_kernels.hip
+++ b/slam-constructor_amd/csrc/score_kernels.hip
@@ -4,6 +4,7 @@
 
 #include "gm_score_device.h"
 #include "kernel_pick.h"
+#include "scan_assemble_device.h"
 #include "score_device.h"
 
 namespace slamhip {
@@ -55,20 +56,13 @@
 __global__ __launch_bounds__(256) void k_scan_assemble(ScanAssembleArgs a, unsigned *counter, unsigned *h_flag, unsigned seq) {
   const int q = blockIdx.x * 256 + threadIdx.x;
   if (q < (int)a.stride) {
-    double r = 0.0, c = 0.0, s = 0.0, w = 0.0, f = 0.0;
-    if (q < a.n) {
-      r = a.h_range[q];
-      const int i = a.h_kept ? a.h_kept[q] : q;
-      c = a.tab_cos[i];
-      s = a.tab_sin[i];
-      w = a.h_weight ? a.h_weight[q] : (a.tab_viny ? a.tab_viny[i] * sqrt(r) : a.w_even);
-      f = a.h_factor ? a.h_factor[q] : 1.0;
-    }
-    a.dst[q] = r;
-    a.dst[a.stride + q] = c;
-    a.dst[2 * a.stride + q] = s;
-    a.dst[3 * a.stride + q] = w;
-    a.dst[4 * a.stride + q] = f;
+    ScanPoint p{0.0, 0.0, 0.0, 0.0, 0.0};
+    if (q < a.n) p = scan_assemble_point(a, q);
+    a.dst[q] = p.range;
+    a.dst[a.stride + q] = p.cos_a;
+    a.dst[2 * a.stride + q] = p.sin_a;
+    a.dst[3 * a.stride + q] = p.weight;
+    a.dst[4 * a.stride + q] = p.factor;
   }
   __syncthreads();
   if (threadIdx.x == 0) {
diff --git a/slam-constructor_amd/csrc/slamhip_api.cpp b/slam-constructor_amd/csrc/slamhip_api.cpp
--- a/slam-constructor_amd/csrc/slamhip_api.cpp
+++ b/slam-constructor_amd/csrc/slamhip_api.cpp
@@ -696,6 +696,8 @@
     case SLAMHIP_OPT_K6_BATCH_KEY64: ctx->k6_batch_key64 = value != 0; break;
     case SLAMHIP_OPT_RESIDENT_CHAINS: ctx->resident_chains = value != 0; break;
     case SLAMHIP_OPT_TBM_PLANE: ctx->tbm_plane = value != 0; break;
+    case SLAMHIP_OPT_RAW_PROLOGUE: ctx->raw_prologue = value != 0; break;
+    case SLAMHIP_OPT_RAW_PROLOGUE_MATCHES: return invalid("SLAMHIP_OPT_RAW_PROLOGUE_MATCHES is read-only");
     case SLAMHIP_OPT_INERT_TAIL:
       if (value < 0 || value > 2) return invalid("SLAMHIP_OPT_INERT_TAIL: 0 (off), 1 (identical poses) or 2 (default: certified poses too)");
       ctx->inert_tail = value;
@@ -717,6 +719,8 @@
     case SLAMHIP_OPT_RESIDENT_CHAINS: *value = ctx->resident_chains; break;
     case SLAMHIP_OPT_TBM_PLANE: *value = ctx->tbm_plane; break;
     case SLAMHIP_OPT_INERT_TAIL: *value = ctx->inert_tail; break;
+    case SLAMHIP_OPT_RAW_PROLOGUE: *value = ctx->raw_prologue; break;
+    case SLAMHIP_OPT_RAW_PROLOGUE_MATCHES: *value = (int)(ctx->raw_prologue_matches & 0x7fffffff); break;
     default: return invalid("unknown option");
   }
   return SLAMHIP_OK;
@@ -1318,7 +1322,54 @@
                                const int *is_occ, const double *factor, int trig_mode, double a_min, double a_max,
                                double a_inc, const double pose[3], unsigned skip_rate, double max_range, int bounded,
                                int weighting, int *kept_n, int *kept_idx) {
+  const int rc = slamhip::scan_filter_stage(ctx, map_id, n, range, angle, is_occ, factor, trig_mode, a_min, a_max, a_inc,
+                                            pose, skip_rate, max_range, bounded, weighting, kept_n, kept_idx);
+  return rc ? rc : slamhip::scan_assemble_now(ctx);
+}
+
+}
+
+namespace slamhip {
+
+void scan_record_finish(slamhip_ctx *ctx) {
+  slamhip_ctx::ScanPending &sp = ctx->scan_pending;
+  if (!sp.record_due) return;
+  sp.record_due = false;
+  const int k = sp.as.n;
+  if (sp.weighting == 0) ctx->h_weight.assign(k, sp.as.w_even);
+  else if (sp.weighting == 2) ctx->h_weight.assign(sp.as.h_weight, sp.as.h_weight + k);
+  if (sp.as.h_factor) ctx->h_factor.assign(sp.as.h_factor, sp.as.h_factor + k);
+  else ctx->h_factor.assign(k, 1.0);
+}
+
+int scan_assemble_now(slamhip_ctx *ctx) {
+  slamhip_ctx::ScanPending &sp = ctx->scan_pending;
+  if (!sp.active) return SLAMHIP_OK;
+  sp.active = false;
+  const hipError_t e = launch_scan_assemble(sp.as, ctx->d_scan_pull_count, ctx->h_scan_pulled + sp.turn, sp.seq, ctx->stream);
+  scan_record_finish(ctx);
+  SLAMHIP_CHECK(e);
+  return scan_stage_fork(ctx, sp.turn);
+}
+
+int scan_fused_done(slamhip_ctx *ctx) {
+  slamhip_ctx::ScanPending &sp = ctx->scan_pending;
+  if (!sp.active) return SLAMHIP_OK;
+  sp.active = false;
+  ++ctx->raw_prologue_matches;
+  scan_record_finish(ctx);
+  __atomic_store_n(ctx->h_scan_pulled + sp.turn, sp.seq, __ATOMIC_RELAXED);
+  return scan_stage_fork(ctx, sp.turn);
+}
+
+int scan_filter_stage(slamhip_ctx *ctx, int map_id, int n, const double *range, const double *angle, const int *is_occ,
+                      const double *factor, int trig_mode, double a_min, double a_max, double a_inc, const double pose[3],
+                      unsigned skip_rate, double max_range, int bounded, int weighting, int *kept_n, int *kept_idx) {
   if (!ctx || n <= 0 || !range || !angle || !pose) return invalid("bad arguments");
+  {
+    const int rc0 = scan_assemble_now(ctx);
+    if (rc0) return rc0;
+  }
   if (weighting < 0 || weighting > 2) return invalid("unknown weighting kind");
   DeviceMap *m = get_map(ctx, map_id);
   if (bounded && !m) return invalid("unknown map id");
@@ -1407,7 +1458,6 @@
   }
   if (weighting == 0) {
     as.w_even = 1.0 / k;
-    ctx->h_weight.assign(k, as.w_even);
   } else if (weighting == 1) {
     ctx->h_weight.resize(k);
     for (int q = 0; q < k; ++q) ctx->h_weight[q] = sp.viny_f[kept[q]] * std::sqrt(r_[q]);
@@ -1421,16 +1471,12 @@
     if (rc) return rc;
     double *w_ = st + 3 * c;
     std::memcpy(w_, sp.w.data(), sizeof(double) * k);
-    ctx->h_weight.assign(w_, w_ + k);
     as.h_weight = w_;
   }
   if (factor) {
     double *f_ = st + 2 * c;
     for (int q = 0; q < k; ++q) f_[q] = factor[kept[q]];
-    ctx->h_factor.assign(f_, f_ + k);
     as.h_factor = f_;
-  } else {
-    ctx->h_factor.assign(k, 1.0);
   }
   as.tab_cos = ctx->d_scan_tab;
   as.tab_sin = ctx->d_scan_tab + (size_t)ctx->scan_tab_cap;
@@ -1438,15 +1484,25 @@
   as.stride = c;
   as.n = k;
   int turn = 0;
-  const double tot_w = weighting == 0 ? scan_total_weight_even(k, as.w_even) : scan_total_weight(ctx->h_weight.data(), k);
+  const double tot_w = weighting == 0   ? scan_total_weight_even(k, as.w_even)
+                       : weighting == 1 ? scan_total_weight(ctx->h_weight.data(), k)
+                                        : scan_total_weight(as.h_weight, k);
   const unsigned seq = scan_stage_turnover(ctx, k, c, tot_w, &turn);
-  SLAMHIP_CHECK(launch_scan_assemble(as, ctx->d_scan_pull_count, ctx->h_scan_pulled + turn, seq, ctx->stream));
-  rc = scan_stage_fork(ctx, turn);
-  if (rc) return rc;
   sp.kept.swap(kept);
   ctx->scan_angle_lazy = true;
-  return SLAMHIP_OK;
-}
+  slamhip_ctx::ScanPending &pend = ctx->scan_pending;
+  pend.as = as;
+  pend.turn = turn;
+  pend.seq = seq;
+  pend.weighting = weighting;
+  pend.record_due = true;
+  pend.active = true;
+  return SLAMHIP_OK;
+}
+
+}
+
+extern "C" {
 
 int slamhip_scan_set_angles(slamhip_ctx *ctx, int n, const double *angle) {
   if (!ctx || !angle) return invalid("bad arguments");
diff --git a/slam-constructor_amd/csrc/slamhip_internal.h b/slam-constructor_amd/csrc/slamhip_internal.h
--- a/slam-constructor_amd/csrc/slamhip_internal.h
+++ b/slam-constructor_amd/csrc/slamhip_internal.h
@@ -260,6 +260,12 @@
   int scan_tab_cap = 0;
   long long scan_tab_uploads = 0;
   std::vector<double> h_weight, h_factor;
+  struct ScanPending {
+    bool active = false, record_due = false;
+    slamhip::ScanAssembleArgs as{};
+    int turn = 0, weighting = 0;
+    unsigned seq = 0;
+  } scan_pending;
   std::vector<double> h_scan_angle;
   bool scan_angle_lazy = false;
   double *d_scan_angle = nullptr;
@@ -301,6 +307,8 @@
   bool stage_poses = false;
   bool filter_chains = true, k6_batch_fast = true, k6_batch_key64 = false, resident_chains = true, tbm_plane = true;
   int inert_tail = 2;
+  bool raw_prologue = true;
+  long long raw_prologue_matches = 0;
   int k6_path = 0;
   bool profile = false;
   std::vector<hipEvent_t> ev_pool;
@@ -317,6 +325,12 @@
   return ctx->scan_angle_lazy || (int)ctx->h_scan_angle.size() == ctx->scan_n;
 }
 void scan_angles_materialise(slamhip_ctx *ctx);
+int scan_filter_stage(slamhip_ctx *ctx, int map_id, int n, const double *range, const double *angle, const int *is_occ,
+                      const double *factor, int trig_mode, double a_min, double a_max, double a_inc, const double pose[3],
+                      unsigned skip_rate, double max_range, int bounded, int weighting, int *kept_n, int *kept_idx);
+int scan_assemble_now(slamhip_ctx *ctx);
+int scan_fused_done(slamhip_ctx *ctx);
+void scan_record_finish(slamhip_ctx *ctx);
 struct TiledTarget {
   const double *pool;
   const int *tables;
```

Measured after the change: 13.30 billion pose-candidates*beams/s, median of 6. 1.01x the previous value.
